# uber-research/UPSNet

Hardware: AMD Instinct MI355X
Metric: images/sec (whole node), UPSNet-50 1024x2048 (higher is better)
Workload: dtype f32

## Files before the change

include/upsnet_hip.h:

```cpp
#ifndef UPSNET_HIP_H
#define UPSNET_HIP_H

#include <stddef.h>
#include <stdint.h>

#ifdef __cplusplus
extern "C" {
#endif

const char *upsnet_last_error(void);
const char *upsnet_last_kernel_form(void);
int upsnet_abi_version(void);

int upsnet_zero_fill(void *stream, void *ptr, size_t bytes);


int upsnet_roi_align_forward(void *stream, const float *bottom_data, float spatial_scale, int num_rois,
                             int height, int width, int channels, int pooled_height, int pooled_width,
                             int sampling_ratio, const float *bottom_rois, float *top_data);

int upsnet_roi_align_forward_nhwc(void *stream, const float *feat_nhwc, int batch, int height, int width,
                                  int channels, float spatial_scale, const float *rois, int num_rois,
                                  int pooled_height, int pooled_width, int sampling_ratio, float *out_nhwc);

int upsnet_fpn_roi_align_forward(void *stream, const float *const feat_nhwc[4], const int feat_h[4],
                                 const int feat_w[4], const float spatial_scale[4], int channels,
                                 const float *rois, int num_rois, const int *num_rois_dev, int pooled_height,
                                 int pooled_width, int sampling_ratio, float *out_nhwc, int *levels_out);

int upsnet_fpn_roi_order(void *stream, const float *rois, int num_rois, const int *num_rois_dev, int image_height, int image_width,
                         int *order_out);
int upsnet_fpn_roi_align_forward_ordered(void *stream, const float *const feat_nhwc[4], const int feat_h[4], const int feat_w[4],
                                         const float spatial_scale[4], int channels, const float *rois, int num_rois, const int *num_rois_dev,
                                         int pooled_height, int pooled_width, int sampling_ratio, float *out_nhwc, int *levels_out,
                                         const int *order);

void upsnet_roi_tuning(int variant);
void upsnet_roi_geometry(int target_workgroups, int min_bins);


int upsnet_deform_im2col(void *stream, const float *data_im, const float *data_offset, int channels,
                         int height, int width, int ksize_h, int ksize_w, int pad_h, int pad_w, int stride_h,
                         int stride_w, int dilation_h, int dilation_w, int parallel_imgs, int deformable_group,
                         float *data_col);

int upsnet_mod_deform_im2col(void *stream, const float *data_im, const float *data_offset,
                             const float *data_mask, int batch_size, int channels, int height_im, int width_im,
                             int height_col, int width_col, int kernel_h, int kernel_w, int pad_h, int pad_w,
                             int stride_h, int stride_w, int dilation_h, int dilation_w, int deformable_group,
                             float *data_col);


int upsnet_roi_align_backward(void *stream, const float *top_diff, float spatial_scale, int batch_size, int num_rois,
                              int height, int width, int channels, int pooled_height, int pooled_width,
                              int sampling_ratio, const float *bottom_rois, float *bottom_diff);

int upsnet_deform_col2im(void *stream, const float *data_col, const float *data_offset, int channels, int height,
                         int width, int ksize_h, int ksize_w, int pad_h, int pad_w, int stride_h, int stride_w,
                         int dilation_h, int dilation_w, int parallel_imgs, int deformable_group, float *grad_im);

int upsnet_deform_col2im_coord(void *stream, const float *data_col, const float *data_im, const float *data_offset,
                               int channels, int height, int width, int ksize_h, int ksize_w, int pad_h, int pad_w,
                               int stride_h, int stride_w, int dilation_h, int dilation_w, int parallel_imgs,
                               int deformable_group, float *grad_offset);

int upsnet_mod_deform_col2im(void *stream, const float *data_col, const float *data_offset, const float *data_mask,
                             int batch_size, int channels, int height_im, int width_im, int height_col, int width_col,
                             int kernel_h, int kernel_w, int pad_h, int pad_w, int stride_h, int stride_w,
                             int dilation_h, int dilation_w, int deformable_group, float *grad_im);

int upsnet_mod_deform_col2im_coord(void *stream, const float *data_col, const float *data_im, const float *data_offset,
                                   const float *data_mask, int batch_size, int channels, int height_im, int width_im,
                                   int height_col, int width_col, int kernel_h, int kernel_w, int pad_h, int pad_w,
                                   int stride_h, int stride_w, int dilation_h, int dilation_w, int deformable_group,
                                   float *grad_offset, float *grad_mask);

int upsnet_deform_conv_forward_nhwc(void *stream, int nlev, const float *const x[], const float *const offset[],
                                    const float *const mask[], float *const out[], const int height[],
                                    const int width[], int cin, int cout, int kh, int kw, int pad_h, int pad_w,
                                    int stride_h, int stride_w, int dil_h, int dil_w, int deformable_group,
                                    const float *wpack, int ldw, const float *bias, int relu);

size_t upsnet_dcn_packed_weight_floats(int cout, int cin, int kh, int kw);
int upsnet_dcn_pack_weight(void *stream, const float *weight, int cout, int cin, int kh, int kw, float *wpack);
int upsnet_deform_conv_fused_nhwc(void *stream, int nlev, const float *const x[], const float *const offset[],
                                  const float *const mask[], float *const out[], const int height[], const int width[],
                                  int cin, int cout, int kh, int kw, int pad, int stride, int dil, const float *wpack,
                                  const float *bias, int relu);
size_t upsnet_deform_conv_fused_splitk_workspace_bytes(int height, int width, int cout, int kh, int kw, int pad, int stride, int dil,
                                                       int ksplit);
int upsnet_deform_conv_fused_nhwc_splitk(void *stream, const float *x, const float *offset, const float *mask, float *out, int height,
                                         int width, int cin, int cout, int kh, int kw, int pad, int stride, int dil,
                                         const float *wpack, const float *bias, int relu, int ksplit, void *workspace);
void upsnet_dcn_tuning(int variant);

size_t upsnet_dcn_packed_weight_bf16_elems(int cout, int cin, int kh, int kw);
int upsnet_dcn_pack_weight_bf16(void *stream, const float *weight, int cout, int cin, int kh, int kw, void *wpack);
int upsnet_deform_conv_fused_nhwc_bf16(void *stream, int nlev, const float *const x[], const float *const offset[],
                                       const float *const mask[], float *const out[], const int height[], const int width[], int cin,
                                       int cout, int kh, int kw, int pad, int stride, int dil, const void *wpack, const float *bias,
                                       int relu);


int upsnet_prep_image_u8(void *stream, const unsigned char *image_hwc, int height, int width, const double pixel_means[3],
                         double im_scale, int resized_h, int resized_w, int padded_h, int padded_w, int nhwc4, float *blob);

int upsnet_image_to_nhwc4(void *stream, const float *nchw, int batch, int channels, int height, int width, float *nhwc4);


int upsnet_conv2d_nhwc_f32_multiw(void *stream, int nseg, const float *const x[], float *const out[], const int batch[],
                                  const int height[], const int width[], int Cin, const float *const wpack[], int ldw, int Cout,
                                  int KH, int KW, int stride, int pad, int relu);

int upsnet_conv2d_nhwc_f32(void *stream, int nseg, const float *const x[], const float *const residual[],
                           float *const out[], const int batch[], const int height[], const int width[], int Cin,
                           const float *wpack, int ldw, const float *bias, int Cout, int KH, int KW, int stride, int pad,
                           int relu, int residual_up);

size_t upsnet_conv2d_splitk_workspace_bytes(int batch, int height, int width, int Cout, int KH, int KW, int stride, int pad, int ksplit);
int upsnet_conv2d_nhwc_f32_splitk(void *stream, const float *x, const float *residual, float *out, int batch, int height, int width,
                                  int Cin, const float *wpack, int ldw, const float *bias, int Cout, int KH, int KW, int stride,
                                  int pad, int relu, int ksplit, void *workspace);

int upsnet_conv2d_winograd_nhwc_f32(void *stream, int nseg, const float *const x[], const float *const residual[],
                                    float *const out[], const int batch[], const int height[], const int width[], int Cin,
                                    const float *wpack, int ldw, const float *bias, int Cout, int relu);

int upsnet_conv2d_winograd_nhwc_f32_splitk(void *stream, const float *x, const float *residual, float *out, int batch, int height,
                                           int width, int Cin, const float *wpack, int ldw, const float *bias, int Cout, int relu,
                                           int ksplit, void *workspace);
int upsnet_conv_pack_weight_winograd(void *stream, const float *weight, int cout, int cin, int ldw, float *wpack);

int upsnet_conv2d_winograd_nhwc_f32_tn32(void *stream, int nseg, const float *const x[], const float *const residual[],
                                         float *const out[], const int batch[], const int height[], const int width[], int Cin,
                                         const float *wpack, int ldw, const float *bias, int Cout, int relu);
int upsnet_conv_pack_weight_winograd_tn32(void *stream, const float *weight, int cout, int cin, int ldw, float *wpack);
int upsnet_conv2d_winograd_nhwc_f32_tail(void *stream, const float *x, float *out, int batch, int n_main, int height, int width, int Cin,
                                         const float *wpack, int ldw, const float *wpack32, int ldw32, const float *bias, int Cout, int relu);

int upsnet_conv2d_nhwc_bf16(void *stream, int nseg, const float *const x[], const float *const residual[], float *const out[],
                            const int batch[], const int height[], const int width[], int Cin, const void *wpack_hi,
                            const void *wpack_lo, int ldw, const float *bias, int Cout, int KH, int KW, int stride, int pad,
                            int relu);
int upsnet_conv_pack_weight_bf16(void *stream, const float *weight, int cout, int cin, int kh, int kw, int ldw, void *wpack_hi,
                                 void *wpack_lo);
int upsnet_bottleneck_proj_bf16(void *stream, const void *x, void *out, int batch, int height_in, int width_in, int cin, int cmid, int stride,
                                const void *w1, const void *w2, const void *w3d, const float *b1, const float *b2, const float *b3d);
int upsnet_conv_bf16_tuning(int enable, int tile_rows);
int upsnet_conv1x1_bf16_tuning(int enable);
int upsnet_stem_pool_pack_weight_f32(void *stream, const float *weight, int cin, float *wpack);
int upsnet_stem_pool_f32(void *stream, const float *x4, int batch, int height, int width, const float *wpack, const float *bias, float *out);
int upsnet_stem_pool_pack_weight_bf16(void *stream, const float *weight, int cin, void *wpack);
int upsnet_stem_pool_bf16(void *stream, const float *x4, int batch, int height, int width, const void *wpack, const float *bias, void *out);
int upsnet_deconv2x2_nhwc_bf16(void *stream, const void *x, int batch, int height, int width, int Cin, const void *wpack_hi, int ldw,
                               const float *bias, int Cout, int relu, void *out, int out_bf16);

int upsnet_bottleneck_bf16(void *stream, const void *x, void *out, int batch, int height, int width, int cmid, const void *w1,
                           const void *w2, const void *w3, const float *b1, const float *b2, const float *b3);

int upsnet_conv2d_stem_nhwc4_f32(void *stream, const float *x, int batch, int height, int width, const float *wpack,
                                 int ldw, const float *bias, int Cout, int KH, int KW, int stride, int pad, int relu,
                                 float *out);
int upsnet_conv_pack_weight_stem(void *stream, const float *weight, int cout, int cin, int kh, int kw, int ldw, float *wpack);

int upsnet_deconv2x2_nhwc_f32(void *stream, const float *x, int batch, int height, int width, int Cin, const float *wpack,
                              int ldw, const float *bias, int Cout, int relu, float *out);
int upsnet_deconv2x2_pack_weight(void *stream, const float *weight, int cin, int cout, int ldw, float *wpack);

int upsnet_deconv2x2_frag_nhwc_f32(void *stream, const float *x, float *out, int batch, int height, int width, int Cin,
                                   const float *wpack, const float *bias4, int Cout, int relu);

void upsnet_conv_tuning(int winograd_tiles, int force_tile);

int upsnet_conv_pack_weight(void *stream, const float *weight, int cout, int cin, int kh, int kw, int ldw, float *wpack);

int upsnet_conv1x1_frag_nhwc_f32(void *stream, const float *x, const float *residual, float *out, int batch, int height, int width,
                                 int Cin, const float *wpack, const float *bias, int Cout, int stride, int relu, int residual_up);
void upsnet_conv1x1_tuning(int bn);
int upsnet_conv1x1_siblings_nhwc_f32(void *stream, const float *x, float *out_a, float *out_b, int batch, int height, int width, int Cin,
                                     const float *wpack, const float *bias, int cout_a, int cout_b, int stride, int relu_a, int relu_b);
void upsnet_conv1x1_pair32_tuning(int waves);

int upsnet_conv2d_winograd36_nhwc_f32(void *stream, int nseg, const float *const x[], float *const out[], const int batch[],
                                      const int height[], const int width[], int Cin, const float *wpack, int ldw, const float *bias,
                                      int Cout, int relu);
int upsnet_conv_pack_weight_winograd36(void *stream, const float *weight, int cout, int cin, int ldw, float *wpack);
size_t upsnet_conv2d_winograd36_splitk_workspace_bytes(int batch, int height, int width, int Cout, int ksplit);
int upsnet_conv2d_winograd36_nhwc_f32_splitk(void *stream, const float *x, float *out, int batch, int height, int width, int Cin,
                                             const float *wpack, int ldw, const float *bias, int Cout, int relu, int ksplit, void *workspace);

size_t upsnet_conv1x1_ksw_packed_weight_floats(int cout, int cin);
int upsnet_conv1x1_ksw_pack_weight(void *stream, const float *weight, int cout, int cin, float *wpack);
int upsnet_conv1x1_ksw_nhwc_f32(void *stream, const float *x, const float *residual, float *out, int batch, int height, int width, int Cin,
                                const float *wpack, const float *bias, int Cout, int stride, int relu, int tile_pixels, int tile_channels,
                                int split_n);
void upsnet_conv1x1_ksw_tuning(int tile);

size_t upsnet_conv3x3_ksw_packed_weight_floats(int cin);
int upsnet_conv3x3_ksw_pack_weight(void *stream, const float *weight, int cout, int cin, float *wpack);
int upsnet_conv3x3_ksw_nhwc_f32(void *stream, const float *x, float *out, int batch, int height, int width, int Cin, const float *wpack,
                                const float *bias, int Cout, int relu);

size_t upsnet_conv1x1_splitk_workspace_bytes(int batch, int out_height, int out_width, int Cout, int ksplit);
int upsnet_conv1x1_frag_nhwc_f32_splitk(void *stream, const float *x, const float *residual, float *out, int batch, int height, int width,
                                        int Cin, const float *wpack, const float *bias, int Cout, int stride, int relu, int ksplit,
                                        void *workspace);

int upsnet_conv1x1_pair_nhwc_f32(void *stream, const float *x, const float *residual, float *out1, float *out2, long pixels, int C0,
                                 const float *w3pack, const float *bias3, int C1, const float *w1pack, const float *bias1, int C2);


int upsnet_nms_host(int *keep_out_host, int *num_out_host, const float *boxes_host, int boxes_num,
                    int boxes_dim, float nms_overlap_thresh, int device_id);

size_t upsnet_nms_workspace_bytes(int num_problems, int nmax);
int upsnet_nms_batched(void *stream, const float *boxes, const float *scores, const int *counts,
                       const uint8_t *pre_removed, int num_problems, int nmax, float thresh, int *keep_idx,
                       int *keep_cnt, void *workspace);

void upsnet_nms_tuning(int lds_staging);

int upsnet_cpu_nms_batched(void *stream, const float *boxes, const float *scores, const int *counts, int num_problems,
                           int nmax, double thresh, int *keep_idx, int *keep_cnt, void *workspace);

size_t upsnet_soft_nms_batched_workspace_bytes(int num_problems, int nmax);
int upsnet_soft_nms_batched(void *stream, float *boxes, int64_t *inds, const int *counts, int num_problems, int nmax,
                            float sigma, float Nt, float threshold, int method, int *n_out, void *workspace);

size_t upsnet_soft_nms_workspace_bytes(int n);
int upsnet_soft_nms(void *stream, float *boxes, int64_t *inds, int n, float sigma, float Nt, float threshold,
                    int method, int *n_out, void *workspace);


size_t upsnet_proposal_workspace_bytes(int nlev, const int *heights_host, const int *widths_host, int num_anchors,
                                       int pre_nms_top_n, int post_nms_top_n);
int upsnet_pyramid_proposals(void *stream, int nlev, const float *const cls_prob[], const float *const bbox_pred[],
                             const int *heights_host, const int *widths_host, const int *strides_host,
                             const float *anchors_host, int num_anchors, const float *im_info, int pre_nms_top_n,
                             int post_nms_top_n, float nms_thresh, float min_size, float *rois_out,
                             float *scores_out, int *num_out, void *workspace);

int upsnet_pyramid_proposals_strided(void *stream, int nlev, const float *const cls_prob[], const float *const bbox_pred[],
                                     const long *cls_chan_stride, const long *cls_pix_stride, const long *box_chan_stride,
                                     const long *box_pix_stride, const int *heights_host, const int *widths_host,
                                     const int *strides_host, const float *anchors_host, int num_anchors, const float *im_info,
                                     int pre_nms_top_n, int post_nms_top_n, float nms_thresh, float min_size, float *rois_out,
                                     float *scores_out, int *num_out, void *workspace);
int upsnet_pyramid_proposals_strided_ordered(void *stream, int nlev, const float *const cls_prob[], const float *const bbox_pred[],
                                     const long *cls_chan_stride, const long *cls_pix_stride, const long *box_chan_stride,
                                     const long *box_pix_stride, const int *heights_host, const int *widths_host,
                                     const int *strides_host, const float *anchors_host, int num_anchors, const float *im_info,
                                     int pre_nms_top_n, int post_nms_top_n, float nms_thresh, float min_size, float *rois_out,
                                     float *scores_out, int *num_out, void *workspace, int *roi_order_out);

int upsnet_pyramid_proposals_joint_strided(void *stream, int nlev, const float *const cls_prob[], const float *const bbox_pred[],
                                           const long *cls_chan_stride, const long *cls_pix_stride, const long *box_chan_stride,
                                           const long *box_pix_stride, const int *heights_host, const int *widths_host,
                                           const int *strides_host, const float *anchors_host, int num_anchors, const float *im_info,
                                           int pre_nms_top_n, int post_nms_top_n, float nms_thresh, float min_size, float *rois_out,
                                           float *scores_out, int *num_out, void *workspace);


int upsnet_mask_roi_capacity(int num_rois, int num_classes, int class_agnostic);
size_t upsnet_mask_roi_workspace_bytes(int num_rois, int num_classes, int class_agnostic);
int upsnet_mask_roi(void *stream, const float *rois, const float *bbox_delta, const float *cls_prob, int num_rois,
                    const int *num_rois_dev, int num_classes, const float *im_info, int class_agnostic,
                    float score_thresh, float nms_thresh, int max_det, const float reg_weights_host[4],
                    float *boxes_out, float *scores_out, int64_t *cls_out, int *src_out, int *num_out,
                    void *workspace);
int upsnet_mask_roi_ex(void *stream, const float *rois, const float *bbox_delta, const float *cls_prob, int num_rois,
                       const int *num_rois_dev, int num_classes, const float *im_info, int class_agnostic, int clip_boxes,
                       float score_thresh, float nms_thresh, int max_det, const float reg_weights_host[4],
                       float *boxes_out, float *scores_out, int64_t *cls_out, int *src_out, int *num_out,
                       void *workspace);

int upsnet_mask_roi_dedup(void *stream, const int *a_src, const int64_t *a_cls, const int *num_a, int cap_a, const int *b_src,
                          const int64_t *b_cls, const float *b_boxes, const int *num_b, int cap_b, int *map_out,
                          float *extra_boxes, int *num_extra);

int upsnet_mask_logit_gather(void *stream, const float *mask_logit, int n_rows, int num_classes, int hw, long stride_n,
                             long stride_c, long stride_e, const int *row, const int64_t *cls, int K, float *out);


size_t upsnet_mask_removal_workspace_bytes(int m, int num_thing_classes, int height, int width);
int upsnet_mask_removal(void *stream, const float *mask_rois, const float *cls_prob, const float *mask_logit,
                        const int64_t *cls_idx, int m, const int *m_dev, int mask_size, int num_thing_classes, int height, int width,
                        double fraction_threshold, int64_t *keep_inds, int *num_keep, int *real_keep,
                        void *workspace);

int upsnet_panoptic_tail_pack(void *stream, const int64_t *keep, const int *num_keep, int K, const int64_t *cls, const float *scores,
                              const int *det_num, const int *pan_num, const int *extra_num, int64_t *kept_cls, float *kept_scores,
                              int *counters);

int upsnet_mask_paste(void *stream, const float *mask_rois, const float *mask_logit, const int64_t *keep_inds,
                      const int *num_keep, const int *real_keep, int kmax, int mask_size, int height, int width,
                      float *mask_energy);

int upsnet_seg_term(void *stream, const float *fcn_output, int num_seg, int height, int width, const float *boxes,
                    const int64_t *cls, const int64_t *class_map, int k, float *seg_inst);

int upsnet_panoptic_fuse(void *stream, const float *fcn_output, int num_seg, int height, int width, int num_stuff,
                         const float *mask_rois, const float *mask_logit, const int64_t *cls_idx,
                         const int64_t *keep_inds, const int *num_keep, const int *real_keep, int kmax,
                         int mask_size, const int64_t *class_map, int enable_void, int64_t *pan_out,
                         int64_t *sem_out);

int upsnet_fcn_score_combine(void *stream, int nlev, const float *const part[], int num_seg, int height, int width,
                             const float *bias, float *score);

int upsnet_panoptic_fuse_up(void *stream, const float *fcn_score, int score_nhwc, int num_seg, int score_h, int score_w,
                            int scale, int num_stuff, const float *mask_rois, const float *mask_logit,
                            const int64_t *cls_idx, const int64_t *keep_inds, const int *num_keep, const int *real_keep,
                            int kmax, int mask_size, const int64_t *class_map, int64_t *pan_out, int64_t *sem_out);

int upsnet_panoptic_argmax(void *stream, const float *fcn_output, int num_seg, int height, int width, int num_stuff,
                           const float *seg_inst, const float *mask_energy, int k, int enable_void,
                           int64_t *pan_out);


size_t upsnet_unified_pan_workspace_bytes(void);
int upsnet_unified_pan_result(void *stream, const int64_t *pan, const int64_t *seg, const int64_t *cls_inds, int num_inst,
                              int height, int width, int id_last_stuff, int num_seg_classes, int stuff_area_limit,
                              void *workspace, unsigned char *pan_2ch);

size_t upsnet_combined_pan_workspace_bytes(int num_images, long total_pixels);
int upsnet_combined_pan_result(void *stream, int num_images, const int64_t *images, int max_height, int max_width, long total_pixels,
                               const int *cand, const int *segments, int id_last_stuff, int num_classes, int stuff_area_limit,
                               double fraction_threshold, void *workspace);

int upsnet_im_post_rle(void *stream, const float *pred_boxes, const float *mask_prob, const int64_t *cls_inds, int num_det,
                       int num_mask_channels, int mask_size, int im_height, int im_width, int cap, unsigned *transitions,
                       int *transition_count);

int upsnet_restore_label_maps(void *stream, const int64_t *sseg, const int64_t *pano, long src_stride, int src_height, int src_width,
                              const int *y_ofs, int out_height, const int *x_ofs, int out_width, unsigned char *out_sseg,
                              unsigned char *out_pano);


size_t upsnet_pq_workspace_bytes(int max_gt);
int upsnet_pq_accumulate(void *stream, const unsigned char *pred_2ch, const unsigned char *gt_rgb, int height, int width,
                         const int64_t *segments, int num_segments, const unsigned char *cat_known, int image_index, int max_gt,
                         void *workspace, int64_t *tp, int64_t *fp, int64_t *fn, double *iou, uint64_t *status);

int upsnet_confusion_accumulate(void *stream, const unsigned char *gt_label, const unsigned char *pred_label, long npix,
                                int class_num, int ignore_label, int64_t *confusion);


size_t upsnet_det_eval_image_workspace_bytes(int num_det, int num_rows, int num_gt, int height, int width, int segm);
int upsnet_det_eval_image(void *stream, int segm, int height, int width, int num_rows, int num_det, const double *det_xyxy,
                          const double *det_score, const int64_t *det_cls, const int *class_to_row, int num_classes,
                          const float *det_box_f32, const float *mask_prob, int num_mask_channels, int mask_size,
                          const int *det_trans, const int64_t *det_trans_off, int num_gt, const int *gt_row_off,
                          const double *gt_box, const double *gt_area, const int *gt_crowd, const int *gt_trans,
                          const int64_t *gt_trans_off, const int *gt_trans_dst, int num_gt_rle, const unsigned char *const *gt_u8,
                          const int *gt_u8_dst, int num_gt_u8, const int *rows_with_gt, int num_rows_with_gt,
                          const double *params, int image_index, void *workspace, double *rec_score, int *rec_img, int *rec_rk,
                          uint64_t *rec_match, uint64_t *rec_ign, int64_t *npig);

size_t upsnet_det_eval_accumulate_workspace_bytes(long num_records, int num_rows);
int upsnet_det_eval_accumulate(void *stream, long num_records, const double *rec_score, const int *rec_img, const int *rec_rk,
                               const uint64_t *rec_match, const uint64_t *rec_ign, const int *img_ord, int num_rows,
                               const int64_t *npig, const double *rec_thrs, void *workspace, double *precision, double *recall,
                               double *scores);

size_t upsnet_poly_raster_workspace_bytes(long total_vertices, long total_points);
int upsnet_poly_raster(void *stream, const double *vertices, const int *poly_off, const int *obj_off, const int *poly_off_dev,
                       const int *obj_off_dev, int num_poly, int num_obj, long total_points, int height, int width, void *workspace,
                       int *trans, int64_t *trans_off);


size_t upsnet_proposal_recall_workspace_bytes(int num_problems, long total_proposals);
int upsnet_proposal_recall(void *stream, int num_problems, const int64_t *problems, const float *proposals, const float *gt_boxes,
                           int max_gt, long total_proposals, void *workspace, float *out);

#ifdef __cplusplus
}
#endif
#endif
```

upsnet_amd/_lib.py:

```python
import ctypes
import os

import torch

_HERE = os.path.dirname(os.path.abspath(__file__))
LIB_PATH = os.environ.get("UPSNET_LIB_PATH") or os.path.join(_HERE, "csrc", "libupsnet_hip.so")

c_int, c_float, c_double, c_void_p, c_size_t, c_long = ctypes.c_int, ctypes.c_float, ctypes.c_double, ctypes.c_void_p, ctypes.c_size_t, ctypes.c_long
P = c_void_p

_SIGNATURES = {
    "upsnet_last_error": (ctypes.c_char_p, []),
    "upsnet_last_kernel_form": (ctypes.c_char_p, []),
    "upsnet_abi_version": (c_int, []),
    "upsnet_zero_fill": (c_int, [P, P, c_size_t]),
    "upsnet_roi_align_forward": (c_int, [P, P, c_float, c_int, c_int, c_int, c_int, c_int, c_int, c_int, P, P]),
    "upsnet_roi_align_forward_nhwc": (c_int, [P, P, c_int, c_int, c_int, c_int, c_float, P, c_int, c_int, c_int, c_int, P]),
    "upsnet_fpn_roi_align_forward": (c_int, [P, P, P, P, P, c_int, P, c_int, P, c_int, c_int, c_int, P, P]),
    "upsnet_fpn_roi_order": (c_int, [P, P, c_int, P, c_int, c_int, P]),
    "upsnet_fpn_roi_align_forward_ordered": (c_int, [P, P, P, P, P, c_int, P, c_int, P, c_int, c_int, c_int, P, P, P]),
    "upsnet_roi_tuning": (None, [c_int]),
    "upsnet_roi_geometry": (None, [c_int, c_int]),
    "upsnet_deform_im2col": (c_int, [P, P, P] + [c_int] * 13 + [P]),
    "upsnet_mod_deform_im2col": (c_int, [P, P, P, P] + [c_int] * 15 + [P]),
    "upsnet_roi_align_backward": (c_int, [P, P, c_float] + [c_int] * 8 + [P, P]),
    "upsnet_deform_col2im": (c_int, [P, P, P] + [c_int] * 13 + [P]),
    "upsnet_deform_col2im_coord": (c_int, [P, P, P, P] + [c_int] * 13 + [P]),
    "upsnet_mod_deform_col2im": (c_int, [P, P, P, P] + [c_int] * 15 + [P]),
    "upsnet_mod_deform_col2im_coord": (c_int, [P, P, P, P, P] + [c_int] * 15 + [P, P]),
    "upsnet_deform_conv_forward_nhwc": (c_int, [P, c_int, P, P, P, P, P, P] + [c_int] * 11 + [P, c_int, P, c_int]),
    "upsnet_dcn_packed_weight_floats": (c_size_t, [c_int, c_int, c_int, c_int]),
    "upsnet_dcn_pack_weight": (c_int, [P, P, c_int, c_int, c_int, c_int, P]),
    "upsnet_deform_conv_fused_nhwc": (c_int, [P, c_int, P, P, P, P, P, P] + [c_int] * 7 + [P, P, c_int]),
    "upsnet_deform_conv_fused_splitk_workspace_bytes": (c_size_t, [c_int] * 9),
    "upsnet_deform_conv_fused_nhwc_splitk": (c_int, [P, P, P, P, P] + [c_int] * 9 + [P, P, c_int, c_int, P]),
    "upsnet_dcn_tuning": (None, [c_int]),
    "upsnet_dcn_packed_weight_bf16_elems": (c_size_t, [c_int, c_int, c_int, c_int]),
    "upsnet_dcn_pack_weight_bf16": (c_int, [P, P, c_int, c_int, c_int, c_int, P]),
    "upsnet_deform_conv_fused_nhwc_bf16": (c_int, [P, c_int, P, P, P, P, P, P] + [c_int] * 7 + [P, P, c_int]),
    "upsnet_conv1x1_frag_nhwc_f32": (c_int, [P, P, P, P, c_int, c_int, c_int, c_int, P, P, c_int, c_int, c_int, c_int]),
    "upsnet_conv1x1_tuning": (None, [c_int]),
    "upsnet_conv1x1_siblings_nhwc_f32": (c_int, [P, P, P, P, c_int, c_int, c_int, c_int, P, P, c_int, c_int, c_int, c_int, c_int]),
    "upsnet_conv1x1_pair32_tuning": (None, [c_int]),
    "upsnet_conv1x1_splitk_workspace_bytes": (ctypes.c_size_t, [c_int, c_int, c_int, c_int, c_int]),
    "upsnet_conv1x1_frag_nhwc_f32_splitk": (c_int, [P, P, P, P, c_int, c_int, c_int, c_int, P, P, c_int, c_int, c_int, c_int, P]),
    "upsnet_conv1x1_ksw_packed_weight_floats": (ctypes.c_size_t, [c_int, c_int]),
    "upsnet_conv1x1_ksw_pack_weight": (c_int, [P, P, c_int, c_int, P]),
    "upsnet_conv1x1_ksw_nhwc_f32": (c_int, [P, P, P, P, c_int, c_int, c_int, c_int, P, P, c_int, c_int, c_int, c_int, c_int, c_int]),
    "upsnet_conv1x1_ksw_tuning": (None, [c_int]),
    "upsnet_conv3x3_ksw_packed_weight_floats": (ctypes.c_size_t, [c_int]),
    "upsnet_conv3x3_ksw_pack_weight": (c_int, [P, P, c_int, c_int, P]),
    "upsnet_conv3x3_ksw_nhwc_f32": (c_int, [P, P, P, c_int, c_int, c_int, c_int, P, P, c_int, c_int]),
    "upsnet_conv2d_winograd36_splitk_workspace_bytes": (ctypes.c_size_t, [c_int, c_int, c_int, c_int, c_int]),
    "upsnet_conv2d_winograd36_nhwc_f32_splitk": (c_int, [P, P, P, c_int, c_int, c_int, c_int, P, c_int, P, c_int, c_int, c_int, P]),
    "upsnet_conv1x1_pair_nhwc_f32": (c_int, [P, P, P, P, P, c_long, c_int, P, P, c_int, P, P, c_int]),
    "upsnet_conv2d_nhwc_f32": (c_int, [P, c_int, P, P, P, P, P, P, c_int, P, c_int, P, c_int, c_int, c_int, c_int, c_int, c_int, c_int]),
    "upsnet_conv2d_nhwc_f32_multiw": (c_int, [P, c_int, P, P, P, P, P, c_int, P, c_int, c_int, c_int, c_int, c_int, c_int, c_int]),
    "upsnet_conv_tuning": (None, [c_int, c_int]),
    "upsnet_conv_pack_weight": (c_int, [P, P, c_int, c_int, c_int, c_int, c_int, P]),
    "upsnet_nms_host": (c_int, [P, P, P, c_int, c_int, c_float, c_int]),
    "upsnet_nms_workspace_bytes": (c_size_t, [c_int, c_int]),
    "upsnet_nms_batched": (c_int, [P, P, P, P, P, c_int, c_int, c_float, P, P, P]),
    "upsnet_nms_tuning": (None, [c_int]),
    "upsnet_cpu_nms_batched": (c_int, [P, P, P, P, c_int, c_int, c_double, P, P, P]),
    "upsnet_soft_nms_batched_workspace_bytes": (c_size_t, [c_int, c_int]),
    "upsnet_soft_nms_batched": (c_int, [P, P, P, P, c_int, c_int, c_float, c_float, c_float, c_int, P, P]),
    "upsnet_soft_nms_workspace_bytes": (c_size_t, [c_int]),
    "upsnet_soft_nms": (c_int, [P, P, P, c_int, c_float, c_float, c_float, c_int, P, P]),
    "upsnet_proposal_workspace_bytes": (c_size_t, [c_int, P, P, c_int, c_int, c_int]),
    "upsnet_pyramid_proposals_strided": (c_int, [P, c_int, P, P, P, P, P, P, P, P, P, P, c_int, P, c_int, c_int, c_float, c_float, P, P, P, P]),
    "upsnet_pyramid_proposals_strided_ordered": (c_int, [P, c_int, P, P, P, P, P, P, P, P, P, P, c_int, P, c_int, c_int, c_float, c_float, P, P, P, P, P]),
    "upsnet_pyramid_proposals_joint_strided": (c_int, [P, c_int, P, P, P, P, P, P, P, P, P, P, c_int, P, c_int, c_int, c_float, c_float, P, P, P, P]),
    "upsnet_pyramid_proposals": (c_int, [P, c_int, P, P, P, P, P, P, c_int, P, c_int, c_int, c_float, c_float, P, P, P, P]),
    "upsnet_mask_roi_capacity": (c_int, [c_int, c_int, c_int]),
    "upsnet_mask_roi_workspace_bytes": (c_size_t, [c_int, c_int, c_int]),
    "upsnet_mask_roi": (c_int, [P, P, P, P, c_int, P, c_int, P, c_int, c_float, c_float, c_int, P, P, P, P, P, P, P]),
    "upsnet_mask_roi_ex": (c_int, [P, P, P, P, c_int, P, c_int, P, c_int, c_int, c_float, c_float, c_int, P, P, P, P, P, P, P]),
    "upsnet_mask_logit_gather": (c_int, [P, P, c_int, c_int, c_int, c_long, c_long, c_long, P, P, c_int, P]),
    "upsnet_mask_removal_workspace_bytes": (c_size_t, [c_int, c_int, c_int, c_int]),
    "upsnet_mask_removal": (c_int, [P, P, P, P, P, c_int, P, c_int, c_int, c_int, c_int, c_double, P, P, P, P]),
    "upsnet_panoptic_tail_pack": (c_int, [P, P, P, c_int, P, P, P, P, P, P, P, P]),
    "upsnet_mask_paste": (c_int, [P, P, P, P, P, P, c_int, c_int, c_int, c_int, P]),
    "upsnet_seg_term": (c_int, [P, P, c_int, c_int, c_int, P, P, P, c_int, P]),
    "upsnet_panoptic_fuse": (c_int, [P, P, c_int, c_int, c_int, c_int, P, P, P, P, P, P, c_int, c_int, P, c_int, P, P]),
    "upsnet_panoptic_fuse_up": (c_int, [P, P, c_int, c_int, c_int, c_int, c_int, c_int, P, P, P, P, P, P, c_int, c_int, P, P, P]),
    "upsnet_conv2d_stem_nhwc4_f32": (c_int, [P, P, c_int, c_int, c_int, P, c_int, P, c_int, c_int, c_int, c_int, c_int, c_int, P]),
    "upsnet_conv_pack_weight_stem": (c_int, [P, P, c_int, c_int, c_int, c_int, c_int, P]),
    "upsnet_deconv2x2_nhwc_f32": (c_int, [P, P, c_int, c_int, c_int, c_int, P, c_int, P, c_int, c_int, P]),
    "upsnet_deconv2x2_pack_weight": (c_int, [P, P, c_int, c_int, c_int, P]),
    "upsnet_deconv2x2_frag_nhwc_f32": (c_int, [P, P, P, c_int, c_int, c_int, c_int, P, P, c_int, c_int]),
    "upsnet_prep_image_u8": (c_int, [P, P, c_int, c_int, P, c_double, c_int, c_int, c_int, c_int, c_int, P]),
    "upsnet_image_to_nhwc4": (c_int, [P, P, c_int, c_int, c_int, c_int, P]),
    "upsnet_unified_pan_workspace_bytes": (c_size_t, []),
    "upsnet_unified_pan_result": (c_int, [P, P, P, P, c_int, c_int, c_int, c_int, c_int, c_int, P, P]),
    "upsnet_combined_pan_workspace_bytes": (c_size_t, [c_int, c_long]),
    "upsnet_combined_pan_result": (c_int, [P, c_int, P, c_int, c_int, c_long, P, P, c_int, c_int, c_int, c_double, P]),
    "upsnet_mask_roi_dedup": (c_int, [P, P, P, P, c_int, P, P, P, P, c_int, P, P, P]),
    "upsnet_conv2d_winograd_nhwc_f32": (c_int, [P, c_int, P, P, P, P, P, P, c_int, P, c_int, P, c_int, c_int]),
    "upsnet_conv2d_winograd_nhwc_f32_splitk": (c_int, [P, P, P, P, c_int, c_int, c_int, c_int, P, c_int, P, c_int, c_int, c_int, P]),
    "upsnet_conv_pack_weight_winograd": (c_int, [P, P, c_int, c_int, c_int, P]),
    "upsnet_conv_pack_weight_winograd_tn32": (c_int, [P, P, c_int, c_int, c_int, P]),
    "upsnet_conv2d_winograd_nhwc_f32_tn32": (c_int, [P, c_int, P, P, P, P, P, P, c_int, P, c_int, P, c_int, c_int]),
    "upsnet_conv2d_winograd_nhwc_f32_tail": (c_int, [P, P, P, c_int, c_int, c_int, c_int, c_int, P, c_int, P, c_int, P, c_int, c_int]),
    "upsnet_conv2d_winograd36_nhwc_f32": (c_int, [P, c_int, P, P, P, P, P, c_int, P, c_int, P, c_int, c_int]),
    "upsnet_conv_pack_weight_winograd36": (c_int, [P, P, c_int, c_int, c_int, P]),
    "upsnet_conv2d_nhwc_bf16": (c_int, [P, c_int, P, P, P, P, P, P, c_int, P, P, c_int, P, c_int, c_int, c_int, c_int, c_int, c_int]),
    "upsnet_bottleneck_proj_bf16": (c_int, [P, P, P, c_int, c_int, c_int, c_int, c_int, c_int, P, P, P, P, P, P]),
    "upsnet_conv_bf16_tuning": (c_int, [c_int, c_int]),
    "upsnet_conv1x1_bf16_tuning": (c_int, [c_int]),
    "upsnet_stem_pool_pack_weight_f32": (c_int, [P, P, c_int, P]),
    "upsnet_stem_pool_f32": (c_int, [P, P, c_int, c_int, c_int, P, P, P]),
    "upsnet_stem_pool_pack_weight_bf16": (c_int, [P, P, c_int, P]),
    "upsnet_stem_pool_bf16": (c_int, [P, P, c_int, c_int, c_int, P, P, P]),
    "upsnet_deconv2x2_nhwc_bf16": (c_int, [P, P, c_int, c_int, c_int, c_int, P, c_int, P, c_int, c_int, P, c_int]),
    "upsnet_bottleneck_bf16": (c_int, [P, P, P, c_int, c_int, c_int, c_int, P, P, P, P, P, P]),
    "upsnet_conv_pack_weight_bf16": (c_int, [P, P, c_int, c_int, c_int, c_int, c_int, P, P]),
    "upsnet_conv2d_splitk_workspace_bytes": (c_size_t, [c_int, c_int, c_int, c_int, c_int, c_int, c_int, c_int, c_int]),
    "upsnet_conv2d_nhwc_f32_splitk": (c_int, [P, P, P, P, c_int, c_int, c_int, c_int, P, c_int, P, c_int, c_int, c_int, c_int, c_int, c_int, c_int, P]),
    "upsnet_im_post_rle": (c_int, [P, P, P, P, c_int, c_int, c_int, c_int, c_int, c_int, P, P]),
    "upsnet_fcn_score_combine": (c_int, [P, c_int, P, c_int, c_int, c_int, P, P]),
    "upsnet_panoptic_argmax": (c_int, [P, P, c_int, c_int, c_int, c_int, P, P, c_int, c_int, P]),
    "upsnet_pq_workspace_bytes": (c_size_t, [c_int]),
    "upsnet_pq_accumulate": (c_int, [P, P, P, c_int, c_int, P, c_int, P, c_int, c_int, P, P, P, P, P, P]),
    "upsnet_restore_label_maps": (c_int, [P, P, P, c_long, c_int, c_int, P, c_int, P, c_int, P, P]),
    "upsnet_confusion_accumulate": (c_int, [P, P, P, c_long, c_int, c_int, P]),
    "upsnet_det_eval_image_workspace_bytes": (c_size_t, [c_int] * 6),
    "upsnet_det_eval_image": (c_int, [P, c_int, c_int, c_int, c_int, c_int, P, P, P, P, c_int, P, P, c_int, c_int, P, P, c_int, P, P, P, P,
                                      P, P, P, c_int, P, P, c_int, P, c_int, P, c_int, P, P, P, P, P, P, P]),
    "upsnet_det_eval_accumulate_workspace_bytes": (c_size_t, [c_long, c_int]),
    "upsnet_det_eval_accumulate": (c_int, [P, c_long, P, P, P, P, P, P, c_int, P, P, P, P, P, P]),
    "upsnet_poly_raster_workspace_bytes": (c_size_t, [c_long, c_long]),
    "upsnet_poly_raster": (c_int, [P, P, P, P, P, P, c_int, c_int, c_long, c_int, c_int, P, P, P]),
    "upsnet_proposal_recall_workspace_bytes": (c_size_t, [c_int, c_long]),
    "upsnet_proposal_recall": (c_int, [P, c_int, P, P, P, c_int, c_long, P, P]),
}

_lib = None


def exported_symbols():
    return sorted(_SIGNATURES)


def lib():
    global _lib
    if _lib is None:
        if not os.path.exists(LIB_PATH):
            raise RuntimeError("upsnet_amd: %s is missing -- build it with `python -m upsnet_amd.build` "
                               "(there is no CPU fallback)" % LIB_PATH)
        l = ctypes.CDLL(LIB_PATH)
        for name, (res, args) in _SIGNATURES.items():
            fn = getattr(l, name)
            fn.restype = res
            fn.argtypes = args
        _lib = l
    return _lib


def check(rc, what):
    if rc != 0:
        raise RuntimeError("upsnet_amd.%s failed: %s" % (what, lib().upsnet_last_error().decode()))


def ptr(t):
    return None if t is None else c_void_p(t.data_ptr())


def stream():
    return c_void_p(torch.cuda.current_stream().cuda_stream)


def require_cuda(*tensors):
    for t in tensors:
        if t is not None and not t.is_cuda:
            raise Exception("not implemented")


def f32c(t):
    if t.dtype != torch.float32:
        t = t.float()
    return t.contiguous()


def nhwc(t):
    return t.contiguous(memory_format=torch.channels_last)


def int_array(vals):
    return (c_int * len(vals))(*[int(v) for v in vals])


def float_array(vals):
    return (c_float * len(vals))(*[float(v) for v in vals])


def ptr_array(tensors):
    return (c_void_p * len(tensors))(*[None if t is None else t.data_ptr() for t in tensors])
```

upsnet_amd/csrc/conv_params.h:

```cpp
#pragma once
#include "common.h"

#define CV_BM 128
#define CV_BK 32
#define CV_LDA (CV_BM + 1)
#define CV_MAXSEG 5

typedef float floatx16 __attribute__((ext_vector_type(16)));

struct ConvSeg {
    const float *x, *res, *off, *mask;
    const float *w;
    float *out;
    int N, H, W, Ho, Wo;
    int OH, OW;
    int tile_start;
    long M;
};

struct ConvParams {
    ConvSeg seg[CV_MAXSEG];
    const float *w, *bias;
    int nseg, Cin, Cout, ldw, KH, KW, stride, pad, dil, relu;
    int res_up;
    int m_tiles, n_tiles;
    int ksplit;
    float *partial;
    long m_total;
    int io;
    int sib_split, sib_relu;
    float *sib_out;
};

static inline int conv_fill(ConvParams &p, const char *who, int nseg, const float *const x[], const float *const res[],
                     const float *const off[], const float *const mask[], float *const out[], const int batch[],
                     const int height[], const int width[], int Cin, int Cout, const float *wpack, int ldw, const float *bias,
                     int KH, int KW, int stride, int pad, int dil, int relu)
{
    UPS_REQUIRE(nseg >= 1 && nseg <= CV_MAXSEG, "%s: 1..%d feature maps per launch (got %d)", who, CV_MAXSEG, nseg);
    UPS_REQUIRE(x && out && height && width && wpack, "%s: null pointer", who);
    UPS_REQUIRE(Cin > 0 && Cin % CV_BK == 0, "%s: Cin must be a multiple of 32 (got %d)", who, Cin);
    UPS_REQUIRE(Cout > 0 && ldw % 32 == 0 && ldw >= Cout, "%s: ldw must be Cout rounded up to 32 (got %d for Cout=%d)", who, ldw, Cout);
    UPS_REQUIRE(KH >= 1 && KW >= 1 && KH * KW <= 49 && stride >= 1 && pad >= 0 && dil >= 1, "%s: bad kernel/stride/pad/dilation", who);
    UPS_REQUIRE((long)KH * KW * Cin * ldw < (1L << 30), "%s: packed weight exceeds 4 GiB", who);
    p.w = wpack; p.bias = bias; p.nseg = nseg; p.Cin = Cin; p.Cout = Cout; p.ldw = ldw; p.KH = KH; p.KW = KW;
    p.stride = stride; p.pad = pad; p.dil = dil; p.relu = relu; p.res_up = 0;
    p.ksplit = 1; p.partial = nullptr; p.m_total = 0; p.io = 0; p.sib_split = 0; p.sib_relu = 0; p.sib_out = nullptr;
    int tiles = 0;
    for (int i = 0; i < CV_MAXSEG; ++i) {
        ConvSeg &s = p.seg[i];
        if (i < nseg) {
            const int nb = batch ? batch[i] : 1;
            UPS_REQUIRE(x[i] && out[i] && nb > 0 && height[i] > 0 && width[i] > 0, "%s: bad feature map %d", who, i);
            s.x = x[i]; s.out = out[i]; s.res = res ? res[i] : nullptr; s.off = off ? off[i] : nullptr; s.mask = mask ? mask[i] : nullptr;
            s.w = nullptr;
            s.N = nb; s.H = height[i]; s.W = width[i];
            s.OH = s.OW = 0;
            s.Ho = (height[i] + 2 * pad - (dil * (KH - 1) + 1)) / stride + 1;
            s.Wo = (width[i] + 2 * pad - (dil * (KW - 1) + 1)) / stride + 1;
            UPS_REQUIRE(s.Ho > 0 && s.Wo > 0, "%s: empty output for feature map %d", who, i);
            UPS_REQUIRE((long)nb * height[i] * width[i] * Cin < (1L << 30), "%s: feature map %d exceeds 4 GiB (32-bit byte offsets); split the batch", who, i);
            s.M = (long)nb * s.Ho * s.Wo;
            UPS_REQUIRE(s.M * Cout < (1L << 29), "%s: output %d exceeds 2 GiB (32-bit byte offsets in the epilogue); split the batch", who, i);
            s.tile_start = tiles;
            tiles += (int)((s.M + 127) / 128);
        } else {
            s.x = s.res = s.off = s.mask = nullptr; s.w = nullptr; s.out = nullptr;
            s.N = s.H = s.W = s.Ho = s.Wo = s.OH = s.OW = 0; s.M = 0; s.tile_start = 0x7fffffff;
        }
    }
    p.m_tiles = tiles;
    return 0;
}


int conv_splitk_reduce(hipStream_t st, const float *partial, int ksplit, long m_total, long M, int Cout, const float *bias, const float *res,
                       int relu, float *out);
```

upsnet_amd/csrc/conv_wino.hip:

```cpp
#include <cstdlib>
#include "conv_params.h"
#include "upsnet_hip.h"

#define WG_STEPS 32

typedef unsigned uintx4 __attribute__((ext_vector_type(4)));
typedef unsigned uintx2 __attribute__((ext_vector_type(2)));

__device__ static inline float f1sub(const float a, const float b) { float r; asm("v_sub_f32 %0, %1, %2" : "=v"(r) : "v"(a), "v"(b)); return r; }
__device__ static inline float f1add(const float a, const float b) { float r; asm("v_add_f32 %0, %1, %2" : "=v"(r) : "v"(a), "v"(b)); return r; }
__device__ static inline float2 f2sub(const float2 a, const float2 b) { return make_float2(f1sub(a.x, b.x), f1sub(a.y, b.y)); }
__device__ static inline float2 f2add(const float2 a, const float2 b) { return make_float2(f1add(a.x, b.x), f1add(a.y, b.y)); }

template <bool SPLITK, int TM, int TN>
__device__ __forceinline__ void conv_wino16_body(const ConvParams &p, const int wg)
{
    static_assert(TN == 64 || (TN == 32 && TM == 32), "tile forms: 64x64, 32x64, 32x32");
    extern __shared__ __attribute__((aligned(16))) unsigned char smem_raw[];
    constexpr unsigned WG_BUF = 16u * 4u * TM * 16u;
    constexpr int NPAIR = (TM / 32) * (TN / 32);
    constexpr int NX = (TM / 8) / NPAIR;
    constexpr int NA = 16 / NX;
    constexpr int NS = 2 * NA;
    constexpr unsigned BSTEP = TN * 32u;
    constexpr int WG_RING = 4;
    const int tid = threadIdx.x, lane = tid & 63, wave = tid >> 6;
    const int pair = wave % NPAIR, xh = wave / NPAIR;
    const int wm = TM == 64 ? (pair & 1) : 0, wn = TM == 64 ? (pair >> 1) : pair;
    const int lhalf = lane >> 5, l32 = lane & 31;
    int m_t, n_t, kz;
    {
        const int nt = p.n_tiles;
        const int per = (p.m_tiles + 7) >> 3;
        const int base_grid = 8 * per * nt;
        kz = SPLITK ? wg / base_grid : 0;
        const int bid = wg - kz * base_grid;
        const int q = bid >> 3;
        n_t = q % nt;
        const int local = q / nt;
        m_t = (bid & 7) * per + local;
        if (local >= per || m_t >= p.m_tiles) return;
    }
    int si = 0;
#pragma unroll
    for (int q = 1; q < CV_MAXSEG; ++q) if (q < p.nseg && m_t >= p.seg[q].tile_start) si = q;
    const ConvSeg sg = p.seg[si];
    const long p0 = (long)(m_t - sg.tile_start) * TM;
    const int n0 = n_t * TN;
    const int nslabs = p.Cin >> 4;
    const int s_per = SPLITK ? (nslabs + p.ksplit - 1) / p.ksplit : nslabs;
    const int s_begin = kz * s_per, s_end = min(s_begin + s_per, nslabs);
    const long HoWo = (long)sg.Ho * sg.Wo;

    const int ltile = tid >> 3, lc2 = tid & 7, lq = lc2 >> 1;
    unsigned ro0, ro1, ro2, ro3, co0, co1, co2, co3;
    {
        const long pp = p0 + ltile;
        const bool tile_ok = pp < sg.M;
        const long ppc = tile_ok ? pp : sg.M - 1;
        const int n = (int)(ppc / HoWo);
        const int rem = (int)(ppc - (long)n * HoWo);
        const int ty = rem / sg.Wo, tx = rem - ty * sg.Wo;
        const int h0 = 2 * ty - 1, w0 = 2 * tx - 1;
        const unsigned cin4 = 4u * (unsigned)p.Cin;
        unsigned ro[4], co[4];
#pragma unroll
        for (int r = 0; r < 4; ++r) {
            const int h = h0 + r, w = w0 + r;
            const unsigned rv = (unsigned)((n * sg.H + min(max(h, 0), sg.H - 1)) * sg.W) * cin4;
            const unsigned cv = (unsigned)min(max(w, 0), sg.W - 1) * cin4 + 8u * (unsigned)lc2;
            ro[r] = rv | ((tile_ok && h >= 0 && h < sg.H) ? 0u : 0x80000000u);
            co[r] = cv | ((w >= 0 && w < sg.W) ? 0u : 0x40000000u);
        }
        ro0 = ro[0]; ro1 = ro[1]; ro2 = ro[2]; ro3 = ro[3];
        co0 = co[0]; co1 = co[1]; co2 = co[2]; co3 = co[3];
    }
    const size_t xaddr = reinterpret_cast<size_t>(sg.x);
    const unsigned xlo = __builtin_amdgcn_readfirstlane((unsigned)xaddr), xhi = __builtin_amdgcn_readfirstlane((unsigned)(xaddr >> 32));
    const unsigned xbytes = __builtin_amdgcn_readfirstlane((unsigned)(sg.N * sg.H * sg.W) * 4u * (unsigned)p.Cin);
    const char *xbase = reinterpret_cast<const char *>(((size_t)xhi << 32) | xlo);
    const unsigned st_base = (unsigned)((lq * TM + (ltile ^ (2 * lq))) * 16 + (lc2 & 1) * 8);
    const int frow = 32 * wm + l32;
    constexpr unsigned PLANE = TM * 16u;
    const unsigned fr_base0 = (unsigned)(lhalf * PLANE + (frow ^ (2 * lhalf)) * 16 + xh * NS * 2 * PLANE);
    const unsigned fr_base1 = (unsigned)(lhalf * PLANE + (frow ^ (4 + 2 * lhalf)) * 16 + xh * NS * 2 * PLANE);
    const size_t waddr = reinterpret_cast<size_t>(p.w) + (size_t)n_t * (size_t)nslabs * (WG_STEPS * BSTEP);
    const unsigned wlo = __builtin_amdgcn_readfirstlane((unsigned)waddr), whi = __builtin_amdgcn_readfirstlane((unsigned)(waddr >> 32));
    const __amdgpu_buffer_rsrc_t wrsrc = __builtin_amdgcn_make_buffer_rsrc(reinterpret_cast<void *>(((size_t)whi << 32) | wlo), 0,
                                                                            nslabs * (int)(WG_STEPS * BSTEP), 0x00020000);
    const unsigned b_lane = (unsigned)(lhalf * (TN * 16) + (32 * wn + l32) * 16);
    const int gmax = nslabs * WG_STEPS - 1;
    const int xh_u = __builtin_amdgcn_readfirstlane(xh);

    floatx16 acc[NA];
#pragma unroll
    for (int i = 0; i < NA; ++i)
#pragma unroll
        for (int r = 0; r < 16; ++r) acc[i][r] = 0.f;

#define WG_PO(PX) (((PX) >> 2) == 0 ? ro0 : ((PX) >> 2) == 1 ? ro1 : ((PX) >> 2) == 2 ? ro2 : ro3) + (((PX) & 3) == 0 ? co0 : ((PX) & 3) == 1 ? co1 : ((PX) & 3) == 2 ? co2 : co3)
    float2 ld[16];
    float4 breg[WG_RING];

#define WG_LOAD(PX, RS) { const uintx2 v_ = __builtin_amdgcn_raw_buffer_load_b64(RS, WG_PO(PX), 0, 0); ld[PX] = make_float2(__uint_as_float(v_.x), __uint_as_float(v_.y)); }
#define WG_ROWPASS(R)                                                                                                 \
    {                                                                                                                 \
        const float2 d0 = ld[4 * R + 0], d1 = ld[4 * R + 1], d2 = ld[4 * R + 2], d3 = ld[4 * R + 3];                 \
        ld[4 * R + 0] = f2sub(d0, d2); ld[4 * R + 1] = f2add(d1, d2); ld[4 * R + 2] = f2sub(d2, d1); ld[4 * R + 3] = f2sub(d1, d3); \
    }
#define WG_COLSTASH(J, SB)                                                                                            \
    {                                                                                                                 \
        *reinterpret_cast<float2 *>(smem_raw + (SB) + (0 * 4 + J) * 4 * PLANE) = f2sub(ld[0 + J], ld[8 + J]);            \
        *reinterpret_cast<float2 *>(smem_raw + (SB) + (1 * 4 + J) * 4 * PLANE) = f2add(ld[4 + J], ld[8 + J]);            \
        *reinterpret_cast<float2 *>(smem_raw + (SB) + (2 * 4 + J) * 4 * PLANE) = f2sub(ld[8 + J], ld[4 + J]);            \
        *reinterpret_cast<float2 *>(smem_raw + (SB) + (3 * 4 + J) * 4 * PLANE) = f2sub(ld[4 + J], ld[12 + J]);           \
    }
#define WG_BLOAD(SLOT, G) { const uintx4 v_ = __builtin_amdgcn_raw_buffer_load_b128(wrsrc, b_lane, (unsigned)min((G), gmax) * BSTEP, 0); \
        breg[SLOT] = make_float4(__uint_as_float(v_.x), __uint_as_float(v_.y), __uint_as_float(v_.z), __uint_as_float(v_.w)); }

    {
        const __amdgpu_buffer_rsrc_t xr = __builtin_amdgcn_make_buffer_rsrc(const_cast<char *>(xbase) + (size_t)s_begin * 64, 0, xbytes - (unsigned)s_begin * 64u, 0x00020000);
#pragma unroll
        for (int i = 0; i < 16; ++i) WG_LOAD(i, xr)
#pragma unroll
        for (int u = 0; u < WG_RING; ++u) WG_BLOAD(u, s_begin * WG_STEPS + NS * xh_u + u)
        WG_ROWPASS(0) WG_ROWPASS(1) WG_ROWPASS(2) WG_ROWPASS(3)
        WG_COLSTASH(0, st_base) WG_COLSTASH(1, st_base) WG_COLSTASH(2, st_base) WG_COLSTASH(3, st_base)
    }
    __syncthreads();
    float4 afr = *reinterpret_cast<const float4 *>(smem_raw + fr_base0);

    for (int s = s_begin; s < s_end; ++s) {
        const int sn = min(s + 1, s_end - 1);
        const __amdgpu_buffer_rsrc_t xr = __builtin_amdgcn_make_buffer_rsrc(const_cast<char *>(xbase) + (size_t)sn * 64, 0, xbytes - (unsigned)sn * 64u, 0x00020000);
        const unsigned cur = ((s - s_begin) & 1) ? WG_BUF : 0u, nxt = WG_BUF - cur;
        const unsigned sb = nxt + st_base;
        const int g0 = s * WG_STEPS + NS * xh_u;
#pragma unroll
        for (int u = 0; u < NS; ++u) {
            if (NS == 16 && u < 8) { WG_LOAD(2 * u, xr) WG_LOAD(2 * u + 1, xr) }
            if (NS == 8 && u < 4) { WG_LOAD(4 * u, xr) WG_LOAD(4 * u + 1, xr) WG_LOAD(4 * u + 2, xr) WG_LOAD(4 * u + 3, xr) }
            float4 afn;
            if (u < NS - 1) afn = *reinterpret_cast<const float4 *>(smem_raw + cur + (((u + 1) & 1) ? fr_base1 : fr_base0) + (unsigned)(u + 1) * 2u * PLANE);
            else afn = *reinterpret_cast<const float4 *>(smem_raw + nxt + fr_base0);
            if (NS == 16) {
                if (u == 8) WG_ROWPASS(0)
                if (u == 9) WG_ROWPASS(1)
                if (u == 10) WG_ROWPASS(2)
                if (u == 11) { WG_ROWPASS(3) WG_COLSTASH(0, sb) }
                if (u == 12) WG_COLSTASH(1, sb)
                if (u == 13) WG_COLSTASH(2, sb)
                if (u == 14) WG_COLSTASH(3, sb)
            } else {
                if (u == 4) { WG_ROWPASS(0) WG_ROWPASS(1) }
                if (u == 5) { WG_ROWPASS(2) WG_ROWPASS(3) WG_COLSTASH(0, sb) }
                if (u == 6) { WG_COLSTASH(1, sb) WG_COLSTASH(2, sb) WG_COLSTASH(3, sb) }
            }
            const float4 bf = breg[u % WG_RING];
            acc[u >> 1] = __builtin_amdgcn_mfma_f32_32x32x2f32(afr.x, bf.x, acc[u >> 1], 0, 0, 0);
            acc[u >> 1] = __builtin_amdgcn_mfma_f32_32x32x2f32(afr.y, bf.y, acc[u >> 1], 0, 0, 0);
            acc[u >> 1] = __builtin_amdgcn_mfma_f32_32x32x2f32(afr.z, bf.z, acc[u >> 1], 0, 0, 0);
            acc[u >> 1] = __builtin_amdgcn_mfma_f32_32x32x2f32(afr.w, bf.w, acc[u >> 1], 0, 0, 0);
            WG_BLOAD(u % WG_RING, (u + WG_RING < NS ? g0 : g0 + WG_STEPS - NS) + u + WG_RING)
            if (u == NS - 2) __syncthreads();
            afr = afn;
            __builtin_amdgcn_sched_barrier(0);
        }
    }
#undef WG_LOAD
#undef WG_PO
#undef WG_ROWPASS
#undef WG_COLSTASH
#undef WG_BLOAD

    __syncthreads();
    const bool has_res = sg.res != nullptr;
    const long pbase = p0 + wm * 32 + 4 * lhalf;
    const long pb = pbase < sg.M ? pbase : sg.M - 1;
    const int n_b = (int)(pb / HoWo);
    const int rem_b = (int)(pb - (long)n_b * HoWo);
    const int h_b = rem_b / sg.Wo, w_b = rem_b - h_b * sg.Wo;
    const bool fast = sg.Wo >= 32;
    const int co = n0 + wn * 32 + l32;
    const bool co_ok = co < p.Cout;
    const float bv = (p.bias != nullptr && co_ok) ? p.bias[co] : 0.f;
#define WG_WHERE(OFF, N_, H_, W_)                                                                                     \
    int N_ = n_b, H_ = h_b, W_ = w_b;                                                                                 \
    if (fast) {                                                                                                       \
        W_ += (OFF);                                                                                                  \
        if (W_ >= sg.Wo) { W_ -= sg.Wo; ++H_; }                                                                       \
        if (H_ >= sg.Ho) { H_ -= sg.Ho; ++N_; }                                                                       \
    } else {                                                                                                          \
        const long pp_ = pbase + (OFF);                                                                               \
        N_ = (int)(pp_ / HoWo);                                                                                       \
        const int rem_ = (int)(pp_ - (long)N_ * HoWo);                                                                \
        H_ = rem_ / sg.Wo; W_ = rem_ - H_ * sg.Wo;                                                                    \
    }
    const unsigned crow = (unsigned)p.Cout * 4u;
    const unsigned co4 = 4u * (unsigned)co;
    const size_t oaddr_ = reinterpret_cast<size_t>(SPLITK ? (float *)(p.partial + (long)kz * p.m_total * p.Cout) : sg.out);
    const unsigned obytes_ = __builtin_amdgcn_readfirstlane((unsigned)(SPLITK ? p.m_total : (long)sg.N * sg.OH * sg.OW) * crow);
    const __amdgpu_buffer_rsrc_t orsrc = __builtin_amdgcn_make_buffer_rsrc(
        reinterpret_cast<void *>(((size_t)(unsigned)__builtin_amdgcn_readfirstlane((unsigned)(oaddr_ >> 32)) << 32) | (unsigned)__builtin_amdgcn_readfirstlane((unsigned)oaddr_)),
        0, (int)obytes_, 0x00020000);
    const size_t raddr_ = reinterpret_cast<size_t>(has_res ? sg.res : sg.out);
    const __amdgpu_buffer_rsrc_t rrsrc = __builtin_amdgcn_make_buffer_rsrc(
        reinterpret_cast<void *>(((size_t)(unsigned)__builtin_amdgcn_readfirstlane((unsigned)(raddr_ >> 32)) << 32) | (unsigned)__builtin_amdgcn_readfirstlane((unsigned)raddr_)),
        0, (int)__builtin_amdgcn_readfirstlane((unsigned)((long)sg.N * sg.OH * sg.OW) * crow), 0x00020000);
#define WG_STORE_ROW(N_, OY, OX, V0, V1)                                                                              \
    if ((OY) < sg.OH) {                                                                                               \
        float v0_ = (V0), v1_ = (V1);                                                                                 \
        const unsigned o0_ = (unsigned)(((N_) * sg.OH + (OY)) * sg.OW + (OX)) * crow + co4;                           \
        const unsigned o1_ = ((OX) + 1 < sg.OW) ? o0_ + crow : 0x80000000u;                                           \
        if (!SPLITK) {                                                                                                \
            v0_ = v0_ + bv; v1_ = v1_ + bv;                                                                           \
            if (has_res) {                                                                                            \
                v0_ = v0_ + __uint_as_float(__builtin_amdgcn_raw_buffer_load_b32(rrsrc, o0_, 0, 0));                  \
                v1_ = v1_ + __uint_as_float(__builtin_amdgcn_raw_buffer_load_b32(rrsrc, o1_, 0, 0));                  \
            }                                                                                                         \
            if (p.relu) { v0_ = fmaxf(v0_, 0.f); v1_ = fmaxf(v1_, 0.f); }                                             \
        }                                                                                                             \
        __builtin_amdgcn_raw_buffer_store_b32(__float_as_uint(v0_), orsrc, o0_, 0, 0);                                \
        __builtin_amdgcn_raw_buffer_store_b32(__float_as_uint(v1_), orsrc, o1_, 0, 0);                                \
    }
    if constexpr (NX == 2) {
        float4 *mine = reinterpret_cast<float4 *>(smem_raw + pair * 32768 + xh_u * 16384) + lane;
        const float4 *theirs = reinterpret_cast<const float4 *>(smem_raw + pair * 32768 + (1 - xh_u) * 16384) + lane;
        if (xh_u == 0) {
#pragma unroll
            for (int r = 0; r < 16; ++r) mine[r * 64] = make_float4(acc[4][r], acc[5][r], acc[6][r], acc[7][r]);
        } else {
#pragma unroll
            for (int r = 0; r < 16; ++r) mine[r * 64] = make_float4(acc[0][r], acc[1][r], acc[2][r], acc[3][r]);
        }
        __syncthreads();
#pragma unroll
        for (int r = 0; r < 16; ++r) {
            const int off = (r & 3) + 8 * (r >> 2);
            const float4 o = theirs[r * 64];
            if (!(co_ok && pbase + off < sg.M)) continue;
            WG_WHERE(off, n, h, w)
            float t0, t1, t2, t3;
            if (xh_u == 0) {
                t0 = (acc[0][r] + acc[4][r]) + o.x; t1 = (acc[1][r] + acc[5][r]) + o.y;
                t2 = (acc[2][r] + acc[6][r]) + o.z; t3 = (acc[3][r] + acc[7][r]) + o.w;
            } else {
                t0 = (o.x - acc[0][r]) - acc[4][r]; t1 = (o.y - acc[1][r]) - acc[5][r];
                t2 = (o.z - acc[2][r]) - acc[6][r]; t3 = (o.w - acc[3][r]) - acc[7][r];
            }
            WG_STORE_ROW(n, 2 * h + xh_u, 2 * w, (t0 + t1) + t2, (t1 - t2) - t3)
        }
    } else {
        float4 *mine = reinterpret_cast<float4 *>(smem_raw + xh_u * 16384) + lane;
#pragma unroll
        for (int r = 0; r < 16; ++r) mine[r * 64] = make_float4(acc[0][r], acc[1][r], acc[2][r], acc[3][r]);
        __syncthreads();
#pragma unroll
        for (int rr = 0; rr < 4; ++rr) {
            const int r = 4 * xh_u + rr;
            const int off = rr + 8 * xh_u;
            const float4 m0 = reinterpret_cast<const float4 *>(smem_raw)[r * 64 + lane];
            const float4 m1 = reinterpret_cast<const float4 *>(smem_raw + 16384)[r * 64 + lane];
            const float4 m2 = reinterpret_cast<const float4 *>(smem_raw + 32768)[r * 64 + lane];
            const float4 m3 = reinterpret_cast<const float4 *>(smem_raw + 49152)[r * 64 + lane];
            if (!(co_ok && pbase + off < sg.M)) continue;
            WG_WHERE(off, n, h, w)
            const float a0 = (m0.x + m1.x) + m2.x, a1 = (m0.y + m1.y) + m2.y, a2 = (m0.z + m1.z) + m2.z, a3 = (m0.w + m1.w) + m2.w;
            const float b0 = (m1.x - m2.x) - m3.x, b1 = (m1.y - m2.y) - m3.y, b2 = (m1.z - m2.z) - m3.z, b3 = (m1.w - m2.w) - m3.w;
            WG_STORE_ROW(n, 2 * h, 2 * w, (a0 + a1) + a2, (a1 - a2) - a3)
            WG_STORE_ROW(n, 2 * h + 1, 2 * w, (b0 + b1) + b2, (b1 - b2) - b3)
        }
    }
#undef WG_WHERE
#undef WG_STORE_ROW
}

template <bool SPLITK, int TM, int TN>
__global__ void __launch_bounds__(8 * TM, TM == 64 ? 1 : 2) conv_wino16_f32_kernel(const ConvParams p)
{
    conv_wino16_body<SPLITK, TM, TN>(p, (int)blockIdx.x);
}

__global__ void __launch_bounds__(256, 2) conv_wino16_tail_f32_kernel(const ConvParams pm, const ConvParams pt, const int main_grid)
{
    if ((int)blockIdx.x < main_grid) conv_wino16_body<false, 32, 64>(pm, (int)blockIdx.x);
    else conv_wino16_body<false, 32, 32>(pt, (int)blockIdx.x - main_grid);
}

template <int TM, int TN>
static int conv_wino16_launch_tm(hipStream_t st, ConvParams &p)
{
    int tiles = 0;
    for (int i = 0; i < p.nseg; ++i) { p.seg[i].tile_start = tiles; tiles += (int)((p.seg[i].M + TM - 1) / TM); }
    p.m_tiles = tiles;
    p.n_tiles = p.ldw / TN;
    const size_t smem = 2 * 16 * 4 * TM * 16;
    static std::atomic<unsigned long long> attr_dev{0};
    UPS_ONCE_PER_DEVICE(attr_dev,
        UPS_CHECK_HIP(hipFuncSetAttribute(reinterpret_cast<const void *>(&conv_wino16_f32_kernel<false, TM, TN>), hipFuncAttributeMaxDynamicSharedMemorySize, (int)smem));
        UPS_CHECK_HIP(hipFuncSetAttribute(reinterpret_cast<const void *>(&conv_wino16_f32_kernel<true, TM, TN>), hipFuncAttributeMaxDynamicSharedMemorySize, (int)smem)));
    const int grid = 8 * ((p.m_tiles + 7) / 8) * p.n_tiles;
    if (p.ksplit > 1) hipLaunchKernelGGL((conv_wino16_f32_kernel<true, TM, TN>), dim3(grid * p.ksplit), dim3(8 * TM), smem, st, p);
    else hipLaunchKernelGGL((conv_wino16_f32_kernel<false, TM, TN>), dim3(grid), dim3(8 * TM), smem, st, p);
    UPS_CHECK_LAUNCH("conv_wino16_f32_kernel");
    ups_set_form("wino<%d,%d,%d>", p.ksplit > 1 ? 1 : 0, TM, TN);
    return 0;
}

int g_wino_tm = 0;
static int conv_wino16_launch(hipStream_t st, ConvParams &p, int tn32 = 0)
{
    UPS_REQUIRE(p.Cin % 16 == 0 && (p.ldw == 32 || p.ldw % 64 == 0 || (tn32 && p.ldw % 32 == 0)), "conv2d_winograd_nhwc_f32: Cin %% 16 must be 0 and ldw 32 or a multiple of 64");
    for (int i = 0; i < p.nseg; ++i) {
        UPS_REQUIRE((long)p.seg[i].N * p.seg[i].H * p.seg[i].W * p.Cin < (1L << 28), "conv2d_winograd_nhwc_f32: feature map %d exceeds 1 GiB; split the batch", i);
        UPS_REQUIRE((long)p.seg[i].N * p.seg[i].OH * p.seg[i].OW * p.Cout < (1L << 29), "conv2d_winograd_nhwc_f32: output %d exceeds 2 GiB; split the batch", i);
    }
    if (p.ksplit > 1) {
        const int nslabs = p.Cin / 16;
        UPS_REQUIRE(p.nseg == 1 && p.partial, "conv2d_winograd_nhwc_f32_splitk: one map and a workspace");
        UPS_REQUIRE(((nslabs + p.ksplit - 1) / p.ksplit) * (p.ksplit - 1) < nslabs, "conv2d_winograd_nhwc_f32_splitk: %d K slabs cannot be split %d ways", nslabs, p.ksplit);
        p.m_total = (long)p.seg[0].N * p.seg[0].OH * p.seg[0].OW;
    }
    if (p.ldw == 32 || tn32) {
        UPS_REQUIRE(p.ldw % 32 == 0, "conv2d_winograd_nhwc_f32: the 32-channel form needs ldw %% 32 == 0");
        return conv_wino16_launch_tm<32, 32>(st, p);
    }
    long wgs64 = 0;
    for (int i = 0; i < p.nseg; ++i) wgs64 += (p.seg[i].M + 63) / 64;
    wgs64 *= p.ldw / 64;
    static const long tm64_min = getenv("UPSNET_WINO_TM64_MIN") ? atol(getenv("UPSNET_WINO_TM64_MIN")) : 768;
    const int tm = g_wino_tm ? g_wino_tm : (wgs64 > tm64_min ? 64 : 32);
    return tm == 32 ? conv_wino16_launch_tm<32, 64>(st, p) : conv_wino16_launch_tm<64, 64>(st, p);
}

__global__ void conv_pack_weight_wino16_kernel(const float *__restrict__ w, int cout, int cin, int ldw, int tn, float *__restrict__ wp)
{
    const long total = (long)ldw * cin;
    const int nslabs = cin >> 4;
    for (long idx = (long)blockIdx.x * blockDim.x + threadIdx.x; idx < total; idx += (long)blockDim.x * gridDim.x) {
        const int co = idx % ldw, c = idx / ldw;
        float g[3][3], t[4][3], u[4][4];
#pragma unroll
        for (int a = 0; a < 3; ++a)
#pragma unroll
            for (int b = 0; b < 3; ++b) g[a][b] = co < cout ? w[(((long)co * cin + c) * 3 + a) * 3 + b] : 0.f;
#pragma unroll
        for (int b = 0; b < 3; ++b) {
            t[0][b] = g[0][b];
            t[1][b] = 0.5f * ((g[0][b] + g[1][b]) + g[2][b]);
            t[2][b] = 0.5f * ((g[0][b] - g[1][b]) + g[2][b]);
            t[3][b] = g[2][b];
        }
#pragma unroll
        for (int a = 0; a < 4; ++a) {
            u[a][0] = t[a][0];
            u[a][1] = 0.5f * ((t[a][0] + t[a][1]) + t[a][2]);
            u[a][2] = 0.5f * ((t[a][0] - t[a][1]) + t[a][2]);
            u[a][3] = t[a][2];
        }
        const long blk = ((long)(co / tn) * nslabs + (c >> 4)) * 16;
        const int q = (c & 15) >> 2, ci = c & 3, cl = co % tn;
#pragma unroll
        for (int a = 0; a < 4; ++a)
#pragma unroll
            for (int b = 0; b < 4; ++b) wp[(((blk + a * 4 + b) * 4 + q) * tn + cl) * 4 + ci] = u[a][b];
    }
}

static int wino_pack(void *stream, const float *weight, int cout, int cin, int ldw, int tn, float *wpack)
{
    UPS_REQUIRE(weight && wpack && cout > 0 && cin > 0 && ldw >= cout, "conv_pack_weight_winograd: bad args");
    UPS_REQUIRE(cin % 16 == 0 && (tn == 32 || tn == 64) && ldw % tn == 0, "conv_pack_weight_winograd: Cin %% 16 must be 0 and ldw a multiple of the channel tile");
    const long total = (long)ldw * cin;
    int blocks = (int)((total + 255) / 256);
    if (blocks > 65535) blocks = 65535;
    hipLaunchKernelGGL(conv_pack_weight_wino16_kernel, dim3(blocks), dim3(256), 0, (hipStream_t)stream, weight, cout, cin, ldw, tn, wpack);
    UPS_CHECK_LAUNCH("conv_pack_weight_wino16_kernel");
    return 0;
}

extern "C" int upsnet_conv_pack_weight_winograd(void *stream, const float *weight, int cout, int cin, int ldw, float *wpack)
{
    UPS_REQUIRE(ldw == 32 || ldw % 64 == 0, "conv_pack_weight_winograd: ldw 32 or a multiple of 64");
    return wino_pack(stream, weight, cout, cin, ldw, ldw == 32 ? 32 : 64, wpack);
}

extern "C" int upsnet_conv_pack_weight_winograd_tn32(void *stream, const float *weight, int cout, int cin, int ldw, float *wpack)
{
    return wino_pack(stream, weight, cout, cin, ldw, 32, wpack);
}

static int wino_fill(ConvParams &p, const char *who, int nseg, const float *const x[], const float *const residual[], float *const out[],
                     const int batch[], const int height[], const int width[], int Cin, int Cout, const float *wpack, int ldw,
                     const float *bias, int relu)
{
    int rc = conv_fill(p, who, nseg, x, residual, nullptr, nullptr, out, batch, height, width, Cin, Cout, wpack, ldw, bias, 3, 3, 1, 1, 1, relu);
    if (rc) return rc;
    UPS_REQUIRE((long)16 * Cin * ldw < (1L << 30), "%s: packed weight exceeds 4 GiB", who);
    for (int i = 0; i < nseg; ++i) {
        ConvSeg &s = p.seg[i];
        s.OH = s.Ho; s.OW = s.Wo;
        s.Ho = (s.OH + 1) / 2; s.Wo = (s.OW + 1) / 2;
        s.M = (long)s.N * s.Ho * s.Wo;
    }
    return 0;
}

extern "C" int upsnet_conv2d_winograd_nhwc_f32(void *stream, int nseg, const float *const x[], const float *const residual[],
                                               float *const out[], const int batch[], const int height[], const int width[], int Cin,
                                               const float *wpack, int ldw, const float *bias, int Cout, int relu)
{
    ConvParams p;
    int rc = wino_fill(p, "conv2d_winograd_nhwc_f32", nseg, x, residual, out, batch, height, width, Cin, Cout, wpack, ldw, bias, relu);
    if (rc) return rc;
    return conv_wino16_launch((hipStream_t)stream, p);
}

extern "C" int upsnet_conv2d_winograd_nhwc_f32_tn32(void *stream, int nseg, const float *const x[], const float *const residual[],
                                                    float *const out[], const int batch[], const int height[], const int width[], int Cin,
                                                    const float *wpack, int ldw, const float *bias, int Cout, int relu)
{
    ConvParams p;
    int rc = wino_fill(p, "conv2d_winograd_nhwc_f32_tn32", nseg, x, residual, out, batch, height, width, Cin, Cout, wpack, ldw, bias, relu);
    if (rc) return rc;
    return conv_wino16_launch((hipStream_t)stream, p, 1);
}

extern "C" int upsnet_conv2d_winograd_nhwc_f32_tail(void *stream, const float *x, float *out, int batch, int n_main, int height, int width,
                                                    int Cin, const float *wpack, int ldw, const float *wpack32, int ldw32, const float *bias,
                                                    int Cout, int relu)
{
    UPS_REQUIRE(x && out && wpack && wpack32 && n_main > 0 && n_main < batch && ldw % 64 == 0 && ldw32 % 32 == 0 && Cin % 16 == 0,
                "conv2d_winograd_nhwc_f32_tail: 0 < n_main < batch, ldw %% 64 == 0, ldw32 %% 32 == 0, Cin %% 16 == 0");
    ConvParams pm, pt;
    const float *xm[1] = {x}, *xt[1] = {x + (size_t)n_main * height * width * Cin};
    float *om[1] = {out}, *ot[1] = {out + (size_t)n_main * height * width * Cout};
    const int nm[1] = {n_main}, nt[1] = {batch - n_main}, hh[1] = {height}, ww[1] = {width};
    int rc = wino_fill(pm, "conv2d_winograd_nhwc_f32_tail", 1, xm, nullptr, om, nm, hh, ww, Cin, Cout, wpack, ldw, bias, relu);
    if (rc) return rc;
    rc = wino_fill(pt, "conv2d_winograd_nhwc_f32_tail", 1, xt, nullptr, ot, nt, hh, ww, Cin, Cout, wpack32, ldw32, bias, relu);
    if (rc) return rc;
    UPS_REQUIRE((long)batch * height * width * Cin < (1L << 28) && (long)batch * height * width * Cout < (1L << 29),
                "conv2d_winograd_nhwc_f32_tail: feature map exceeds 1 GiB; split the batch");
    pm.seg[0].tile_start = 0; pm.m_tiles = (int)((pm.seg[0].M + 31) / 32); pm.n_tiles = ldw / 64;
    pt.seg[0].tile_start = 0; pt.m_tiles = (int)((pt.seg[0].M + 31) / 32); pt.n_tiles = ldw32 / 32;
    const int main_grid = 8 * ((pm.m_tiles + 7) / 8) * pm.n_tiles, tail_grid = 8 * ((pt.m_tiles + 7) / 8) * pt.n_tiles;
    const size_t smem = 2 * 16 * 4 * 32 * 16;
    static std::atomic<unsigned long long> attr_dev{0};
    UPS_ONCE_PER_DEVICE(attr_dev, UPS_CHECK_HIP(hipFuncSetAttribute(reinterpret_cast<const void *>(&conv_wino16_tail_f32_kernel), hipFuncAttributeMaxDynamicSharedMemorySize, (int)smem)));
    hipLaunchKernelGGL(conv_wino16_tail_f32_kernel, dim3(main_grid + tail_grid), dim3(256), smem, (hipStream_t)stream, pm, pt, main_grid);
    UPS_CHECK_LAUNCH("conv_wino16_tail_f32_kernel");
    ups_set_form("wino_tail<%d,%d>", main_grid, tail_grid);
    return 0;
}

extern "C" int upsnet_conv2d_winograd_nhwc_f32_splitk(void *stream, const float *x, const float *residual, float *out, int batch, int height,
                                                      int width, int Cin, const float *wpack, int ldw, const float *bias, int Cout, int relu,
                                                      int ksplit, void *workspace)
{
    const float *xs[1] = {x};
    float *os[1] = {out};
    const int nb[1] = {batch}, hh[1] = {height}, ww[1] = {width};
    ConvParams p;
    int rc = wino_fill(p, "conv2d_winograd_nhwc_f32_splitk", 1, xs, nullptr, os, nb, hh, ww, Cin, Cout, wpack, ldw, bias, relu);
    if (rc) return rc;
    UPS_REQUIRE(workspace && ksplit >= 2 && ksplit <= 8, "conv2d_winograd_nhwc_f32_splitk: ksplit must be 2..8 and a workspace given");
    UPS_REQUIRE(Cout % 4 == 0, "conv2d_winograd_nhwc_f32_splitk: Cout must be a multiple of 4");
    p.ksplit = ksplit;
    p.partial = (float *)workspace;
    rc = conv_wino16_launch((hipStream_t)stream, p);
    if (rc) return rc;
    return conv_splitk_reduce((hipStream_t)stream, p.partial, ksplit, p.m_total, p.m_total, Cout, bias, residual, relu, out);
}
```

upsnet_amd/csrc/conv_wino36.hip:

```cpp
#include <cstdlib>
#include <type_traits>
#include "conv_params.h"
#include "upsnet_hip.h"

#define W36_TM 32
#define W36_TN 64
#define W36_PTS 36
#define W36_VBUF (W36_PTS * 4 * W36_TM * 16)
#define W36_BSTEP (2 * W36_TN * 16)
#define W36_STEPS (2 * W36_PTS)
#define W36_XCH (16 * W36_PTS * 64 * 4)
#define W36_RING 3

typedef unsigned w36_uintx4 __attribute__((ext_vector_type(4)));

#define W36_BT(D0, D1, D2, D3, D4, D5)                                                                               \
    {                                                                                                                \
        const float a0_ = D0, a1_ = D1, a2_ = D2, a3_ = D3, a4_ = D4, a5_ = D5;                                       \
        const float e1_ = __builtin_fmaf(-2.25f, a2_, a4_), o1_ = __builtin_fmaf(-2.25f, a1_, a3_);                   \
        const float e3_ = __builtin_fmaf(-0.5625f, a2_, a4_), o3_ = __builtin_fmaf(-0.5625f, a1_, a3_);               \
        D0 = __builtin_fmaf(1.265625f, a0_, __builtin_fmaf(-2.8125f, a2_, a4_));                                     \
        D1 = __builtin_fmaf(0.75f, o1_, e1_);                                                                        \
        D2 = __builtin_fmaf(-0.75f, o1_, e1_);                                                                       \
        D3 = __builtin_fmaf(1.5f, o3_, e3_);                                                                         \
        D4 = __builtin_fmaf(-1.5f, o3_, e3_);                                                                        \
        D5 = __builtin_fmaf(1.265625f, a1_, __builtin_fmaf(-2.8125f, a3_, a5_));                                     \
    }
#define W36_AT(M0, M1, M2, M3, M4, M5, Y0, Y1, Y2, Y3)                                                               \
    {                                                                                                                \
        const float s1_ = (M1) + (M2), d1_ = (M1) - (M2), s2_ = (M3) + (M4), d2_ = (M3) - (M4);                      \
        Y0 = ((M0) + s1_) + s2_;                                                                                     \
        Y1 = __builtin_fmaf(1.5f, d2_, 0.75f * d1_);                                                                 \
        Y2 = __builtin_fmaf(2.25f, s2_, 0.5625f * s1_);                                                              \
        Y3 = __builtin_fmaf(3.375f, d2_, __builtin_fmaf(0.421875f, d1_, (M5)));                                      \
    }

template <bool SK>
__global__ void __launch_bounds__(512, 1) conv_wino36_f32_kernel(const ConvParams p)
{
    extern __shared__ __attribute__((aligned(16))) unsigned char smem_raw[];
    const int tid = threadIdx.x, lane = tid & 63;
    const int wave = __builtin_amdgcn_readfirstlane(tid >> 6);
    const int cb = wave >> 2, pg = wave & 3;
    const int lhalf = lane >> 5, l32 = lane & 31;
    int m_t, n_t, kz = 0;
    {
        const int nt = p.n_tiles;
        const int per = (p.m_tiles + 7) >> 3;
        int bid = (int)blockIdx.x;
        if constexpr (SK) { const int base_grid = 8 * per * nt; kz = bid / base_grid; bid -= kz * base_grid; }
        const int q = bid >> 3;
        n_t = q % nt;
        const int local = q / nt;
        m_t = (bid & 7) * per + local;
        if (local >= per || m_t >= p.m_tiles) return;
    }
    int si = 0;
#pragma unroll
    for (int q = 1; q < CV_MAXSEG; ++q) if (q < p.nseg && m_t >= p.seg[q].tile_start) si = q;
    const ConvSeg sg = p.seg[si];
    const long p0 = (long)(m_t - sg.tile_start) * W36_TM;
    const int nslabs_all = p.Cin >> 4;
    const int s_first = SK ? (kz * nslabs_all) / p.ksplit : 0;
    const int nslabs = SK ? ((kz + 1) * nslabs_all) / p.ksplit - s_first : nslabs_all;
    const long HoWo = (long)sg.Ho * sg.Wo;

    const int ltile = tid >> 4, lch = tid & 15;
    int hrow0, wcol0;
    int hlo, hhi;
    unsigned tbase, nrmask = 0, ncmask = 0;
    bool lane_fix;
    {
        const long pp = p0 + ltile;
        const bool tile_ok = pp < sg.M;
        const long ppc = tile_ok ? pp : sg.M - 1;
        const int n = (int)(ppc / HoWo);
        const int rem = (int)(ppc - (long)n * HoWo);
        const int ty = rem / sg.Wo, tx = rem - ty * sg.Wo;
        const int h0 = 4 * ty - 1;
        hlo = n * sg.H; hhi = tile_ok ? hlo + sg.H : hlo;
        hrow0 = hlo + h0;
        wcol0 = 4 * tx - 1;
#pragma unroll
        for (int r = 0; r < 6; ++r) nrmask |= (h0 + r >= 0 && h0 + r < sg.H) ? 0u : (1u << r);
#pragma unroll
        for (int c = 0; c < 6; ++c) ncmask |= (wcol0 + c >= 0 && wcol0 + c < sg.W) ? 0u : (1u << c);
        lane_fix = tile_ok && (nrmask | ncmask) != 0;
        tbase = (unsigned)(hrow0 * sg.W + wcol0) * (4u * (unsigned)p.Cin) + 4u * (unsigned)lch;
    }
    const bool fix = __builtin_amdgcn_ballot_w64(lane_fix) != 0ull;
    bool risky;
    {
        const long plast = min(p0 + (long)W36_TM, sg.M) - 1;
        const long nl = plast / HoWo;
        const long tyl = (plast - nl * HoWo) / sg.Wo;
        risky = (nl * sg.H + 4 * tyl + 4) * (long)sg.W + 4L * sg.Wo >= (long)sg.N * sg.H * sg.W;
    }
    const unsigned cin4 = 4u * (unsigned)p.Cin;
    const unsigned rowpitch = (unsigned)sg.W * cin4;
    const unsigned cin4_s = __builtin_amdgcn_readfirstlane(cin4);
    const unsigned rowpitch_s = __builtin_amdgcn_readfirstlane((unsigned)sg.W) * cin4_s;
    const unsigned cbase = (unsigned)wcol0 * cin4 + 4u * (unsigned)lch;
#define W36_ROWOFF(R) (((unsigned)min(max(hrow0 + (R), hlo), max(hhi - 1, hlo)) * rowpitch) | ((hrow0 + (R) >= hlo && hrow0 + (R) < hhi) ? 0u : 0x80000000u))
    const size_t xaddr = reinterpret_cast<size_t>(sg.x);
    const unsigned xlo = __builtin_amdgcn_readfirstlane((unsigned)xaddr), xhi = __builtin_amdgcn_readfirstlane((unsigned)(xaddr >> 32));
    const unsigned xbytes = __builtin_amdgcn_readfirstlane((unsigned)(sg.N * sg.H * sg.W) * 4u * (unsigned)p.Cin - (SK ? (unsigned)s_first * 64u : 0u));
    const char *xbase = reinterpret_cast<const char *>(((size_t)xhi << 32) | xlo) + (SK ? (size_t)s_first * 64 : 0);
#define W36_SWZ(Q) ((((Q) & 1) << 2) | (((Q) >> 1) << 1))
    const unsigned st_base = (unsigned)((((lch >> 2) * W36_TM + (ltile ^ W36_SWZ(lch >> 2))) * 16) + (lch & 3) * 4);
    constexpr unsigned XI_PITCH = 4 * W36_TM * 16;
    const unsigned fr_base0 = (unsigned)((lhalf * W36_TM + (l32 ^ W36_SWZ(lhalf))) * 16) + (unsigned)pg * 9u * XI_PITCH;
    const unsigned fr_base1 = (unsigned)(((2 + lhalf) * W36_TM + (l32 ^ W36_SWZ(2 + lhalf))) * 16) + (unsigned)pg * 9u * XI_PITCH;
    const size_t waddr = reinterpret_cast<size_t>(p.w) + ((size_t)n_t * (size_t)nslabs_all + (size_t)s_first) * (W36_STEPS * W36_BSTEP);
    const unsigned wlo = __builtin_amdgcn_readfirstlane((unsigned)waddr), whi = __builtin_amdgcn_readfirstlane((unsigned)(waddr >> 32));
    const __amdgpu_buffer_rsrc_t wrsrc = __builtin_amdgcn_make_buffer_rsrc(reinterpret_cast<void *>(((size_t)whi << 32) | wlo), 0,
                                                                            nslabs * (int)(W36_STEPS * W36_BSTEP), 0x00020000);
    const unsigned b_lane = (unsigned)(lhalf * (W36_TN * 16) + (32 * cb + l32) * 16);
    const int gmax = nslabs * W36_STEPS - 1;

    floatx16 acc[9];
#pragma unroll
    for (int i = 0; i < 9; ++i)
#pragma unroll
        for (int r = 0; r < 16; ++r) acc[i][r] = 0.f;

    float ld[36];
    float4 breg[W36_RING];

#define W36_LOADROW_FAST(R, RS) { unsigned so_ = (unsigned)((R) ? (R) - 1 : 0) * rowpitch_s; asm volatile("" : "+s"(so_));              \
        ld[6 * (R)] = __uint_as_float(__builtin_amdgcn_raw_buffer_load_b32(RS, (R) ? tbase + rowpitch_s : tbase, so_, 0));               \
        _Pragma("unroll") for (int c_ = 1; c_ < 6; ++c_) ld[6 * (R) + c_] = __uint_as_float(__builtin_amdgcn_raw_buffer_load_b32(       \
            RS, ((R) ? tbase + rowpitch_s : tbase) + cin4_s, so_ + (unsigned)(c_ - 1) * cin4_s, 0)); }
#define W36_LOADROW_SAFE(R, RS) { unsigned cb_ = cbase; asm volatile("" : "+v"(cb_)); const unsigned rb_ = W36_ROWOFF(R) + cb_; _Pragma("unroll") for (int c_ = 0; c_ < 6; ++c_) \
        ld[6 * (R) + c_] = __uint_as_float(__builtin_amdgcn_raw_buffer_load_b32(RS, (rb_ + (unsigned)c_ * cin4) | ((ncmask << (30 - c_)) & 0x40000000u), 0, 0)); }
#define W36_FIXROW(R) if (fix) { asm volatile("" ::: "memory"); const unsigned bad_ = ((nrmask >> (R)) & 1u) ? 0x3fu : ncmask;           \
        _Pragma("unroll") for (int c_ = 0; c_ < 6; ++c_) ld[6 * (R) + c_] = ((bad_ >> c_) & 1u) ? 0.f : ld[6 * (R) + c_]; }
#define W36_ROWPASS(R) W36_BT(ld[6 * (R) + 0], ld[6 * (R) + 1], ld[6 * (R) + 2], ld[6 * (R) + 3], ld[6 * (R) + 4], ld[6 * (R) + 5])
#define W36_COLSTASH(J, SB)                                                                                           \
    {                                                                                                                 \
        float c0_ = ld[0 + (J)], c1_ = ld[6 + (J)], c2_ = ld[12 + (J)], c3_ = ld[18 + (J)], c4_ = ld[24 + (J)], c5_ = ld[30 + (J)]; \
        W36_BT(c0_, c1_, c2_, c3_, c4_, c5_)                                                                          \
        *reinterpret_cast<float *>(smem_raw + (SB) + (0 * 6 + (J)) * XI_PITCH) = c0_;                                 \
        *reinterpret_cast<float *>(smem_raw + (SB) + (1 * 6 + (J)) * XI_PITCH) = c1_;                                 \
        *reinterpret_cast<float *>(smem_raw + (SB) + (2 * 6 + (J)) * XI_PITCH) = c2_;                                 \
        *reinterpret_cast<float *>(smem_raw + (SB) + (3 * 6 + (J)) * XI_PITCH) = c3_;                                 \
        *reinterpret_cast<float *>(smem_raw + (SB) + (4 * 6 + (J)) * XI_PITCH) = c4_;                                 \
        *reinterpret_cast<float *>(smem_raw + (SB) + (5 * 6 + (J)) * XI_PITCH) = c5_;                                 \
    }
#define W36_BLOAD(SLOT, G) { const w36_uintx4 v_ = __builtin_amdgcn_raw_buffer_load_b128(wrsrc, b_lane, (unsigned)min((G), gmax) * W36_BSTEP, 0); \
        breg[SLOT] = make_float4(__uint_as_float(v_.x), __uint_as_float(v_.y), __uint_as_float(v_.z), __uint_as_float(v_.w)); }

#pragma unroll
    for (int u = 0; u < W36_RING; ++u) W36_BLOAD(u, 18 * pg + u)
    {
        const __amdgpu_buffer_rsrc_t xr = __builtin_amdgcn_make_buffer_rsrc(const_cast<char *>(xbase), 0, xbytes, 0x00020000);
#pragma unroll
        for (int r = 0; r < 6; ++r) { W36_LOADROW_SAFE(r, xr) }
#pragma unroll
        for (int r = 0; r < 6; ++r) { W36_ROWPASS(r) }
#pragma unroll
        for (int j = 0; j < 6; ++j) { W36_COLSTASH(j, st_base) }
    }
    __syncthreads();
    float4 afr = *reinterpret_cast<const float4 *>(smem_raw + fr_base0);

    auto slab_loop = [&](auto fast_tag) __attribute__((always_inline)) {
    constexpr bool FAST = decltype(fast_tag)::value;
    for (int s = 0; s < nslabs; ++s) {
        const int sn = min(s + 1, nslabs - 1);
        const __amdgpu_buffer_rsrc_t xr = __builtin_amdgcn_make_buffer_rsrc(const_cast<char *>(xbase) + (size_t)sn * 64, 0, xbytes - (unsigned)sn * 64u, 0x00020000);
        const unsigned cur = (s & 1) ? W36_VBUF : 0u, nxt = W36_VBUF - cur;
        const unsigned sb = nxt + st_base;
        const int g0 = s * W36_STEPS + 18 * pg;
#pragma unroll
        for (int u = 0; u < 18; ++u) {
            if (u < 6) { if constexpr (FAST) { W36_LOADROW_FAST(u, xr) } else { W36_LOADROW_SAFE(u, xr) } }
            float4 afn;
            if (u < 17) afn = *reinterpret_cast<const float4 *>(smem_raw + cur + (((u + 1) & 1) ? fr_base1 : fr_base0) + (unsigned)((u + 1) >> 1) * XI_PITCH);
            else afn = *reinterpret_cast<const float4 *>(smem_raw + nxt + fr_base0);
            if (u == 6) { if constexpr (FAST) { W36_FIXROW(0) } W36_ROWPASS(0) }
            if (u == 7) { if constexpr (FAST) { W36_FIXROW(1) } W36_ROWPASS(1) }
            if (u == 8) { if constexpr (FAST) { W36_FIXROW(2) } W36_ROWPASS(2) }
            if (u == 9) { if constexpr (FAST) { W36_FIXROW(3) } W36_ROWPASS(3) }
            if (u == 10) { if constexpr (FAST) { W36_FIXROW(4) } W36_ROWPASS(4) }
            if (u == 11) { if constexpr (FAST) { W36_FIXROW(5) } W36_ROWPASS(5) W36_COLSTASH(0, sb) }
            if (u == 12) { W36_COLSTASH(1, sb) }
            if (u == 13) { W36_COLSTASH(2, sb) }
            if (u == 14) { W36_COLSTASH(3, sb) }
            if (u == 15) { W36_COLSTASH(4, sb) }
            if (u == 16) { W36_COLSTASH(5, sb) }
            const float4 bf = breg[u % W36_RING];
            acc[u >> 1] = __builtin_amdgcn_mfma_f32_32x32x2f32(afr.x, bf.x, acc[u >> 1], 0, 0, 0);
            acc[u >> 1] = __builtin_amdgcn_mfma_f32_32x32x2f32(afr.y, bf.y, acc[u >> 1], 0, 0, 0);
            acc[u >> 1] = __builtin_amdgcn_mfma_f32_32x32x2f32(afr.z, bf.z, acc[u >> 1], 0, 0, 0);
            acc[u >> 1] = __builtin_amdgcn_mfma_f32_32x32x2f32(afr.w, bf.w, acc[u >> 1], 0, 0, 0);
            W36_BLOAD(u % W36_RING, (u + W36_RING < 18 ? g0 : g0 + W36_STEPS - 18) + u + W36_RING)
            if (u == 16) __syncthreads();
            afr = afn;
            __builtin_amdgcn_sched_barrier(0);
        }
    }
    };
    if (risky) slab_loop(std::false_type{}); else slab_loop(std::true_type{});
#undef W36_LOADROW_FAST
#undef W36_LOADROW_SAFE
#undef W36_ROWOFF
#undef W36_FIXROW
#undef W36_ROWPASS
#undef W36_COLSTASH
#undef W36_BLOAD

    const unsigned crow = (unsigned)p.Cout * 4u;
    const size_t oaddr_ = reinterpret_cast<size_t>(SK ? p.partial + (size_t)kz * (size_t)p.m_total * (size_t)p.Cout : sg.out);
    const unsigned obytes_ = __builtin_amdgcn_readfirstlane((unsigned)((long)sg.N * sg.OH * sg.OW) * crow);
    const __amdgpu_buffer_rsrc_t orsrc = __builtin_amdgcn_make_buffer_rsrc(
        reinterpret_cast<void *>(((size_t)(unsigned)__builtin_amdgcn_readfirstlane((unsigned)(oaddr_ >> 32)) << 32) | (unsigned)__builtin_amdgcn_readfirstlane((unsigned)oaddr_)),
        0, (int)obytes_, 0x00020000);
    float *xch = reinterpret_cast<float *>(smem_raw);
#pragma unroll 1
    for (int bb = 0; bb < 2; ++bb) {
        __syncthreads();
        if (cb == bb) {
#pragma unroll
            for (int u = 0; u < 9; ++u)
#pragma unroll
                for (int r = 0; r < 16; ++r) xch[(r * W36_PTS + 9 * pg + u) * 64 + lane] = acc[u][r];
        }
        __syncthreads();
        const int co_ch = n_t * W36_TN + 32 * bb + l32;
        const bool co_ok = co_ch < p.Cout;
        const float bv = (p.bias != nullptr && co_ok) ? p.bias[co_ch] : 0.f;
#pragma unroll 1
        for (int rr = 0; rr < 2; ++rr) {
            const int r = 2 * wave + rr;
            const long pp = p0 + 8 * (r >> 2) + 4 * lhalf + (r & 3);
            float m[36];
#pragma unroll
            for (int x = 0; x < 36; ++x) m[x] = xch[(r * W36_PTS + x) * 64 + lane];
            if (!(co_ok && pp < sg.M)) continue;
            const int n = (int)(pp / HoWo);
            const int rem = (int)(pp - (long)n * HoWo);
            const int ty = rem / sg.Wo, tx = rem - ty * sg.Wo;
            float t[6][4];
#pragma unroll
            for (int i = 0; i < 6; ++i) W36_AT(m[6 * i + 0], m[6 * i + 1], m[6 * i + 2], m[6 * i + 3], m[6 * i + 4], m[6 * i + 5], t[i][0], t[i][1], t[i][2], t[i][3])
#pragma unroll
            for (int c = 0; c < 4; ++c) {
                float y[4];
                W36_AT(t[0][c], t[1][c], t[2][c], t[3][c], t[4][c], t[5][c], y[0], y[1], y[2], y[3])
                const int ox = 4 * tx + c;
#pragma unroll
                for (int a = 0; a < 4; ++a) {
                    const int oy = 4 * ty + a;
                    float v = y[a];
                    if constexpr (!SK) { v = v + bv; if (p.relu) v = fmaxf(v, 0.f); }
                    const unsigned off = (oy < sg.OH && ox < sg.OW) ? (unsigned)((n * sg.OH + oy) * sg.OW + ox) * crow + 4u * (unsigned)co_ch : 0x80000000u;
                    __builtin_amdgcn_raw_buffer_store_b32(__float_as_uint(v), orsrc, off, 0, 0);
                }
            }
        }
    }
}

static int w36_fill(ConvParams &p, const char *who, int nseg, const float *const x[], float *const out[], const int batch[], const int height[],
                    const int width[], int Cin, int Cout, const float *wpack, int ldw, const float *bias, int relu)
{
    UPS_REQUIRE(Cin > 0 && Cin % 32 == 0 && ldw % W36_TN == 0, "%s: Cin %% 32 == 0 and ldw %% 64 == 0 (got %d, %d)", who, Cin, ldw);
    int rc = conv_fill(p, who, nseg, x, nullptr, nullptr, nullptr, out, batch, height, width, Cin, Cout, wpack, ldw, bias, 3, 3, 1, 1, 1, relu);
    if (rc) return rc;
    UPS_REQUIRE((long)W36_PTS * Cin * ldw < (1L << 29), "%s: packed weight exceeds 2 GiB", who);
    int tiles = 0;
    for (int i = 0; i < nseg; ++i) {
        ConvSeg &s = p.seg[i];
        s.OH = s.Ho; s.OW = s.Wo;
        s.Ho = (s.OH + 3) / 4; s.Wo = (s.OW + 3) / 4;
        s.M = (long)s.N * s.Ho * s.Wo;
        UPS_REQUIRE((long)s.N * s.H * s.W * Cin < (1L << 28), "%s: feature map %d exceeds 1 GiB; split the batch", who, i);
        UPS_REQUIRE((long)s.N * s.OH * s.OW * Cout < (1L << 29), "%s: output %d exceeds 2 GiB; split the batch", who, i);
        s.tile_start = tiles;
        tiles += (int)((s.M + W36_TM - 1) / W36_TM);
    }
    p.m_tiles = tiles;
    p.n_tiles = ldw / W36_TN;
    return 0;
}

extern "C" int upsnet_conv2d_winograd36_nhwc_f32(void *stream, int nseg, const float *const x[], float *const out[], const int batch[],
                                                 const int height[], const int width[], int Cin, const float *wpack, int ldw, const float *bias,
                                                 int Cout, int relu)
{
    ConvParams p;
    int rc = w36_fill(p, "conv2d_winograd36_nhwc_f32", nseg, x, out, batch, height, width, Cin, Cout, wpack, ldw, bias, relu);
    if (rc) return rc;
    static std::atomic<unsigned long long> attr_dev{0};
    UPS_ONCE_PER_DEVICE(attr_dev, UPS_CHECK_HIP(hipFuncSetAttribute(reinterpret_cast<const void *>(&conv_wino36_f32_kernel<false>), hipFuncAttributeMaxDynamicSharedMemorySize, W36_XCH)));
    const int grid = 8 * ((p.m_tiles + 7) / 8) * p.n_tiles;
    hipLaunchKernelGGL(conv_wino36_f32_kernel<false>, dim3(grid), dim3(512), W36_XCH, (hipStream_t)stream, p);
    UPS_CHECK_LAUNCH("conv_wino36_f32_kernel");
    ups_set_form("wino36<%d,%d>", W36_TM, W36_TN);
    return 0;
}

extern "C" size_t upsnet_conv2d_winograd36_splitk_workspace_bytes(int batch, int height, int width, int Cout, int ksplit)
{
    return (size_t)ksplit * (size_t)batch * height * width * Cout * sizeof(float);
}

extern "C" int upsnet_conv2d_winograd36_nhwc_f32_splitk(void *stream, const float *x, float *out, int batch, int height, int width, int Cin,
                                                        const float *wpack, int ldw, const float *bias, int Cout, int relu, int ksplit,
                                                        void *workspace)
{
    const float *xs[1] = {x};
    float *os[1] = {out};
    const int nb[1] = {batch}, hh[1] = {height}, ww[1] = {width};
    ConvParams p;
    int rc = w36_fill(p, "conv2d_winograd36_nhwc_f32_splitk", 1, xs, os, nb, hh, ww, Cin, Cout, wpack, ldw, bias, relu);
    if (rc) return rc;
    UPS_REQUIRE(workspace && ksplit >= 2 && ksplit <= 8 && Cin / 16 >= ksplit, "conv2d_winograd36_nhwc_f32_splitk: ksplit 2..8, <= Cin / 16, and a workspace");
    p.ksplit = ksplit;
    p.partial = (float *)workspace;
    p.m_total = (long)batch * height * width;
    UPS_REQUIRE(p.m_total * Cout < (1L << 29), "conv2d_winograd36_nhwc_f32_splitk: output exceeds 2 GiB; split the batch");
    static std::atomic<unsigned long long> attr_dev{0};
    UPS_ONCE_PER_DEVICE(attr_dev, UPS_CHECK_HIP(hipFuncSetAttribute(reinterpret_cast<const void *>(&conv_wino36_f32_kernel<true>), hipFuncAttributeMaxDynamicSharedMemorySize, W36_XCH)));
    const int grid = 8 * ((p.m_tiles + 7) / 8) * p.n_tiles * ksplit;
    hipLaunchKernelGGL(conv_wino36_f32_kernel<true>, dim3(grid), dim3(512), W36_XCH, (hipStream_t)stream, p);
    UPS_CHECK_LAUNCH("conv_wino36_f32_kernel<splitk>");
    ups_set_form("wino36<%d,%d> splitk%d", W36_TM, W36_TN, ksplit);
    return conv_splitk_reduce((hipStream_t)stream, p.partial, ksplit, p.m_total, p.m_total, Cout, bias, nullptr, relu, out);
}

__global__ void conv_pack_weight_wino36_kernel(const float *__restrict__ w, int cout, int cin, int ldw, float *__restrict__ wp)
{
    const long total = (long)ldw * cin;
    const int nslabs = cin >> 4;
    const double G[6][3] = {{64.0 / 81, 0.0, 0.0}, {-128.0 / 243, -32.0 / 81, -8.0 / 27}, {-128.0 / 243, 32.0 / 81, -8.0 / 27},
                            {32.0 / 243, 16.0 / 81, 8.0 / 27}, {32.0 / 243, -16.0 / 81, 8.0 / 27}, {0.0, 0.0, 1.0}};
    for (long idx = (long)blockIdx.x * blockDim.x + threadIdx.x; idx < total; idx += (long)blockDim.x * gridDim.x) {
        const int co = idx % ldw, c = idx / ldw;
        double g[3][3], t[6][3];
#pragma unroll
        for (int a = 0; a < 3; ++a)
#pragma unroll
            for (int b = 0; b < 3; ++b) g[a][b] = co < cout ? (double)w[(((long)co * cin + c) * 3 + a) * 3 + b] : 0.0;
#pragma unroll
        for (int i = 0; i < 6; ++i)
#pragma unroll
            for (int b = 0; b < 3; ++b) t[i][b] = G[i][0] * g[0][b] + G[i][1] * g[1][b] + G[i][2] * g[2][b];
        const long blk = ((long)(co / W36_TN) * nslabs + (c >> 4)) * W36_PTS;
        const int q = (c & 15) >> 2, ci = c & 3, cl = co % W36_TN;
#pragma unroll
        for (int i = 0; i < 6; ++i)
#pragma unroll
            for (int j = 0; j < 6; ++j) {
                const double u = t[i][0] * G[j][0] + t[i][1] * G[j][1] + t[i][2] * G[j][2];
                wp[(((blk + i * 6 + j) * 4 + q) * W36_TN + cl) * 4 + ci] = (float)u;
            }
    }
}

extern "C" int upsnet_conv_pack_weight_winograd36(void *stream, const float *weight, int cout, int cin, int ldw, float *wpack)
{
    UPS_REQUIRE(weight && wpack && cout > 0 && cin > 0 && ldw >= cout, "conv_pack_weight_winograd36: bad args");
    UPS_REQUIRE(cin % 16 == 0 && ldw % W36_TN == 0, "conv_pack_weight_winograd36: Cin %% 16 must be 0 and ldw a multiple of 64");
    const long total = (long)ldw * cin;
    int blocks = (int)((total + 255) / 256);
    if (blocks > 65535) blocks = 65535;
    hipLaunchKernelGGL(conv_pack_weight_wino36_kernel, dim3(blocks), dim3(256), 0, (hipStream_t)stream, weight, cout, cin, ldw, wpack);
    UPS_CHECK_LAUNCH("conv_pack_weight_wino36_kernel");
    return 0;
}
```

upsnet_amd/csrc/proposal.hip:

```cpp
#include "common.h"
#include "roi_order.h"
#include "sort.h"
#include "upsnet_hip.h"

#define PROP_CH 8192
#define PROP_MAXLEV 8

int ups_nms_batched_impl(hipStream_t st, const float *boxes, const float *scores, const int *counts,
                         const uint8_t *pre_removed, int P, int nmax, float thresh, int tie_mode, int *keep_idx,
                         int *keep_cnt, void *workspace, int ge);
void ups_nms_ws_views(void *workspace, int P, int nmax, float4 **sorted_boxes, int **order);
int ups_nms_batched_presorted_impl(hipStream_t st, const int *counts, const uint8_t *pre_removed, int P, int nmax, float thresh,
                                   int *keep_idx, int *keep_cnt, void *workspace, int ge);

struct PropLevels {
    const float *cls[PROP_MAXLEV];
    const float *box[PROP_MAXLEV];
    long cls_cs[PROP_MAXLEV], cls_ps[PROP_MAXLEV];
    long box_cs[PROP_MAXLEV], box_ps[PROP_MAXLEV];
    int H[PROP_MAXLEV], W[PROP_MAXLEV], stride[PROP_MAXLEV];
    int n[PROP_MAXLEV];
    long key_off[PROP_MAXLEV];
    float anchors[PROP_MAXLEV][4][4];
    int nlev, A;
};

struct PropSel {
    ups_u64 prefix;
    unsigned need;
    unsigned done;
    unsigned cnt;
    unsigned pad;
};

#define PROP_BINS 2048

__global__ void __launch_bounds__(256)
prop_key_kernel(const PropLevels lv, ups_u64 *__restrict__ keys, PropSel *__restrict__ sel, const int k)
{
    const int l = blockIdx.y;
    if (blockIdx.x == 0 && threadIdx.x == 0) {
        PropSel st;
        st.prefix = 0; st.need = (unsigned)k; st.done = 0; st.cnt = 0; st.pad = 0;
        sel[l] = st;
    }
    const int n = lv.n[l], A = lv.A;
    const long hw = (long)lv.H[l] * lv.W[l];
    const float *__restrict__ s = lv.cls[l];
    ups_u64 *__restrict__ out = keys + lv.key_off[l];
    for (long i = (long)blockIdx.x * blockDim.x + threadIdx.x; i < n; i += (long)blockDim.x * gridDim.x) {
        const int a = (int)(i / hw);
        const long pix = i % hw;
        const unsigned idx = (unsigned)(pix * A + a);
        out[idx] = ups_make_key(s[a * lv.cls_cs[l] + pix * lv.cls_ps[l]], idx, 1);
    }
}

__global__ void __launch_bounds__(256)
prop_hist_kernel(const PropLevels lv, const ups_u64 *__restrict__ keys, const PropSel *__restrict__ sel, unsigned *__restrict__ hist,
                 const int shift, const int hi)
{
    __shared__ unsigned s_hist[PROP_BINS];
    const int l = blockIdx.y;
    const PropSel st = sel[l];
    if (st.done) return;
    for (int i = threadIdx.x; i < PROP_BINS; i += blockDim.x) s_hist[i] = 0;
    __syncthreads();
    const int n = lv.n[l];
    const ups_u64 *__restrict__ src = keys + lv.key_off[l];
    const unsigned mask = (1u << (hi - shift)) - 1u;
    const long stride = (long)blockDim.x * gridDim.x;
    long i = (long)blockIdx.x * blockDim.x + threadIdx.x;
    for (; i < n; i += 8 * stride) {
        ups_u64 kk[8];
#pragma unroll
        for (int u = 0; u < 8; ++u) kk[u] = (i + u * stride < n) ? src[i + u * stride] : 0ULL;
#pragma unroll
        for (int u = 0; u < 8; ++u)
            if (i + u * stride < n && (hi >= 64 || ((kk[u] ^ st.prefix) >> hi) == 0)) atomicAdd(&s_hist[(unsigned)(kk[u] >> shift) & mask], 1u);
    }
    __syncthreads();
    for (int i = threadIdx.x; i < PROP_BINS; i += blockDim.x) {
        const unsigned v = s_hist[i];
        if (v) atomicAdd(&hist[(long)l * PROP_BINS + i], v);
    }
}

__global__ void __launch_bounds__(256)
prop_pick_kernel(PropSel *__restrict__ sel, unsigned *__restrict__ hist, const int shift, const int last)
{
    __shared__ unsigned s_hist[PROP_BINS], s_part[256];
    const int l = blockIdx.x, tid = threadIdx.x;
    unsigned *h = hist + (long)l * PROP_BINS;
    PropSel st = sel[l];
    unsigned part = 0;
    for (int q = 0; q < PROP_BINS / 256; ++q) {
        const unsigned v = h[tid * (PROP_BINS / 256) + q];
        s_hist[tid * (PROP_BINS / 256) + q] = v;
        part += v;
        h[tid * (PROP_BINS / 256) + q] = 0;
    }
    s_part[tid] = part;
    __syncthreads();
    if (st.done) return;
    unsigned above = 0;
    for (int u = tid + 1; u < 256; ++u) above += s_part[u];
    if (tid == 0 && above + part < st.need) {
        st.done = 1;
        sel[l] = st;
    }
    if (above < st.need && st.need <= above + part) {
        unsigned cum = above;
        for (int q = PROP_BINS / 256 - 1; q >= 0; --q) {
            const int bin = tid * (PROP_BINS / 256) + q;
            const unsigned v = s_hist[bin];
            if (cum + v >= st.need) {
                st.prefix |= (ups_u64)bin << shift;
                st.need -= cum;
                if (v == st.need || last) st.done = 1;
                sel[l] = st;
                break;
            }
            cum += v;
        }
    }
}

__global__ void __launch_bounds__(1024)
prop_tail_select_kernel(const PropLevels lv, const ups_u64 *__restrict__ keys, PropSel *__restrict__ sel)
{
    __shared__ unsigned s_hist[PROP_BINS], s_part[256];
    __shared__ PropSel s_st;
    const int l = blockIdx.x, tid = threadIdx.x;
    PropSel st = sel[l];
    if (st.done) return;
    const int n = lv.n[l];
    const ups_u64 *__restrict__ src = keys + lv.key_off[l];
    const int shifts[3] = {20, 9, 0}, his[3] = {31, 20, 9};
    for (int pass = 0; pass < 3; ++pass) {
        const int shift = shifts[pass], hi = his[pass];
        for (int i = tid; i < PROP_BINS; i += 1024) s_hist[i] = 0;
        __syncthreads();
        const unsigned mask = (1u << (hi - shift)) - 1u;
        for (int i = tid; i < n; i += 1024) {
            const ups_u64 key = src[i];
            if (((key ^ st.prefix) >> hi) == 0) atomicAdd(&s_hist[(unsigned)(key >> shift) & mask], 1u);
        }
        __syncthreads();
        unsigned part = 0;
        if (tid < 256) {
            for (int q = 0; q < PROP_BINS / 256; ++q) part += s_hist[tid * (PROP_BINS / 256) + q];
            s_part[tid] = part;
        }
        if (tid == 0) s_st = st;
        __syncthreads();
        if (tid < 256) {
            unsigned above = 0;
            for (int u = tid + 1; u < 256; ++u) above += s_part[u];
            if (tid == 0 && above + part < st.need) {
                PropSel t = st;
                t.done = 1;
                s_st = t;
            }
            if (above < st.need && st.need <= above + part) {
                unsigned cum = above;
                for (int q = PROP_BINS / 256 - 1; q >= 0; --q) {
                    const int bin = tid * (PROP_BINS / 256) + q;
                    const unsigned v = s_hist[bin];
                    if (cum + v >= st.need) {
                        PropSel t = st;
                        t.prefix |= (ups_u64)bin << shift;
                        t.need -= cum;
                        if (v == t.need || pass == 2) t.done = 1;
                        s_st = t;
                        break;
                    }
                    cum += v;
                }
            }
        }
        __syncthreads();
        st = s_st;
        if (st.done) break;
        __syncthreads();
    }
    if (tid == 0) sel[l] = st;
}

__global__ void __launch_bounds__(256)
prop_compact_kernel(const PropLevels lv, const ups_u64 *__restrict__ keys, PropSel *__restrict__ sel, ups_u64 *__restrict__ out,
                    const int k)
{
    __shared__ unsigned s_wave[4], s_base;
    const int l = blockIdx.y, lane = threadIdx.x & 63, wave = threadIdx.x >> 6;
    const int n = lv.n[l];
    const ups_u64 thr = sel[l].prefix;
    const ups_u64 *__restrict__ src = keys + lv.key_off[l];
    ups_u64 *__restrict__ dst = out + lv.key_off[l];
    const long stride = (long)blockDim.x * gridDim.x;
    for (long i0 = (long)blockIdx.x * blockDim.x; i0 < n; i0 += 8 * stride) {
        ups_u64 kk[8];
#pragma unroll
        for (int u = 0; u < 8; ++u) { const long i = i0 + u * stride + threadIdx.x; kk[u] = i < n ? src[i] : 0ULL; }
        unsigned mine = 0;
#pragma unroll
        for (int u = 0; u < 8; ++u) mine |= (kk[u] != 0ULL && kk[u] >= thr) ? (1u << u) : 0u;
        const unsigned cnt = (unsigned)__builtin_popcount(mine);
        unsigned incl = cnt;
#pragma unroll
        for (int d = 1; d < 64; d <<= 1) { const unsigned t = __shfl_up(incl, d, 64); if (lane >= d) incl += t; }
        if (lane == 63) s_wave[wave] = incl;
        __syncthreads();
        const unsigned w0 = s_wave[0], w1 = s_wave[1], w2 = s_wave[2], w3 = s_wave[3];
        const unsigned total = w0 + w1 + w2 + w3;
        if (total) {
            if (threadIdx.x == 0) s_base = atomicAdd(&sel[l].cnt, total);
            __syncthreads();
            unsigned pos = s_base + (wave > 0 ? w0 : 0u) + (wave > 1 ? w1 : 0u) + (wave > 2 ? w2 : 0u) + (incl - cnt);
#pragma unroll
            for (int u = 0; u < 8; ++u)
                if (mine & (1u << u)) { if (pos < (unsigned)k) dst[pos] = kk[u]; ++pos; }
        }
        __syncthreads();
    }
}

__global__ void __launch_bounds__(1024)
prop_sortk_kernel(const PropLevels lv, const PropSel *__restrict__ sel, ups_u64 *__restrict__ out, const int k, const int M)
{
    extern __shared__ __attribute__((aligned(16))) unsigned char smem_raw[];
    ups_u64 *keys = reinterpret_cast<ups_u64 *>(smem_raw);
    const int l = blockIdx.x;
    const int c = (int)min(sel[l].cnt, (unsigned)k);
    ups_u64 *__restrict__ buf = out + lv.key_off[l];
    for (int i = threadIdx.x; i < M; i += blockDim.x) keys[i] = i < c ? buf[i] : 0ULL;
    ups_block_sort_desc(keys, M);
    for (int i = threadIdx.x; i < k; i += blockDim.x) buf[i] = keys[i];
}

__device__ static inline void prop_decode_anchor(const PropLevels &lv, const int l, const unsigned idx, const float im_h, const float im_w,
                                                 float o[4])
{
    const int A = lv.A, W = lv.W[l];
    const int a = idx % A;
    const int pix = idx / A;
    const int h = pix / W, w = pix % W;
    const float sx = (float)(w * lv.stride[l]), sy = (float)(h * lv.stride[l]);
    const float ax1 = lv.anchors[l][a][0] + sx, ay1 = lv.anchors[l][a][1] + sy;
    const float ax2 = lv.anchors[l][a][2] + sx, ay2 = lv.anchors[l][a][3] + sy;
    const long bcs = lv.box_cs[l];
    const float *__restrict__ d = lv.box[l] + (long)(a * 4) * bcs + (long)pix * lv.box_ps[l];
    ups_decode_clip(ax1, ay1, ax2, ay2, d[0], d[bcs], d[2 * bcs], d[3 * bcs], 1.f, 1.f, 1.f, 1.f, im_h, im_w, true, o);
}

__global__ void __launch_bounds__(1024)
prop_sort_decode_kernel(const PropLevels lv, const PropSel *__restrict__ sel, const ups_u64 *__restrict__ cand, const int k, const int M,
                        const float *__restrict__ im_info, const float min_size, float *__restrict__ boxes, float *__restrict__ scores,
                        uint8_t *__restrict__ pre_removed, int *__restrict__ counts, float4 *__restrict__ sorted_boxes,
                        int *__restrict__ order)
{
    extern __shared__ __attribute__((aligned(16))) unsigned char smem_raw[];
    ups_u64 *keys = reinterpret_cast<ups_u64 *>(smem_raw);
    const int l = blockIdx.x;
    const int c = (int)min(sel[l].cnt, (unsigned)k);
    const ups_u64 *__restrict__ buf = cand + lv.key_off[l];
    for (int i = threadIdx.x; i < M; i += blockDim.x) keys[i] = i < c ? buf[i] : 0ULL;
    ups_block_sort_desc(keys, M);
    if (threadIdx.x == 0) counts[l] = c;
    const float im_h = im_info[0], im_w = im_info[1], ms = min_size * im_info[2];
    for (int i = threadIdx.x; i < k; i += blockDim.x) {
        const long row = (long)l * k + i;
        float *b = boxes + row * 4;
        if (i >= c) {
            b[0] = b[1] = b[2] = b[3] = 0.f;
            scores[row] = 0.f;
            pre_removed[row] = 1;
            continue;
        }
        const ups_u64 key = keys[i];
        float o[4];
        prop_decode_anchor(lv, l, ups_key_index(key, 1), im_h, im_w, o);
        b[0] = o[0]; b[1] = o[1]; b[2] = o[2]; b[3] = o[3];
        scores[row] = ups_key_score(key);
        const float ws = o[2] - o[0] + 1.0f, hs = o[3] - o[1] + 1.0f;
        pre_removed[row] = !((ws >= ms) && (hs >= ms));
        const unsigned sb = (unsigned)(key >> 32);
        int lo = 0, hi = i;
        while (lo < hi) { const int mid = (lo + hi) >> 1; if ((unsigned)(keys[mid] >> 32) > sb) lo = mid + 1; else hi = mid; }
        const int a = lo;
        lo = i; hi = c;
        while (lo < hi) { const int mid = (lo + hi) >> 1; if ((unsigned)(keys[mid] >> 32) >= sb) lo = mid + 1; else hi = mid; }
        const int pos = a + (lo - 1) - i;
        order[(long)l * k + pos] = i;
        sorted_boxes[(long)l * k + pos] = make_float4(o[0], o[1], o[2], o[3]);
    }
}

__global__ void __launch_bounds__(1024)
prop_merge_kernel(const int nlev, const int pre_n, const int post_n, const float *__restrict__ boxes,
                  const float *__restrict__ scores, const int *__restrict__ keep_idx, const int *__restrict__ keep_cnt,
                  float *__restrict__ rois_out, float *__restrict__ scores_out, int *__restrict__ num_out, int *__restrict__ roi_order,
                  const float *__restrict__ im_info)
{
    extern __shared__ __attribute__((aligned(16))) unsigned char smem_raw[];
    ups_u64 *keys = reinterpret_cast<ups_u64 *>(smem_raw);
    __shared__ int s_start[PROP_MAXLEV + 1];
    if (threadIdx.x == 0) {
        int t = 0;
        for (int l = 0; l < nlev; ++l) { s_start[l] = t; t += min(keep_cnt[l], post_n); }
        s_start[nlev] = t;
    }
    __syncthreads();
    const int total = s_start[nlev];
    const int nout = min(total, post_n);
    for (int i = threadIdx.x; i < total; i += blockDim.x) {
        int l = 0;
        for (int q = 1; q < nlev; ++q) if (i >= s_start[q]) l = q;
        const int src = keep_idx[(long)l * pre_n + (i - s_start[l])];
        keys[i] = ups_make_key(scores[(long)l * pre_n + src], (unsigned)i, 1);
    }
    for (int i = nout + threadIdx.x; i < post_n; i += blockDim.x) {
        float *r = rois_out + (long)i * 5;
        r[0] = r[1] = r[2] = r[3] = r[4] = 0.f;
        scores_out[i] = 0.f;
    }
    __syncthreads();
    for (int i = threadIdx.x; i < total; i += blockDim.x) {
        int l = 0;
        for (int q = 1; q < nlev; ++q) if (i >= s_start[q]) l = q;
        const ups_u64 key = keys[i];
        int rank = i - s_start[l];
        for (int q = 0; q < nlev; ++q) {
            if (q == l) continue;
            int lo = s_start[q], hi = s_start[q + 1];
            while (lo < hi) {
                const int mid = (lo + hi) >> 1;
                if (keys[mid] > key) lo = mid + 1; else hi = mid;
            }
            rank += lo - s_start[q];
        }
        if (rank < post_n) {
            const int src = keep_idx[(long)l * pre_n + (i - s_start[l])];
            const float *b = boxes + ((long)l * pre_n + src) * 4;
            float *r = rois_out + (long)rank * 5;
            r[0] = 0.f; r[1] = b[0]; r[2] = b[1]; r[3] = b[2]; r[4] = b[3];
            scores_out[rank] = scores[(long)l * pre_n + src];
        }
    }
    if (threadIdx.x == 0) *num_out = nout;
    if (roi_order != nullptr && post_n <= ROI_ORDER_MAX) {
        __syncthreads();
        ups_roi_order_block(rois_out, post_n, nout, 16.0f / im_info[0], 8.0f / im_info[1], roi_order, reinterpret_cast<int *>(smem_raw));
    }
}


struct PropJoint {
    long goff[PROP_MAXLEV + 1];
};

__global__ void __launch_bounds__(256)
prop_key_joint_kernel(const PropLevels lv, const PropJoint jt, ups_u64 *__restrict__ keys, PropSel *__restrict__ sel, const int k,
                      const float *__restrict__ im_info, const float min_size)
{
    const int l = blockIdx.y;
    if (blockIdx.x == 0 && l == 0 && threadIdx.x == 0) {
        PropSel st;
        st.prefix = 0; st.need = (unsigned)k; st.done = 0; st.cnt = 0; st.pad = 0;
        sel[0] = st;
    }
    const int n = lv.n[l], A = lv.A;
    const long hw = (long)lv.H[l] * lv.W[l];
    const float *__restrict__ s = lv.cls[l];
    const float im_h = im_info[0], im_w = im_info[1], ms = min_size * im_info[2];
    ups_u64 *__restrict__ out = keys + jt.goff[l];
    for (long i = (long)blockIdx.x * blockDim.x + threadIdx.x; i < n; i += (long)blockDim.x * gridDim.x) {
        const int a = (int)(i / hw);
        const long pix = i % hw;
        const unsigned idx = (unsigned)(pix * A + a);
        float o[4];
        prop_decode_anchor(lv, l, idx, im_h, im_w, o);
        const float ws = o[2] - o[0] + 1.0f, hs = o[3] - o[1] + 1.0f;
        const bool ok = (ws >= ms) && (hs >= ms);
        out[idx] = ok ? ups_make_key(s[a * lv.cls_cs[l] + pix * lv.cls_ps[l]], (unsigned)(jt.goff[l] + idx), 0) : 0ULL;
    }
}

__global__ void __launch_bounds__(256)
prop_decode_joint_kernel(const PropLevels lv, const PropJoint jt, const ups_u64 *__restrict__ keys, const PropSel *__restrict__ sel,
                         const int pre_n, const float *__restrict__ im_info, float *__restrict__ boxes, float *__restrict__ scores,
                         int *__restrict__ counts)
{
    const int cnt = (int)min(sel[0].cnt, (unsigned)pre_n);
    if (blockIdx.x == 0 && threadIdx.x == 0) counts[0] = cnt;
    const int i = blockIdx.x * blockDim.x + threadIdx.x;
    if (i >= pre_n) return;
    float *b = boxes + (long)i * 4;
    const ups_u64 key = i < cnt ? keys[i] : 0ULL;
    if (key == 0ULL) {
        b[0] = b[1] = b[2] = b[3] = 0.f;
        scores[i] = 0.f;
        return;
    }
    const long g = (long)ups_key_index(key, 0);
    int l = 0;
    for (int q = 1; q < lv.nlev; ++q) if (g >= jt.goff[q]) l = q;
    float o[4];
    prop_decode_anchor(lv, l, (unsigned)(g - jt.goff[l]), im_info[0], im_info[1], o);
    b[0] = o[0]; b[1] = o[1]; b[2] = o[2]; b[3] = o[3];
    scores[i] = ups_key_score(key);
}

__global__ void __launch_bounds__(256)
prop_emit_joint_kernel(const int post_n, const float *__restrict__ boxes, const float *__restrict__ scores,
                       const int *__restrict__ keep_idx, const int *__restrict__ keep_cnt, float *__restrict__ rois_out,
                       float *__restrict__ scores_out, int *__restrict__ num_out)
{
    const int nout = min(keep_cnt[0], post_n);
    const int i = blockIdx.x * blockDim.x + threadIdx.x;
    if (i == 0) *num_out = nout;
    if (i >= post_n) return;
    float *r = rois_out + (long)i * 5;
    if (i < nout) {
        const int src = keep_idx[i];
        const float *b = boxes + (long)src * 4;
        r[0] = 0.f; r[1] = b[0]; r[2] = b[1]; r[3] = b[2]; r[4] = b[3];
        scores_out[i] = scores[src];
    } else {
        r[0] = r[1] = r[2] = r[3] = r[4] = 0.f;
        scores_out[i] = 0.f;
    }
}

static inline size_t al256(size_t v) { return (v + 255) & ~(size_t)255; }

struct PropPlan {
    long key_total;
    size_t off_keys0, off_keys1, off_boxes, off_scores, off_pre, off_counts, off_keep, off_keepcnt, off_hist, off_sel, off_nms, total;
};

static PropPlan prop_plan(int nlev, const int *H, const int *W, int A, int pre_n)
{
    PropPlan p;
    long tot = 0;
    for (int l = 0; l < nlev; ++l) {
        long n = (long)H[l] * W[l] * A;
        long chunks = (n + PROP_CH - 1) / PROP_CH;
        long need = n > chunks * pre_n ? n : chunks * pre_n;
        tot += need + pre_n;
    }
    p.key_total = tot;
    size_t o = 0;
    p.off_keys0 = o; o += al256((size_t)tot * 8);
    p.off_keys1 = o; o += al256((size_t)tot * 8);
    p.off_boxes = o; o += al256((size_t)nlev * pre_n * 16);
    p.off_scores = o; o += al256((size_t)nlev * pre_n * 4);
    p.off_pre = o; o += al256((size_t)nlev * pre_n);
    p.off_counts = o; o += 256;
    p.off_keep = o; o += al256((size_t)nlev * pre_n * 4);
    p.off_keepcnt = o; o += 256;
    p.off_hist = o; o += al256((size_t)nlev * PROP_BINS * 4);
    p.off_sel = o; o += al256((size_t)nlev * sizeof(PropSel));
    p.off_nms = o; o += upsnet_nms_workspace_bytes(nlev, pre_n);
    p.total = o + 256;
    return p;
}

extern "C" size_t upsnet_proposal_workspace_bytes(int nlev, const int *heights, const int *widths, int num_anchors,
                                                  int pre_nms_top_n, int post_nms_top_n)
{
    (void)post_nms_top_n;
    if (nlev <= 0 || nlev > PROP_MAXLEV || !heights || !widths) return 0;
    return prop_plan(nlev, heights, widths, num_anchors, pre_nms_top_n).total;
}

static int prop_fill_levels(PropLevels &lv, int nlev, const float *const cls_prob[], const float *const bbox_pred[], const long *cls_cs,
                            const long *cls_ps, const long *box_cs, const long *box_ps, const int *heights, const int *widths,
                            const int *strides, const float *anchors, int num_anchors, int pre_n)
{
    lv.nlev = nlev; lv.A = num_anchors;
    long off = 0;
    int maxn = 0;
    for (int l = 0; l < nlev; ++l) {
        if (!(cls_prob[l] && bbox_pred[l] && heights[l] > 0 && widths[l] > 0)) return -1 - l;
        lv.cls[l] = cls_prob[l]; lv.box[l] = bbox_pred[l];
        const long hw_ = (long)heights[l] * widths[l];
        lv.cls_cs[l] = cls_cs ? cls_cs[l] : hw_; lv.cls_ps[l] = cls_ps ? cls_ps[l] : 1;
        lv.box_cs[l] = box_cs ? box_cs[l] : hw_; lv.box_ps[l] = box_ps ? box_ps[l] : 1;
        lv.H[l] = heights[l]; lv.W[l] = widths[l]; lv.stride[l] = strides[l];
        lv.n[l] = heights[l] * widths[l] * num_anchors;
        for (int a = 0; a < num_anchors; ++a)
            for (int q = 0; q < 4; ++q) lv.anchors[l][a][q] = anchors[((long)l * num_anchors + a) * 4 + q];
        long n = lv.n[l];
        long chunks = (n + PROP_CH - 1) / PROP_CH;
        long need = n > chunks * pre_n ? n : chunks * pre_n;
        lv.key_off[l] = off;
        off += need + pre_n;
        if (lv.n[l] > maxn) maxn = lv.n[l];
    }
    return maxn;
}

static int prop_select_compact(hipStream_t st, const PropLevels &lv, int nlev, int maxn, int pre_n, ups_u64 *keys, ups_u64 *out, unsigned *hist,
                               PropSel *sel)
{
    int gh = (maxn + 256 * 8 - 1) / (256 * 8);
    if (gh > 512) gh = 512;
    if (gh < 1) gh = 1;
    static const int digit_shift[3] = {53, 42, 31}, digit_hi[3] = {64, 53, 42};
    for (int pass = 0; pass < 3; ++pass) {
        hipLaunchKernelGGL(prop_hist_kernel, dim3(gh, nlev), dim3(256), 0, st, lv, keys, sel, hist, digit_shift[pass], digit_hi[pass]);
        UPS_CHECK_LAUNCH("prop_hist_kernel");
        hipLaunchKernelGGL(prop_pick_kernel, dim3(nlev), dim3(256), 0, st, sel, hist, digit_shift[pass], 0);
        UPS_CHECK_LAUNCH("prop_pick_kernel");
    }
    hipLaunchKernelGGL(prop_tail_select_kernel, dim3(nlev), dim3(1024), 0, st, lv, keys, sel);
    UPS_CHECK_LAUNCH("prop_tail_select_kernel");
    hipLaunchKernelGGL(prop_compact_kernel, dim3(gh, nlev), dim3(256), 0, st, lv, keys, sel, out, pre_n);
    UPS_CHECK_LAUNCH("prop_compact_kernel");
    return 0;
}

template <auto KERNEL>
static int prop_sort_lds(int pre_n, int *M2_out)
{
    constexpr auto kernel = KERNEL;
    const int M2 = ups_next_pow2(pre_n < 64 ? 64 : pre_n);
    *M2_out = M2;
    if ((size_t)M2 * 8 > 64 * 1024) {
        static std::atomic<unsigned long long> attr_dev{0};
        UPS_ONCE_PER_DEVICE(attr_dev, UPS_CHECK_HIP(hipFuncSetAttribute(reinterpret_cast<const void *>(kernel), hipFuncAttributeMaxDynamicSharedMemorySize,
                                                                        PROP_CH * 8)));
    }
    return 0;
}

extern "C" int upsnet_pyramid_proposals_strided_ordered(void *stream, int nlev, const float *const cls_prob[], const float *const bbox_pred[],
                                        const long *cls_cs, const long *cls_ps, const long *box_cs, const long *box_ps, const int *heights, const int *widths, const int *strides, const float *anchors,
                                        int num_anchors, const float *im_info, int pre_n, int post_n, float nms_thresh,
                                        float min_size, float *rois_out, float *scores_out, int *num_out, void *workspace, int *roi_order_out);

extern "C" int upsnet_pyramid_proposals_strided(void *stream, int nlev, const float *const cls_prob[], const float *const bbox_pred[],
                                        const long *cls_cs, const long *cls_ps, const long *box_cs, const long *box_ps, const int *heights, const int *widths, const int *strides, const float *anchors,
                                        int num_anchors, const float *im_info, int pre_n, int post_n, float nms_thresh,
                                        float min_size, float *rois_out, float *scores_out, int *num_out, void *workspace)
{
    return upsnet_pyramid_proposals_strided_ordered(stream, nlev, cls_prob, bbox_pred, cls_cs, cls_ps, box_cs, box_ps, heights, widths, strides, anchors, num_anchors,
                                                    im_info, pre_n, post_n, nms_thresh, min_size, rois_out, scores_out, num_out, workspace, nullptr);
}

extern "C" int upsnet_pyramid_proposals_strided_ordered(void *stream, int nlev, const float *const cls_prob[], const float *const bbox_pred[],
                                        const long *cls_cs, const long *cls_ps, const long *box_cs, const long *box_ps, const int *heights, const int *widths, const int *strides, const float *anchors,
                                        int num_anchors, const float *im_info, int pre_n, int post_n, float nms_thresh,
                                        float min_size, float *rois_out, float *scores_out, int *num_out, void *workspace, int *roi_order_out)
{
    UPS_REQUIRE(roi_order_out == nullptr || post_n <= ROI_ORDER_MAX, "pyramid_proposals: the ROI order table needs post_nms_top_n <= %d", ROI_ORDER_MAX);
    UPS_REQUIRE(nlev >= 1 && nlev <= PROP_MAXLEV, "pyramid_proposals: nlev must be 1..%d", PROP_MAXLEV);
    UPS_REQUIRE(cls_prob && bbox_pred && heights && widths && strides && anchors && im_info && rois_out && scores_out &&
                    num_out && workspace, "pyramid_proposals: null pointer");
    UPS_REQUIRE(num_anchors >= 1 && num_anchors <= 4, "pyramid_proposals: 1..4 anchors per cell supported (got %d)", num_anchors);
    UPS_REQUIRE(pre_n >= 1 && pre_n <= PROP_CH, "pyramid_proposals: pre_nms_top_n must be 1..%d", PROP_CH);
    UPS_REQUIRE(post_n >= 1 && (long)nlev * (post_n < pre_n ? post_n : pre_n) <= PROP_CH,
                "pyramid_proposals: nlev*post_nms_top_n must be <= %d", PROP_CH);
    hipStream_t st = (hipStream_t)stream;
    const PropPlan plan = prop_plan(nlev, heights, widths, num_anchors, pre_n);
    unsigned char *ws = (unsigned char *)workspace;
    ups_u64 *kbuf[2] = {(ups_u64 *)(ws + plan.off_keys0), (ups_u64 *)(ws + plan.off_keys1)};
    float *boxes = (float *)(ws + plan.off_boxes);
    float *scores = (float *)(ws + plan.off_scores);
    uint8_t *pre_removed = ws + plan.off_pre;
    int *counts = (int *)(ws + plan.off_counts);
    int *keep_idx = (int *)(ws + plan.off_keep);
    int *keep_cnt = (int *)(ws + plan.off_keepcnt);
    void *nms_ws = ws + plan.off_nms;

    PropLevels lv;
    const int maxn = prop_fill_levels(lv, nlev, cls_prob, bbox_pred, cls_cs, cls_ps, box_cs, box_ps, heights, widths, strides, anchors,
                                      num_anchors, pre_n);
    UPS_REQUIRE(maxn > 0, "pyramid_proposals: bad level %d", -1 - maxn);
    int gx = (maxn + 255) / 256;
    if (gx > 1024) gx = 1024;
    unsigned *hist = (unsigned *)(ws + plan.off_hist);
    PropSel *sel = (PropSel *)(ws + plan.off_sel);
    if (ups_zero_async(hist, (size_t)nlev * PROP_BINS * 4, st)) return 1;
    hipLaunchKernelGGL(prop_key_kernel, dim3(gx, nlev), dim3(256), 0, st, lv, kbuf[0], sel, pre_n);
    UPS_CHECK_LAUNCH("prop_key_kernel");

    if (int rc = prop_select_compact(st, lv, nlev, maxn, pre_n, kbuf[0], kbuf[1], hist, sel)) return rc;
    int M2;
    if (int rc = prop_sort_lds<&prop_sort_decode_kernel>(pre_n, &M2)) return rc;
    float4 *nms_sorted_boxes;
    int *nms_order;
    ups_nms_ws_views(nms_ws, nlev, pre_n, &nms_sorted_boxes, &nms_order);
    hipLaunchKernelGGL(prop_sort_decode_kernel, dim3(nlev), dim3(M2 < 1024 ? M2 : 1024), (size_t)M2 * 8, st, lv, sel, kbuf[1], pre_n, M2, im_info,
                       min_size, boxes, scores, pre_removed, counts, nms_sorted_boxes, nms_order);
    UPS_CHECK_LAUNCH("prop_sort_decode_kernel");
    int rc = ups_nms_batched_presorted_impl(st, counts, pre_removed, nlev, pre_n, nms_thresh, keep_idx, keep_cnt, nms_ws, 0);
    if (rc) return rc;
    hipLaunchKernelGGL(prop_merge_kernel, dim3(1), dim3(1024), (size_t)PROP_CH * 8, st, nlev, pre_n, post_n, boxes, scores,
                       keep_idx, keep_cnt, rois_out, scores_out, num_out, roi_order_out, im_info);
    UPS_CHECK_LAUNCH("prop_merge_kernel");
    return 0;
}

extern "C" int upsnet_pyramid_proposals_joint_strided(void *stream, int nlev, const float *const cls_prob[], const float *const bbox_pred[],
                                        const long *cls_cs, const long *cls_ps, const long *box_cs, const long *box_ps, const int *heights, const int *widths, const int *strides, const float *anchors,
                                        int num_anchors, const float *im_info, int pre_n, int post_n, float nms_thresh,
                                        float min_size, float *rois_out, float *scores_out, int *num_out, void *workspace)
{
    UPS_REQUIRE(nlev >= 1 && nlev <= PROP_MAXLEV, "pyramid_proposals_joint: nlev must be 1..%d", PROP_MAXLEV);
    UPS_REQUIRE(cls_prob && bbox_pred && heights && widths && strides && anchors && im_info && rois_out && scores_out &&
                    num_out && workspace, "pyramid_proposals_joint: null pointer");
    UPS_REQUIRE(num_anchors >= 1 && num_anchors <= 4, "pyramid_proposals_joint: 1..4 anchors per cell supported (got %d)", num_anchors);
    UPS_REQUIRE(pre_n >= 1 && pre_n <= PROP_CH, "pyramid_proposals_joint: pre_nms_top_n must be 1..%d (the reference's <= 0 = unlimited is not supported)", PROP_CH);
    UPS_REQUIRE(post_n >= 1, "pyramid_proposals_joint: post_nms_top_n must be >= 1");
    hipStream_t st = (hipStream_t)stream;
    const PropPlan plan = prop_plan(nlev, heights, widths, num_anchors, pre_n);
    unsigned char *ws = (unsigned char *)workspace;
    ups_u64 *kbuf[2] = {(ups_u64 *)(ws + plan.off_keys0), (ups_u64 *)(ws + plan.off_keys1)};
    float *boxes = (float *)(ws + plan.off_boxes);
    float *scores = (float *)(ws + plan.off_scores);
    int *counts = (int *)(ws + plan.off_counts);
    int *keep_idx = (int *)(ws + plan.off_keep);
    int *keep_cnt = (int *)(ws + plan.off_keepcnt);
    unsigned *hist = (unsigned *)(ws + plan.off_hist);
    PropSel *sel = (PropSel *)(ws + plan.off_sel);

    PropLevels lv;
    const int maxn = prop_fill_levels(lv, nlev, cls_prob, bbox_pred, cls_cs, cls_ps, box_cs, box_ps, heights, widths, strides, anchors,
                                      num_anchors, pre_n);
    UPS_REQUIRE(maxn > 0, "pyramid_proposals_joint: bad level %d", -1 - maxn);
    PropJoint jt;
    long total = 0;
    for (int l = 0; l < nlev; ++l) { jt.goff[l] = total; total += lv.n[l]; }
    jt.goff[nlev] = total;
    UPS_REQUIRE(total < (1L << 31), "pyramid_proposals_joint: %ld anchors exceed the 32-bit key index", total);
    PropLevels one = lv;
    one.nlev = 1; one.n[0] = (int)total; one.key_off[0] = 0;

    if (ups_zero_async(hist, (size_t)PROP_BINS * 4, st)) return 1;
    int gx = (maxn + 255) / 256;
    if (gx > 1024) gx = 1024;
    hipLaunchKernelGGL(prop_key_joint_kernel, dim3(gx, nlev), dim3(256), 0, st, lv, jt, kbuf[0], sel, pre_n, im_info, min_size);
    UPS_CHECK_LAUNCH("prop_key_joint_kernel");
    if (int rc = prop_select_compact(st, one, 1, (int)total, pre_n, kbuf[0], kbuf[1], hist, sel)) return rc;
    int M2;
    if (int rc = prop_sort_lds<&prop_sortk_kernel>(pre_n, &M2)) return rc;
    hipLaunchKernelGGL(prop_sortk_kernel, dim3(1), dim3(M2 < 1024 ? M2 : 1024), (size_t)M2 * 8, st, one, sel, kbuf[1], pre_n, M2);
    UPS_CHECK_LAUNCH("prop_sortk_kernel");
    hipLaunchKernelGGL(prop_decode_joint_kernel, dim3((pre_n + 255) / 256), dim3(256), 0, st, lv, jt, kbuf[1], sel, pre_n, im_info,
                       boxes, scores, counts);
    UPS_CHECK_LAUNCH("prop_decode_joint_kernel");
    int rc = ups_nms_batched_impl(st, boxes, scores, counts, nullptr, 1, pre_n, nms_thresh, 0, keep_idx, keep_cnt, ws + plan.off_nms, 0);
    if (rc) return rc;
    hipLaunchKernelGGL(prop_emit_joint_kernel, dim3((post_n + 255) / 256), dim3(256), 0, st, post_n, boxes, scores, keep_idx, keep_cnt,
                       rois_out, scores_out, num_out);
    UPS_CHECK_LAUNCH("prop_emit_joint_kernel");
    return 0;
}

extern "C" int upsnet_pyramid_proposals(void *stream, int nlev, const float *const cls_prob[], const float *const bbox_pred[],
                                        const int *heights, const int *widths, const int *strides, const float *anchors,
                                        int num_anchors, const float *im_info, int pre_n, int post_n, float nms_thresh,
                                        float min_size, float *rois_out, float *scores_out, int *num_out, void *workspace)
{
    return upsnet_pyramid_proposals_strided(stream, nlev, cls_prob, bbox_pred, nullptr, nullptr, nullptr, nullptr, heights, widths, strides,
                                            anchors, num_anchors, im_info, pre_n, post_n, nms_thresh, min_size, rois_out, scores_out,
                                            num_out, workspace);
}
```

upsnet_amd/models/fpn.py:

```python
import torch.nn as nn
import torch.nn.functional as F

from ..config.config import config
from . import hipconv


class FPN(nn.Module):

    def __init__(self, feature_dim, with_extra_level=True, with_bottom_up_path_aggregation=False, with_norm='none',
                 upsample_method='nearest'):
        super(FPN, self).__init__()
        assert with_norm == 'none', "only fpn_with_norm='none' is used by the reference configs"
        assert upsample_method in ['nearest', 'bilinear']
        self.feature_dim = feature_dim
        self.upsample_method = upsample_method
        if with_extra_level:
            self.fpn_p6 = nn.MaxPool2d(kernel_size=1, stride=2)
        if config.network.fpn_with_gap:
            self.fpn_gap = nn.Linear(2048, feature_dim)
        self.fpn_p5_1x1 = nn.Conv2d(2048, feature_dim, 1)
        self.fpn_p4_1x1 = nn.Conv2d(1024, feature_dim, 1)
        self.fpn_p3_1x1 = nn.Conv2d(512, feature_dim, 1)
        self.fpn_p2_1x1 = nn.Conv2d(256, feature_dim, 1)
        self.fpn_p5 = nn.Conv2d(feature_dim, feature_dim, 3, padding=1)
        self.fpn_p4 = nn.Conv2d(feature_dim, feature_dim, 3, padding=1)
        self.fpn_p3 = nn.Conv2d(feature_dim, feature_dim, 3, padding=1)
        self.fpn_p2 = nn.Conv2d(feature_dim, feature_dim, 3, padding=1)
        self.initialize()

    def initialize(self):
        for m in self.modules():
            if isinstance(m, nn.Conv2d):
                nn.init.kaiming_uniform_(m.weight.data, a=1)
                if m.bias is not None:
                    m.bias.data.zero_()

    def fpn_upsample(self, x):
        return F.interpolate(x, scale_factor=2, mode=self.upsample_method,
                             align_corners=False if self.upsample_method == 'bilinear' else None)

    def forward(self, res2, res3, res4, res5):
        p5_1x1 = hipconv.conv(self.fpn_p5_1x1, res5)
        if hasattr(self, 'fpn_gap'):
            gap = self.fpn_gap(F.adaptive_avg_pool2d(res5.float(), (1, 1)).flatten(1)).view(-1, self.feature_dim, 1, 1)
            p5_1x1 = p5_1x1 + gap
        if self.upsample_method == 'nearest' and all(t.shape[2] % 2 == 0 and t.shape[3] % 2 == 0 for t in (res2, res3, res4)):
            ad = hipconv.act_dtype()
            p4_plus = hipconv.conv(self.fpn_p4_1x1, res4, residual=p5_1x1, residual_up=True)
            p3_plus = hipconv.conv(self.fpn_p3_1x1, res3, residual=p4_plus, residual_up=True, out_dtype=ad)
            p2_plus = hipconv.conv(self.fpn_p2_1x1, res2, residual=p3_plus, residual_up=True, out_dtype=ad)
        else:
            p4_plus = hipconv.conv(self.fpn_p4_1x1, res4, residual=self.fpn_upsample(p5_1x1))
            p3_plus = hipconv.conv(self.fpn_p3_1x1, res3, residual=self.fpn_upsample(p4_plus))
            p2_plus = hipconv.conv(self.fpn_p2_1x1, res2, residual=self.fpn_upsample(p3_plus))
        p5 = hipconv.conv(self.fpn_p5, p5_1x1)
        p4 = hipconv.conv(self.fpn_p4, p4_plus)
        p3 = hipconv.conv(self.fpn_p3, p3_plus)
        p2 = hipconv.conv(self.fpn_p2, p2_plus)
        if hasattr(self, 'fpn_p6'):
            return p2, p3, p4, p5, self.fpn_p6(p5)
        return p2, p3, p4, p5
```

upsnet_amd/ops.py:

```python
import os

import numpy as np
import torch

from . import _lib
from ._lib import check, f32c, float_array, int_array, lib, nhwc, ptr, ptr_array, require_cuda, stream


PROFILE = {'enabled': False, 'events': []}


def _prof_begin():
    if not PROFILE['enabled']:
        return None
    ev0 = torch.cuda.Event(enable_timing=True)
    ev0.record()
    return ev0


def _prof_end(ev0, kind, flops, nbytes, label=None):
    ev1 = torch.cuda.Event(enable_timing=True)
    ev1.record()
    PROFILE['events'].append((kind, ev0, ev1, flops, nbytes) if label is None else (kind, ev0, ev1, flops, nbytes, label))

# ... 983 lines not shown

def restore_label_maps(sseg, pano, y_ofs, x_ofs):
    require_cuda(sseg, pano)
    maps = [m.reshape(m.shape[-2], m.shape[-1]) if m is not None else None for m in (sseg, pano)]
    for m in maps:
        if m is not None and (m.dtype != torch.int64 or m.stride(1) != 1):
            raise ValueError("restore_label_maps: int64 maps with contiguous rows required, got %s stride %s" % (m.dtype, m.stride()))
    s, p = maps
    if p is not None and (p.shape != s.shape or p.stride() != s.stride()):
        s, p = s.contiguous(), p.contiguous()
    H, W = s.shape
    ys = torch.as_tensor(y_ofs, dtype=torch.int32).reshape(-1)
    xs = torch.as_tensor(x_ofs, dtype=torch.int32).reshape(-1)
    for name, t, n in (("y_ofs", ys, H), ("x_ofs", xs, W)):
        if t.numel() and (int(t.min()) < 0 or int(t.max()) >= n):
            raise ValueError("restore_label_maps: %s outside 0..%d" % (name, n - 1))
    ys, xs = ys.to(s.device).contiguous(), xs.to(s.device).contiguous()
    H0, W0 = ys.numel(), xs.numel()
    out_s = torch.empty((H0, W0), dtype=torch.uint8, device=s.device)
    out_p = torch.empty((H0, W0), dtype=torch.uint8, device=s.device) if p is not None else None
    if H0 == 0 or W0 == 0:
        return out_s, out_p
    check(lib().upsnet_restore_label_maps(stream(), ptr(s), ptr(p), int(s.stride(0)), H, W, ptr(ys), H0, ptr(xs), W0, ptr(out_s),
                                          ptr(out_p)), "restore_label_maps")
    return out_s, out_p


def unified_pan_result(pan, seg, cls_inds, id_last_stuff, num_seg_classes, stuff_area_limit=4 * 64 * 64):
    require_cuda(pan, seg)
    pan = pan.reshape(pan.shape[-2], pan.shape[-1]).to(torch.int64).contiguous()
    seg = seg.reshape(seg.shape[-2], seg.shape[-1]).to(torch.int64).contiguous()
    if pan.shape != seg.shape:
        raise RuntimeError("unified_pan_result: pan %s and seg %s differ in shape" % (tuple(pan.shape), tuple(seg.shape)))
    cls_inds = cls_inds.to(device=pan.device, dtype=torch.int64).contiguous().reshape(-1)
    H, W = pan.shape
    ws = torch.empty((int(lib().upsnet_unified_pan_workspace_bytes()),), dtype=torch.uint8, device=pan.device)
    out = torch.empty((H, W, 3), dtype=torch.uint8, device=pan.device)
    check(lib().upsnet_unified_pan_result(stream(), ptr(pan), ptr(seg), ptr(cls_inds) if cls_inds.numel() else None, int(cls_inds.numel()),
                                          H, W, int(id_last_stuff), int(num_seg_classes), int(stuff_area_limit), ptr(ws), ptr(out)),
          "unified_pan_result")
    return out


COMBINED_PAN_CHUNK_IMAGES = 256
COMBINED_PAN_CHUNK_PIXELS = 1 << 28
_SEG_BLOCK = 4096


def _combined_seg_u8(seg, dev):
    if isinstance(seg, torch.Tensor):
        t = seg
    else:
        a = np.asarray(seg)
        if a.ndim == 2 and a.dtype != np.uint8 and a.size:
            if not np.issubdtype(a.dtype, np.integer) or int(a.min()) < 0 or int(a.max()) > 255:
                raise ValueError("combined_pan_result: semantic labels must be integers in 0..255")
            a = a.astype(np.uint8)
        t = torch.from_numpy(np.ascontiguousarray(a))
    if t.dim() != 2:
        raise ValueError("combined_pan_result: semantic maps must be [H,W], got %s" % (tuple(t.shape),))
    if t.dtype != torch.uint8 and (t.dtype.is_floating_point or t.dtype.is_complex or t.dtype == torch.bool):
        raise ValueError("combined_pan_result: semantic maps must be uint8 or int64, got %s" % t.dtype)
    return t.to(dev)


def combined_pan_result(segs, boxes, masks, id_last_stuff, score_threshold=0.6, fraction_threshold=0.7, stuff_area_limit=4 * 64 * 64):
    from .dataset.rle import _segmented_cumsum, decode_rle_strings
    n = len(segs)
    if len(boxes) != len(masks):
        raise ValueError("combined_pan_result: %d classes of boxes, %d of masks" % (len(boxes), len(masks)))
    num_classes = len(boxes)
    if num_classes < 2 or id_last_stuff < 0 or id_last_stuff + num_classes - 1 >= 255:
        raise ValueError("combined_pan_result: %d classes after id_last_stuff %d do not fit the uint8 labels" % (num_classes, id_last_stuff))
    for c in range(1, num_classes):
        if len(boxes[c]) != n or len(masks[c]) != n:
            raise ValueError("combined_pan_result: class %d has boxes for %d and masks for %d of %d images" % (c, len(boxes[c]), len(masks[c]), n))
    if n == 0:
        return []
    dev = next((s.device for s in segs if isinstance(s, torch.Tensor) and s.is_cuda), None) or torch.device('cuda', torch.cuda.current_device())
    seg_t = [_combined_seg_u8(s, dev) for s in segs]
    wide = [t for t in seg_t if t.dtype != torch.uint8 and t.numel()]
    if wide:
        r = torch.stack([torch.stack([t.min(), t.max()]).to(torch.int64) for t in wide]).cpu()
        if int(r[:, 0].min()) < 0 or int(r[:, 1].max()) > 255:
            raise ValueError("combined_pan_result: semantic labels must be integers in 0..255")
    seg_t = [t.to(torch.uint8).contiguous() for t in seg_t]
    thr = float(score_threshold)
    strings, cls_of, npix_of, img_ncand = [], [], [], []
    for i, t in enumerate(seg_t):
        H, W = int(t.shape[0]), int(t.shape[1])
        if H * W > (1 << 24):
            raise ValueError("combined_pan_result: image %d has %d x %d pixels; the pixel counts are exact only up to 2^24" % (i, H, W))
        sc, cl, rl = [], [], []
        for c in range(1, num_classes):
            b, m = boxes[c][i], masks[c][i]
            b = np.asarray(b)
            nb = b.shape[0] if b.size else 0
            if nb != len(m):
                raise ValueError("combined_pan_result: image %d class %d: %d boxes, %d masks" % (i, c, nb, len(m)))
            if nb:
                if b.ndim != 2 or b.shape[1] < 5:
                    raise ValueError("combined_pan_result: image %d class %d: boxes must be [n,5], got %s" % (i, c, b.shape))
                sc.append(b[:, 4].astype(np.float64))
                cl.append(np.full(nb, c, np.int32))
                rl.extend(m)
        for r in rl:
            if not isinstance(r, dict) or [int(v) for v in r.get('size', ())] != [H, W]:
                raise ValueError("combined_pan_result: image %d: mask size %s differs from the semantic map's %s" %
                                 (i, r.get('size') if isinstance(r, dict) else type(r), [H, W]))
        if sc:
            s = np.concatenate(sc)
            order = np.argsort(s, kind='stable')[::-1]
            order = order[~(s[order] < thr)]
            cls = np.concatenate(cl)[order]
            per = np.bincount(cls, minlength=num_classes)
            if per.max(initial=0) > 255:
                raise ValueError("combined_pan_result: image %d class %d has %d candidates at or above the score threshold; the "
                                 "instance ids are uint8" % (i, int(per.argmax()), int(per.max())))
            for k in order:
                cnt = rl[k]['counts']
                if not isinstance(cnt, (str, bytes)):
                    raise ValueError("combined_pan_result: image %d: RLE counts must be a compressed string" % i)
                strings.append(cnt)
            cls_of.append(cls)
        npix_of.append(np.full(len(order) if sc else 0, H * W, np.int64))
        img_ncand.append(len(order) if sc else 0)
    cls_all = np.concatenate(cls_of) if cls_of else np.zeros(0, np.int32)
    npix_all = np.concatenate(npix_of)
    counts, off = decode_rle_strings(strings)
    ncodes = np.diff(off)
    str_of = np.repeat(np.arange(len(strings)), ncodes)
    if counts.size and counts.min() < 0:
        raise ValueError("combined_pan_result: negative RLE count (string %d)" % int(str_of[np.argmax(counts < 0)]))
    total = np.bincount(str_of, weights=counts.astype(np.float64), minlength=len(strings))
    bad = np.flatnonzero(total != npix_all)
    if bad.size:
        raise ValueError("combined_pan_result: RLE counts of candidate %d sum to %d, not H * W = %d" %
                         (int(bad[0]), int(total[bad[0]]), int(npix_all[bad[0]])))
    first = np.zeros(counts.size, bool)
    first[off[:-1][ncodes > 0]] = True
    pos = _segmented_cumsum(counts, first) if counts.size else counts
    j = np.arange(counts.size) - np.repeat(off[:-1], ncodes)
    odd = np.flatnonzero(((j & 1) == 1) & (counts > 0))
    run_b = pos[odd]
    run_a = run_b - counts[odd]
    run_str = str_of[odd]
    area = np.bincount(run_str, weights=(run_b - run_a).astype(np.float64), minlength=len(strings)).astype(np.int64)
    blk_a, blk_b = run_a // _SEG_BLOCK, (run_b - 1) // _SEG_BLOCK
    nseg = blk_b - blk_a + 1
    run_idx = np.repeat(np.arange(run_a.size), nseg)
    blk = blk_a[run_idx] + (np.arange(run_idx.size) - np.repeat(np.cumsum(nseg) - nseg, nseg))
    seg_a = np.maximum(run_a[run_idx], blk * _SEG_BLOCK)
    seg_b = np.minimum(run_b[run_idx], (blk + 1) * _SEG_BLOCK)
    seg_str = run_str[run_idx]
    seg_cnt = np.bincount(seg_str, minlength=len(strings))
    keep = area > 0
    cand_img = np.repeat(np.arange(n), img_ncand)
    out = [torch.empty((int(t.shape[0]), int(t.shape[1]), 3), dtype=torch.uint8, device=dev) for t in seg_t]
    live = [i for i in range(n) if seg_t[i].numel()]
    chunks, cur, cur_pix = [], [], 0
    for i in live:
        p = seg_t[i].numel()
        if cur and (len(cur) >= COMBINED_PAN_CHUNK_IMAGES or cur_pix + p > COMBINED_PAN_CHUNK_PIXELS):
            chunks.append(cur)
            cur, cur_pix = [], 0
        cur.append(i)
        cur_pix += p
    if cur:
        chunks.append(cur)
    for ch in chunks:
        in_chunk = keep & np.isin(cand_img, ch)
        sel = np.flatnonzero(in_chunk)
        cbeg = np.concatenate([[0], np.cumsum(np.bincount(np.searchsorted(ch, cand_img[sel]), minlength=len(ch)))])
        segs_sel = np.flatnonzero(in_chunk[seg_str])
        c_seg_end = np.cumsum(seg_cnt[sel])
        cand = np.stack([cls_all[sel], area[sel], c_seg_end - seg_cnt[sel], c_seg_end], 1).astype(np.int32) if sel.size else None
        segs_np = np.stack([seg_a[segs_sel], seg_b[segs_sel]], 1).astype(np.int32) if segs_sel.size else None
        hw = np.array([[int(seg_t[i].shape[0]), int(seg_t[i].shape[1])] for i in ch], np.int64)
        npx = hw[:, 0] * hw[:, 1]
        img = np.zeros((len(ch), 8), np.int64)
        img[:, 0:2] = hw
        img[:, 2] = [seg_t[i].data_ptr() for i in ch]
        img[:, 3] = [out[i].data_ptr() for i in ch]
        img[:, 4], img[:, 5] = cbeg[:-1], cbeg[1:]
        img[:, 6] = np.concatenate([[0], np.cumsum((npx + 63) // 64)[:-1]])
        img[:, 7] = np.concatenate([[0], np.cumsum(npx)[:-1]])
        total_pix = int(npx.sum())
        img_d = torch.from_numpy(img).to(dev)
        cand_d = torch.from_numpy(cand).to(dev) if cand is not None else None
        segs_d = torch.from_numpy(segs_np).to(dev) if segs_np is not None else None
        ws = torch.empty((int(lib().upsnet_combined_pan_workspace_bytes(len(ch), total_pix)),), dtype=torch.uint8, device=dev)
        check(lib().upsnet_combined_pan_result(stream(), len(ch), ptr(img_d), int(hw[:, 0].max()), int(hw[:, 1].max()), total_pix,
                                               ptr(cand_d), ptr(segs_d), int(id_last_stuff), num_classes, int(stuff_area_limit),
                                               float(fraction_threshold), ptr(ws)), "combined_pan_result")
    return out


def pq_workspace(max_gt, device):
    nbytes = int(lib().upsnet_pq_workspace_bytes(int(max_gt)))
    if nbytes == 0:
        raise ValueError("pq_workspace: max_gt %d outside 0..4096" % max_gt)
    return torch.zeros((nbytes,), dtype=torch.uint8, device=device)


def pq_accumulate(pred_2ch, gt_rgb, segments, cat_known, image_index, max_gt, workspace, tp, fp, fn, iou, status):
    require_cuda(pred_2ch, gt_rgb, segments, cat_known, workspace, tp, fp, fn, iou, status)
    if pred_2ch.dtype != torch.uint8 or gt_rgb.dtype != torch.uint8 or pred_2ch.dim() != 3 or pred_2ch.shape[2] != 3 \
            or tuple(pred_2ch.shape) != tuple(gt_rgb.shape):
        raise ValueError("pq_accumulate: pred_2ch %s %s and gt_rgb %s %s must both be uint8 [H,W,3]"
                         % (tuple(pred_2ch.shape), pred_2ch.dtype, tuple(gt_rgb.shape), gt_rgb.dtype))
    if segments.dtype != torch.int64 or segments.dim() != 2 or segments.shape[1] != 4:
        raise ValueError("pq_accumulate: segments must be int64 [n,4]")
    for t, dt, n in ((cat_known, torch.uint8, 256), (tp, torch.int64, 256), (fp, torch.int64, 256), (fn, torch.int64, 256),
                     (iou, torch.float64, 256), (status, torch.int64, 1)):
        if t.dtype != dt or t.numel() != n or not t.is_contiguous():
            raise ValueError("pq_accumulate: accumulator / table of %d %s expected, got %s %s" % (n, dt, tuple(t.shape), t.dtype))
    pred_2ch, gt_rgb, segments = pred_2ch.contiguous(), gt_rgb.contiguous(), segments.contiguous()
    H, W = pred_2ch.shape[:2]
    check(lib().upsnet_pq_accumulate(stream(), ptr(pred_2ch), ptr(gt_rgb), H, W, ptr(segments) if segments.numel() else None,
                                     int(segments.shape[0]), ptr(cat_known), int(image_index), int(max_gt), ptr(workspace), ptr(tp), ptr(fp),
                                     ptr(fn), ptr(iou), ptr(status)), "pq_accumulate")


def confusion_accumulate(gt_label, pred_label, class_num, ignore_label, confusion):
    require_cuda(gt_label, pred_label, confusion)
    if gt_label.dtype != torch.uint8 or pred_label.dtype != torch.uint8 or gt_label.shape != pred_label.shape:
        raise ValueError("confusion_accumulate: gt %s %s and pred %s %s must both be uint8 of one shape"
                         % (tuple(gt_label.shape), gt_label.dtype, tuple(pred_label.shape), pred_label.dtype))
    if confusion.dtype != torch.int64 or tuple(confusion.shape) != (class_num, class_num) or not confusion.is_contiguous():
        raise ValueError("confusion_accumulate: confusion must be a contiguous int64 [%d,%d] tensor" % (class_num, class_num))
    gt_label, pred_label = gt_label.contiguous(), pred_label.contiguous()
    check(lib().upsnet_confusion_accumulate(stream(), ptr(gt_label), ptr(pred_label), int(gt_label.numel()), int(class_num),
                                            int(ignore_label), ptr(confusion)), "confusion_accumulate")
    return confusion


def mask_roi_dedup(a_src, a_cls, a_num, b_src, b_cls, b_boxes, b_num):
    require_cuda(a_src, b_src, b_boxes)
    cap_a, cap_b = a_src.shape[0], b_src.shape[0]
    dev = b_boxes.device
    mp = torch.empty((cap_b,), dtype=torch.int32, device=dev)
    extra = torch.empty((cap_b, 5), dtype=torch.float32, device=dev)
    n_extra = torch.empty((1,), dtype=torch.int32, device=dev)
    check(lib().upsnet_mask_roi_dedup(stream(), ptr(a_src), ptr(a_cls), ptr(a_num), cap_a, ptr(b_src), ptr(b_cls), ptr(f32c(b_boxes)),
                                      ptr(b_num), cap_b, ptr(mp), ptr(extra), ptr(n_extra)), "mask_roi_dedup")
    return mp, extra, n_extra


def pack_winograd_weight(weight, tn32=False):
    require_cuda(weight)
    weight = f32c(weight)
    Cout, Cin, kh, kw = weight.shape
    if (kh, kw) != (3, 3):
        raise RuntimeError("pack_winograd_weight: kernel must be 3x3")
    if tn32:
        ldw = (Cout + 31) // 32 * 32
        wp = torch.empty((16 * Cin, ldw), dtype=torch.float32, device=weight.device)
        check(lib().upsnet_conv_pack_weight_winograd_tn32(stream(), ptr(weight), Cout, Cin, ldw, ptr(wp)), "conv_pack_weight_winograd_tn32")
        return wp, ldw
    ldw = 32 if Cout <= 32 else (Cout + 63) // 64 * 64
    wp = torch.empty((16 * Cin, ldw), dtype=torch.float32, device=weight.device)
    check(lib().upsnet_conv_pack_weight_winograd(stream(), ptr(weight), Cout, Cin, ldw, ptr(wp)), "conv_pack_weight_winograd")
    return wp, ldw


def conv2d_winograd_splitk(x, wpack, ldw, bias, cout, ksplit, relu=False, residual=None):
    require_cuda(x, wpack)
    x = nhwc(x.float())
    N, C, H, W = x.shape
    out = _nhwc_out(N, cout, H, W, x.device)
    res = None
    if residual is not None:
        res = nhwc(residual.float())
        if tuple(res.shape) != tuple(out.shape):
            raise RuntimeError("conv2d_winograd_splitk: residual shape %s != %s" % (tuple(res.shape), tuple(out.shape)))
    ws = _ws(lib().upsnet_conv2d_splitk_workspace_bytes(N, H, W, int(cout), 3, 3, 1, 1, int(ksplit)), x.device)
    ev0 = _prof_begin()
    check(lib().upsnet_conv2d_winograd_nhwc_f32_splitk(stream(), ptr(x), ptr(res), ptr(out), N, H, W, C, ptr(wpack), int(ldw),
                                                       ptr(None if bias is None else f32c(bias)), int(cout), int(bool(relu)), int(ksplit),
                                                       ptr(ws)), "conv2d_winograd_nhwc_f32_splitk")
    if ev0 is not None:
        npix = N * H * W
        _prof_end(ev0, 'conv', 2.0 * cout * C * 9 * npix, 4.0 * (C * npix + cout * npix * (2 if res is not None else 1) + cout * C * 9),
                  "winograd split-K x%d 3x3/1 %d->%d %s" % (ksplit, C, cout, (N, H, W)))
    return out


def conv2d_winograd_tail(x, wpack, ldw, wpack32, ldw32, bias, cout, n_main, relu=False):
    require_cuda(wpack, wpack32, x)
    x = nhwc(x.float())
    N, C, H, W = x.shape
    out = _nhwc_out(N, cout, H, W, x.device)
    ev0 = _prof_begin()
    check(lib().upsnet_conv2d_winograd_nhwc_f32_tail(stream(), ptr(x), ptr(out), int(N), int(n_main), int(H), int(W), int(C), ptr(wpack), int(ldw),
                                                     ptr(wpack32), int(ldw32), ptr(None if bias is None else f32c(bias)), int(cout),
                                                     int(bool(relu))), "conv2d_winograd_nhwc_f32_tail")
    if ev0 is not None:
        npix = N * H * W
        _prof_end(ev0, 'conv', 2.0 * cout * C * 9 * npix, 4.0 * (C * npix + cout * npix + cout * C * 9),
                  "winograd 3x3/1 %d->%d [%s] tail %d" % (C, cout, (N, H, W), N - n_main))
    return out


def conv2d_winograd_multi(xs, wpack, ldw, bias, cout, relu=False, residuals=None, outs=None, tn32=False):
    require_cuda(wpack, *xs)
    assert 1 <= len(xs) <= 5
    xs = [nhwc(x.float()) for x in xs]
    cin = xs[0].shape[1]
    given, outs, ress = outs, [], None
    for i, x in enumerate(xs):
        N, C, H, W = x.shape
        if C != cin:
            raise RuntimeError("conv2d_winograd_multi: channel mismatch")
        if given is not None:
            o = given[i]
            if tuple(o.shape) != (N, cout, H, W) or o.dtype != torch.float32 or not o.permute(0, 2, 3, 1).is_contiguous():
                raise RuntimeError("conv2d_winograd_multi: outs[%d] must be a channels_last fp32 [%d,%d,%d,%d]" % (i, N, cout, H, W))
            outs.append(o)
        else:
            outs.append(_nhwc_out(N, cout, H, W, x.device))
    if residuals is not None:
        ress = [nhwc(r.float()) for r in residuals]
        for r, o in zip(ress, outs):
            if tuple(r.shape) != tuple(o.shape):
                raise RuntimeError("conv2d_winograd: residual shape %s != %s" % (tuple(r.shape), tuple(o.shape)))
    ev0 = _prof_begin()
    fn = lib().upsnet_conv2d_winograd_nhwc_f32_tn32 if tn32 else lib().upsnet_conv2d_winograd_nhwc_f32
    check(fn(stream(), len(xs), ptr_array(xs), ptr_array(ress) if ress is not None else None,
             ptr_array(outs), int_array([x.shape[0] for x in xs]), int_array([x.shape[2] for x in xs]),
             int_array([x.shape[3] for x in xs]), int(cin), ptr(wpack), int(ldw),
             ptr(None if bias is None else f32c(bias)), int(cout), int(bool(relu))),
          "conv2d_winograd_nhwc_f32")
    if ev0 is not None:
        npix = sum(o.shape[0] * o.shape[2] * o.shape[3] for o in outs)
        _prof_end(ev0, 'conv', 2.0 * cout * cin * 9 * npix, 4.0 * (cin * npix + cout * npix * (2 if ress is not None else 1) + cout * cin * 9),
                  "winograd 3x3/1 %d->%d %s%s%s" % (cin, cout, [tuple(x.shape[0:1] + x.shape[2:]) for x in xs],
                                                    " +res" if ress is not None else "", " tn32" if tn32 else ""))
    return outs


def pack_winograd36_weight(weight):
    require_cuda(weight)
    weight = f32c(weight)
    Cout, Cin, kh, kw = weight.shape
    if (kh, kw) != (3, 3) or Cin % 32:
        raise RuntimeError("pack_winograd36_weight: 3x3 kernel and Cin %% 32 == 0")
    ldw = (Cout + 63) // 64 * 64
    wp = torch.empty((36 * Cin, ldw), dtype=torch.float32, device=weight.device)
    check(lib().upsnet_conv_pack_weight_winograd36(stream(), ptr(weight), Cout, Cin, ldw, ptr(wp)), "conv_pack_weight_winograd36")
    return wp, ldw


def conv2d_winograd36_multi(xs, wpack, ldw, bias, cout, relu=False, outs=None):
    require_cuda(wpack, *xs)
    assert 1 <= len(xs) <= 5
    xs = [nhwc(x.float()) for x in xs]
    cin = xs[0].shape[1]
    given, outs = outs, []
    for i, x in enumerate(xs):
        N, C, H, W = x.shape
        if C != cin:
            raise RuntimeError("conv2d_winograd36_multi: channel mismatch")
        if given is not None:
            o = given[i]
            if tuple(o.shape) != (N, cout, H, W) or o.dtype != torch.float32 or not o.permute(0, 2, 3, 1).is_contiguous():
                raise RuntimeError("conv2d_winograd36_multi: outs[%d] must be a channels_last fp32 [%d,%d,%d,%d]" % (i, N, cout, H, W))
            outs.append(o)
        else:
            outs.append(_nhwc_out(N, cout, H, W, x.device))
    ev0 = _prof_begin()
    check(lib().upsnet_conv2d_winograd36_nhwc_f32(stream(), len(xs), ptr_array(xs), ptr_array(outs), int_array([x.shape[0] for x in xs]),
                                                  int_array([x.shape[2] for x in xs]), int_array([x.shape[3] for x in xs]), int(cin), ptr(wpack),
                                                  int(ldw), ptr(None if bias is None else f32c(bias)), int(cout), int(bool(relu))),
          "conv2d_winograd36_nhwc_f32")
    if ev0 is not None:
        npix = sum(o.shape[0] * o.shape[2] * o.shape[3] for o in outs)
        _prof_end(ev0, 'conv', 2.0 * cout * cin * 9 * npix, 4.0 * (cin * npix + cout * npix + cout * cin * 9),
                  "winograd36 3x3/1 %d->%d %s" % (cin, cout, [tuple(x.shape[0:1] + x.shape[2:]) for x in xs]))
    return outs


def conv2d_winograd36_splitk(x, wpack, ldw, bias, cout, ksplit, relu=False):
    require_cuda(wpack, x)
    x = nhwc(x.float())
    N, cin, H, W = x.shape
    out = _nhwc_out(N, cout, H, W, x.device)
    ws = _ws(lib().upsnet_conv2d_winograd36_splitk_workspace_bytes(N, H, W, int(cout), int(ksplit)), x.device)
    ev0 = _prof_begin()
    check(lib().upsnet_conv2d_winograd36_nhwc_f32_splitk(stream(), ptr(x), ptr(out), N, H, W, int(cin), ptr(wpack), int(ldw),
                                                         ptr(None if bias is None else f32c(bias)), int(cout), int(bool(relu)), int(ksplit), ptr(ws)),
          "conv2d_winograd36_nhwc_f32_splitk")
    if ev0 is not None:
        npix = N * H * W
        _prof_end(ev0, 'conv', 2.0 * cout * cin * 9 * npix, 4.0 * (cin * npix + cout * npix + cout * cin * 9),
                  "winograd36 split-K x%d 3x3/1 %d->%d %s" % (ksplit, cin, cout, (N, H, W)))
    return out


def pack_conv_weight_bf16(weight, split=True):
    require_cuda(weight)
    weight = f32c(weight)
    Cout, Cin, kh, kw = weight.shape
    ldw = (Cout + 127) // 128 * 128
    shape = (kh * kw * Cin // 32, ldw, 32)
    hi = torch.empty(shape, dtype=torch.bfloat16, device=weight.device)
    lo = torch.empty(shape, dtype=torch.bfloat16, device=weight.device) if split else None
    check(lib().upsnet_conv_pack_weight_bf16(stream(), ptr(weight), Cout, Cin, kh, kw, ldw, ptr(hi), ptr(lo)), "conv_pack_weight_bf16")
    return hi, lo, ldw


def conv2d_nhwc_bf16_multi(xs, whi, wlo, ldw, bias, cout, ksize, stride, pad, relu=False, residuals=None, residual_up=False,
                           out_dtype=torch.float32):
    require_cuda(whi, *xs)
    assert 1 <= len(xs) <= 5
    in16 = xs[0].dtype == torch.bfloat16
    out16 = out_dtype == torch.bfloat16
    if (in16 or out16) and wlo is not None:
        raise RuntimeError("conv2d_nhwc_bf16_multi: bf16 tensors only in the plain bf16 mode")
    xs = [nhwc(x if (in16 and x.dtype == torch.bfloat16) else x.float()) for x in xs]
    if in16 and any(x.dtype != torch.bfloat16 for x in xs):
        raise RuntimeError("conv2d_nhwc_bf16_multi: mixed input dtypes in one launch")
    cin = xs[0].shape[1]
    outs, ress = [], None
    for x in xs:
        N, C, H, W = x.shape
        if C != cin:
            raise RuntimeError("conv2d_nhwc_bf16_multi: channel mismatch")
        Ho, Wo = (H + 2 * pad - ksize) // stride + 1, (W + 2 * pad - ksize) // stride + 1
        outs.append(torch.empty((N, Ho, Wo, cout), dtype=torch.bfloat16, device=x.device).permute(0, 3, 1, 2) if out16
                    else _nhwc_out(N, cout, Ho, Wo, x.device))
    res16 = False
    if residuals is not None:
        res16 = residuals[0].dtype == torch.bfloat16 and wlo is None
        ress = [nhwc(r if (res16 and r.dtype == torch.bfloat16) else r.float()) for r in residuals]
        if res16 and any(r.dtype != torch.bfloat16 for r in ress):
            raise RuntimeError("conv2d_nhwc_bf16_multi: mixed residual dtypes in one launch")
        for r, o in zip(ress, outs):
            want = (o.shape[0], o.shape[1], o.shape[2] // 2, o.shape[3] // 2) if residual_up else tuple(o.shape)
            if tuple(r.shape) != want:
                raise RuntimeError("conv2d_nhwc_bf16: residual shape %s != %s" % (tuple(r.shape), want))
    ev0 = _prof_begin()
    check(lib().upsnet_conv2d_nhwc_bf16(stream(), len(xs), ptr_array(xs), ptr_array(ress) if ress is not None else None, ptr_array(outs),
                                        int_array([x.shape[0] for x in xs]), int_array([x.shape[2] for x in xs]),
                                        int_array([x.shape[3] for x in xs]), int(cin), ptr(whi), ptr(wlo), int(ldw),
                                        ptr(None if bias is None else f32c(bias)), int(cout), int(ksize), int(ksize), int(stride), int(pad),
                                        int(bool(relu)) | (2 if (residual_up and ress is not None) else 0) | (4 if in16 else 0) |
                                        (8 if out16 else 0) | (16 if res16 else 0)), "conv2d_nhwc_bf16")
    if ev0 is not None:
        npix = sum(o.shape[0] * o.shape[2] * o.shape[3] for o in outs)
        nin = sum(x.shape[0] * x.shape[2] * x.shape[3] for x in xs)
        _prof_end(ev0, 'conv_bf16', 2.0 * cout * cin * ksize * ksize * npix,
                  (2.0 if in16 else 4.0) * cin * nin + (2.0 if out16 else 4.0) * cout * npix +
                  ((2.0 if res16 else 4.0) * cout * npix * (0.25 if residual_up else 1.0) if ress is not None else 0.0) +
                  2.0 * cout * cin * ksize * ksize)
    return outs


def _bf16_fragments(w2d):
    cout, k = w2d.shape
    return w2d.to(torch.bfloat16).view(cout // 32, 32, k // 16, 2, 8).permute(0, 2, 3, 1, 4).contiguous()


def pack_bottleneck_bf16(w1, w2, w3, b1, b2, b3):
    require_cuda(w1, w2, w3)
    cm, c = w1.shape[0], w1.shape[1]
    if not (c == 4 * cm and tuple(w2.shape) == (cm, cm, 3, 3) and tuple(w3.shape) == (c, cm, 1, 1) and cm in (64, 128, 256, 512)):
        raise RuntimeError("pack_bottleneck_bf16: not an identity bottleneck of width 64/128/256/512")
    zeros = lambda n: torch.zeros(n, dtype=torch.float32, device=w1.device)
    return (_bf16_fragments(w1.detach().float().reshape(cm, c)),
            _bf16_fragments(w2.detach().float().permute(0, 2, 3, 1).reshape(cm, 9 * cm)),
            _bf16_fragments(w3.detach().float().reshape(c, cm)),
            zeros(cm) if b1 is None else f32c(b1.detach()), zeros(cm) if b2 is None else f32c(b2.detach()),
            zeros(c) if b3 is None else f32c(b3.detach()), cm)


def pack_bottleneck_proj_bf16(w1, w2, w3, wd, b1, b2, b3, bd):
    require_cuda(w1, w2, w3, wd)
    cm, cin = w1.shape[0], w1.shape[1]
    c = 4 * cm
    if not (tuple(w2.shape) == (cm, cm, 3, 3) and tuple(w3.shape) == (c, cm, 1, 1) and tuple(wd.shape) == (c, cin, 1, 1) and
            (cm, cin) in ((64, 64), (128, 256), (256, 512))):
        raise RuntimeError("pack_bottleneck_proj_bf16: not the first bottleneck of res2 / res3 / res4")
    z = lambda b, n: torch.zeros(n, dtype=torch.float32, device=w1.device) if b is None else f32c(b.detach())
    w3d = torch.cat([w3.detach().float().reshape(c, cm), wd.detach().float().reshape(c, cin)], 1)
    return (_bf16_fragments(w1.detach().float().reshape(cm, cin)),
            _bf16_fragments(w2.detach().float().permute(0, 2, 3, 1).reshape(cm, 9 * cm)),
            _bf16_fragments(w3d), z(b1, cm), z(b2, cm), (z(b3, c) + z(bd, c)).contiguous(), cm, cin)


def bottleneck_proj_bf16(x, pack, stride):
    w1, w2, w3d, b1, b2, b3d, cm, cin = pack
    require_cuda(x, w1)
    if x.dtype != torch.bfloat16 or x.shape[1] != cin:
        raise RuntimeError("bottleneck_proj_bf16: expects a bf16 map of %d channels" % cin)
    x = nhwc(x)
    N, C, H, W = x.shape
    Ho, Wo = (H - 1) // stride + 1, (W - 1) // stride + 1
    out = torch.empty((N, Ho, Wo, 4 * cm), dtype=torch.bfloat16, device=x.device).permute(0, 3, 1, 2)
    ev0 = _prof_begin()
    check(lib().upsnet_bottleneck_proj_bf16(stream(), ptr(x), ptr(out), N, H, W, int(cin), int(cm), int(stride), ptr(w1), ptr(w2), ptr(w3d),
                                            ptr(b1), ptr(b2), ptr(b3d)), "bottleneck_proj_bf16")
    if ev0 is not None:
        k = cm * cin + 9 * cm * cm + 4 * cm * (cm + cin)
        _prof_end(ev0, 'bottleneck_bf16', 2.0 * k * N * Ho * Wo, 2.0 * C * N * Ho * Wo + 2.0 * 4 * cm * N * Ho * Wo + 2.0 * k)
    return out


def bottleneck_bf16(x, pack):
    w1, w2, w3, b1, b2, b3, cm = pack
    require_cuda(x, w1)
    if x.dtype != torch.bfloat16 or x.shape[1] != 4 * cm:
        raise RuntimeError("bottleneck_bf16: expects a bf16 map of %d channels" % (4 * cm))
    x = nhwc(x)
    N, C, H, W = x.shape
    out = torch.empty((N, H, W, C), dtype=torch.bfloat16, device=x.device).permute(0, 3, 1, 2)
    ev0 = _prof_begin()
    check(lib().upsnet_bottleneck_bf16(stream(), ptr(x), ptr(out), N, H, W, cm, ptr(w1), ptr(w2), ptr(w3), ptr(b1), ptr(b2), ptr(b3)),
          "bottleneck_bf16")
    if ev0 is not None:
        _prof_end(ev0, 'bottleneck_bf16', 2.0 * 17 * cm * cm * N * H * W, 2.0 * 2 * C * N * H * W + 2.0 * 17 * cm * cm)
    return out


def conv2d_nhwc_splitk(x, wpack, ldw, bias, cout, ksize, stride, pad, ksplit, relu=False, residual=None):
    require_cuda(x, wpack)
    x = nhwc(x.float())
    N, C, H, W = x.shape
    Ho, Wo = (H + 2 * pad - ksize) // stride + 1, (W + 2 * pad - ksize) // stride + 1
    out = _nhwc_out(N, cout, Ho, Wo, x.device)
    res = None
    if residual is not None:
        res = nhwc(residual.float())
        if tuple(res.shape) != tuple(out.shape):
            raise RuntimeError("conv2d_nhwc_splitk: residual shape %s != %s" % (tuple(res.shape), tuple(out.shape)))
    ws = _ws(lib().upsnet_conv2d_splitk_workspace_bytes(N, H, W, int(cout), int(ksize), int(ksize), int(stride), int(pad), int(ksplit)), x.device)
    ev0 = _prof_begin()
    check(lib().upsnet_conv2d_nhwc_f32_splitk(stream(), ptr(x), ptr(res), ptr(out), N, H, W, C, ptr(wpack), int(ldw),
                                              ptr(None if bias is None else f32c(bias)), int(cout), int(ksize), int(ksize), int(stride),
                                              int(pad), int(bool(relu)), int(ksplit), ptr(ws)), "conv2d_nhwc_f32_splitk")
    if ev0 is not None:
        npix = N * Ho * Wo
        _prof_end(ev0, 'conv', 2.0 * cout * C * ksize * ksize * npix,
                  4.0 * (C * N * H * W + cout * npix * (2 if res is not None else 1) + cout * C * ksize * ksize),
                  "split-K x%d %dx%d/%d %d->%d %s" % (ksplit, ksize, ksize, stride, C, cout, (N, H, W)))
    return out


PROPOSAL_RECALL_MAX_GT = 4096


def proposal_recall_workspace_bytes(num_problems, total_proposals):
    return int(lib().upsnet_proposal_recall_workspace_bytes(int(num_problems), int(total_proposals)))


def proposal_recall(problems, proposals, gt_boxes, max_gt, total_proposals, workspace, out):
    require_cuda(problems, proposals, gt_boxes, workspace, out)
    if problems.dtype != torch.int64 or problems.dim() != 2 or problems.shape[1] != 6 or not problems.is_contiguous():
        raise ValueError("proposal_recall: problems must be a contiguous int64 [n, 6] table, got %s %s" % (problems.dtype, tuple(problems.shape)))
    for name, b in (('proposals', proposals), ('gt_boxes', gt_boxes)):
        if b.dtype != torch.float32 or b.dim() != 2 or b.shape[1] != 4 or not b.is_contiguous():
            raise ValueError("proposal_recall: %s must be contiguous float32 [., 4], got %s %s" % (name, b.dtype, tuple(b.shape)))
    if not 0 <= int(max_gt) <= PROPOSAL_RECALL_MAX_GT:
        raise ValueError("proposal_recall: %d GT boxes in a problem (at most %d)" % (int(max_gt), PROPOSAL_RECALL_MAX_GT))
    n = int(problems.shape[0])
    if workspace.numel() * workspace.element_size() < proposal_recall_workspace_bytes(n, total_proposals):
        raise ValueError("proposal_recall: workspace of %d bytes, %d needed" % (workspace.numel() * workspace.element_size(),
                                                                             proposal_recall_workspace_bytes(n, total_proposals)))
    if out.dtype != torch.float32 or not out.is_contiguous():
        raise ValueError("proposal_recall: out must be contiguous float32")
    check(lib().upsnet_proposal_recall(stream(), n, ptr(problems), ptr(proposals), ptr(gt_boxes), int(max_gt), int(total_proposals),
                                       ptr(workspace), ptr(out)), "proposal_recall")
    return out
```

Baseline: 171.8.

## Let Winograd convs read strided NHWC views and fold histogram zeroing into key kernel

Adds strided-input variants of the Winograd 16 and 36 conv kernels that take per-segment pixel and row pitches. The Python wrappers can then pass non-contiguous channels_last views, such as the stride-2 subsampled P6, without first copying them into a packed NHWC buffer. FPN P6 is now produced as a strided view of P5 (p5[:, :, ::2, ::2]) rather than by calling the fpn_p6 module. The proposal histogram clear is moved into prop_key_kernel, which removes a separate memset launch but relies on every block of that grid running before the histogram is used.

```diff
diff --git a/include/upsnet_hip.h b/include/upsnet_hip.h
--- a/include/upsnet_hip.h
+++ b/include/upsnet_hip.h
@@ -125,6 +125,9 @@
 int upsnet_conv2d_winograd_nhwc_f32(void *stream, int nseg, const float *const x[], const float *const residual[],
                                     float *const out[], const int batch[], const int height[], const int width[], int Cin,
                                     const float *wpack, int ldw, const float *bias, int Cout, int relu);
+int upsnet_conv2d_winograd_nhwc_f32_strided(void *stream, int nseg, const float *const x[], const int xpix[], const int xrow[],
+                                            const float *const residual[], float *const out[], const int batch[], const int height[],
+                                            const int width[], int Cin, const float *wpack, int ldw, const float *bias, int Cout, int relu);
 
 int upsnet_conv2d_winograd_nhwc_f32_splitk(void *stream, const float *x, const float *residual, float *out, int batch, int height,
                                            int width, int Cin, const float *wpack, int ldw, const float *bias, int Cout, int relu,
@@ -184,6 +187,9 @@
 int upsnet_conv2d_winograd36_nhwc_f32(void *stream, int nseg, const float *const x[], float *const out[], const int batch[],
                                       const int height[], const int width[], int Cin, const float *wpack, int ldw, const float *bias,
                                       int Cout, int relu);
+int upsnet_conv2d_winograd36_nhwc_f32_strided(void *stream, int nseg, const float *const x[], const int xpix[], const int xrow[],
+                                              float *const out[], const int batch[], const int height[], const int width[], int Cin,
+                                              const float *wpack, int ldw, const float *bias, int Cout, int relu);
 int upsnet_conv_pack_weight_winograd36(void *stream, const float *weight, int cout, int cin, int ldw, float *wpack);
 size_t upsnet_conv2d_winograd36_splitk_workspace_bytes(int batch, int height, int width, int Cout, int ksplit);
 int upsnet_conv2d_winograd36_nhwc_f32_splitk(void *stream, const float *x, float *out, int batch, int height, int width, int Cin,
diff --git a/upsnet_amd/_lib.py b/upsnet_amd/_lib.py
--- a/upsnet_amd/_lib.py
+++ b/upsnet_amd/_lib.py
@@ -97,12 +97,14 @@
     "upsnet_combined_pan_result": (c_int, [P, c_int, P, c_int, c_int, c_long, P, P, c_int, c_int, c_int, c_double, P]),
     "upsnet_mask_roi_dedup": (c_int, [P, P, P, P, c_int, P, P, P, P, c_int, P, P, P]),
     "upsnet_conv2d_winograd_nhwc_f32": (c_int, [P, c_int, P, P, P, P, P, P, c_int, P, c_int, P, c_int, c_int]),
+    "upsnet_conv2d_winograd_nhwc_f32_strided": (c_int, [P, c_int, P, P, P, P, P, P, P, P, c_int, P, c_int, P, c_int, c_int]),
     "upsnet_conv2d_winograd_nhwc_f32_splitk": (c_int, [P, P, P, P, c_int, c_int, c_int, c_int, P, c_int, P, c_int, c_int, c_int, P]),
     "upsnet_conv_pack_weight_winograd": (c_int, [P, P, c_int, c_int, c_int, P]),
     "upsnet_conv_pack_weight_winograd_tn32": (c_int, [P, P, c_int, c_int, c_int, P]),
     "upsnet_conv2d_winograd_nhwc_f32_tn32": (c_int, [P, c_int, P, P, P, P, P, P, c_int, P, c_int, P, c_int, c_int]),
     "upsnet_conv2d_winograd_nhwc_f32_tail": (c_int, [P, P, P, c_int, c_int, c_int, c_int, c_int, P, c_int, P, c_int, P, c_int, c_int]),
     "upsnet_conv2d_winograd36_nhwc_f32": (c_int, [P, c_int, P, P, P, P, P, c_int, P, c_int, P, c_int, c_int]),
+    "upsnet_conv2d_winograd36_nhwc_f32_strided": (c_int, [P, c_int, P, P, P, P, P, P, P, c_int, P, c_int, P, c_int, c_int]),
     "upsnet_conv_pack_weight_winograd36": (c_int, [P, P, c_int, c_int, c_int, P]),
     "upsnet_conv2d_nhwc_bf16": (c_int, [P, c_int, P, P, P, P, P, P, c_int, P, P, c_int, P, c_int, c_int, c_int, c_int, c_int, c_int]),
     "upsnet_bottleneck_proj_bf16": (c_int, [P, P, P, c_int, c_int, c_int, c_int, c_int, c_int, P, P, P, P, P, P]),
diff --git a/upsnet_amd/csrc/conv_params.h b/upsnet_amd/csrc/conv_params.h
--- a/upsnet_amd/csrc/conv_params.h
+++ b/upsnet_amd/csrc/conv_params.h
@@ -16,6 +16,8 @@
     int OH, OW;
     int tile_start;
     long M;
+    int xpix, xrow;
+    long xext;
 };
 
 struct ConvParams {
@@ -61,18 +63,35 @@
             UPS_REQUIRE(s.Ho > 0 && s.Wo > 0, "%s: empty output for feature map %d", who, i);
             UPS_REQUIRE((long)nb * height[i] * width[i] * Cin < (1L << 30), "%s: feature map %d exceeds 4 GiB (32-bit byte offsets); split the batch", who, i);
             s.M = (long)nb * s.Ho * s.Wo;
+            s.xpix = Cin; s.xrow = width[i] * Cin; s.xext = (long)nb * height[i] * width[i] * Cin;
             UPS_REQUIRE(s.M * Cout < (1L << 29), "%s: output %d exceeds 2 GiB (32-bit byte offsets in the epilogue); split the batch", who, i);
             s.tile_start = tiles;
             tiles += (int)((s.M + 127) / 128);
         } else {
             s.x = s.res = s.off = s.mask = nullptr; s.w = nullptr; s.out = nullptr;
             s.N = s.H = s.W = s.Ho = s.Wo = s.OH = s.OW = 0; s.M = 0; s.tile_start = 0x7fffffff;
+            s.xpix = s.xrow = 0; s.xext = 0;
         }
     }
     p.m_tiles = tiles;
     return 0;
 }
 
+static inline int conv_set_xstride(ConvParams &p, const char *who, const int xpix[], const int xrow[])
+{
+    if (!xpix || !xrow) return 0;
+    for (int i = 0; i < p.nseg; ++i) {
+        ConvSeg &s = p.seg[i];
+        if (xpix[i] == 0 && xrow[i] == 0) continue;
+        UPS_REQUIRE(xpix[i] >= p.Cin && xpix[i] % 4 == 0 && xrow[i] % 4 == 0 && (long)xrow[i] >= (long)(s.W - 1) * xpix[i] + p.Cin,
+                    "%s: feature map %d: pixel pitch >= Cin, row pitch >= one row, both multiples of 4 elements (got %d, %d)", who, i, xpix[i], xrow[i]);
+        s.xpix = xpix[i]; s.xrow = xrow[i];
+        s.xext = ((long)s.N * s.H - 1) * s.xrow + (long)(s.W - 1) * s.xpix + p.Cin;
+        UPS_REQUIRE(s.xext < (1L << 28), "%s: feature map %d spans more than 1 GiB; split the batch", who, i);
+    }
+    return 0;
+}
+
 
 int conv_splitk_reduce(hipStream_t st, const float *partial, int ksplit, long m_total, long M, int Cout, const float *bias, const float *res,
                        int relu, float *out);
diff --git a/upsnet_amd/csrc/conv_wino.hip b/upsnet_amd/csrc/conv_wino.hip
--- a/upsnet_amd/csrc/conv_wino.hip
+++ b/upsnet_amd/csrc/conv_wino.hip
@@ -62,13 +62,13 @@
         const int rem = (int)(ppc - (long)n * HoWo);
         const int ty = rem / sg.Wo, tx = rem - ty * sg.Wo;
         const int h0 = 2 * ty - 1, w0 = 2 * tx - 1;
-        const unsigned cin4 = 4u * (unsigned)p.Cin;
+        const unsigned pix4 = 4u * (unsigned)sg.xpix, row4 = 4u * (unsigned)sg.xrow;
         unsigned ro[4], co[4];
 #pragma unroll
         for (int r = 0; r < 4; ++r) {
             const int h = h0 + r, w = w0 + r;
-            const unsigned rv = (unsigned)((n * sg.H + min(max(h, 0), sg.H - 1)) * sg.W) * cin4;
-            const unsigned cv = (unsigned)min(max(w, 0), sg.W - 1) * cin4 + 8u * (unsigned)lc2;
+            const unsigned rv = (unsigned)(n * sg.H + min(max(h, 0), sg.H - 1)) * row4;
+            const unsigned cv = (unsigned)min(max(w, 0), sg.W - 1) * pix4 + 8u * (unsigned)lc2;
             ro[r] = rv | ((tile_ok && h >= 0 && h < sg.H) ? 0u : 0x80000000u);
             co[r] = cv | ((w >= 0 && w < sg.W) ? 0u : 0x40000000u);
         }
@@ -77,7 +77,7 @@
     }
     const size_t xaddr = reinterpret_cast<size_t>(sg.x);
     const unsigned xlo = __builtin_amdgcn_readfirstlane((unsigned)xaddr), xhi = __builtin_amdgcn_readfirstlane((unsigned)(xaddr >> 32));
-    const unsigned xbytes = __builtin_amdgcn_readfirstlane((unsigned)(sg.N * sg.H * sg.W) * 4u * (unsigned)p.Cin);
+    const unsigned xbytes = __builtin_amdgcn_readfirstlane((unsigned)sg.xext * 4u);
     const char *xbase = reinterpret_cast<const char *>(((size_t)xhi << 32) | xlo);
     const unsigned st_base = (unsigned)((lq * TM + (ltile ^ (2 * lq))) * 16 + (lc2 & 1) * 8);
     const int frow = 32 * wm + l32;
@@ -312,7 +312,7 @@
 {
     UPS_REQUIRE(p.Cin % 16 == 0 && (p.ldw == 32 || p.ldw % 64 == 0 || (tn32 && p.ldw % 32 == 0)), "conv2d_winograd_nhwc_f32: Cin %% 16 must be 0 and ldw 32 or a multiple of 64");
     for (int i = 0; i < p.nseg; ++i) {
-        UPS_REQUIRE((long)p.seg[i].N * p.seg[i].H * p.seg[i].W * p.Cin < (1L << 28), "conv2d_winograd_nhwc_f32: feature map %d exceeds 1 GiB; split the batch", i);
+        UPS_REQUIRE((long)p.seg[i].N * p.seg[i].H * p.seg[i].W * p.Cin < (1L << 28) && p.seg[i].xext < (1L << 28), "conv2d_winograd_nhwc_f32: feature map %d exceeds 1 GiB; split the batch", i);
         UPS_REQUIRE((long)p.seg[i].N * p.seg[i].OH * p.seg[i].OW * p.Cout < (1L << 29), "conv2d_winograd_nhwc_f32: output %d exceeds 2 GiB; split the batch", i);
     }
     if (p.ksplit > 1) {
@@ -412,6 +412,19 @@
 {
     ConvParams p;
     int rc = wino_fill(p, "conv2d_winograd_nhwc_f32", nseg, x, residual, out, batch, height, width, Cin, Cout, wpack, ldw, bias, relu);
+    if (rc) return rc;
+    return conv_wino16_launch((hipStream_t)stream, p);
+}
+
+extern "C" int upsnet_conv2d_winograd_nhwc_f32_strided(void *stream, int nseg, const float *const x[], const int xpix[], const int xrow[],
+                                                       const float *const residual[], float *const out[], const int batch[], const int height[],
+                                                       const int width[], int Cin, const float *wpack, int ldw, const float *bias, int Cout, int relu)
+{
+    ConvParams p;
+    int rc = wino_fill(p, "conv2d_winograd_nhwc_f32_strided", nseg, x, residual, out, batch, height, width, Cin, Cout, wpack, ldw, bias, relu);
+    if (rc) return rc;
+    UPS_REQUIRE(xpix && xrow, "conv2d_winograd_nhwc_f32_strided: null pointer");
+    rc = conv_set_xstride(p, "conv2d_winograd_nhwc_f32_strided", xpix, xrow);
     if (rc) return rc;
     return conv_wino16_launch((hipStream_t)stream, p);
 }
diff --git a/upsnet_amd/csrc/conv_wino36.hip b/upsnet_amd/csrc/conv_wino36.hip
--- a/upsnet_amd/csrc/conv_wino36.hip
+++ b/upsnet_amd/csrc/conv_wino36.hip
@@ -86,7 +86,7 @@
 #pragma unroll
         for (int c = 0; c < 6; ++c) ncmask |= (wcol0 + c >= 0 && wcol0 + c < sg.W) ? 0u : (1u << c);
         lane_fix = tile_ok && (nrmask | ncmask) != 0;
-        tbase = (unsigned)(hrow0 * sg.W + wcol0) * (4u * (unsigned)p.Cin) + 4u * (unsigned)lch;
+        tbase = (unsigned)hrow0 * (4u * (unsigned)sg.xrow) + (unsigned)wcol0 * (4u * (unsigned)sg.xpix) + 4u * (unsigned)lch;
     }
     const bool fix = __builtin_amdgcn_ballot_w64(lane_fix) != 0ull;
     bool risky;
@@ -94,17 +94,17 @@
         const long plast = min(p0 + (long)W36_TM, sg.M) - 1;
         const long nl = plast / HoWo;
         const long tyl = (plast - nl * HoWo) / sg.Wo;
-        risky = (nl * sg.H + 4 * tyl + 4) * (long)sg.W + 4L * sg.Wo >= (long)sg.N * sg.H * sg.W;
-    }
-    const unsigned cin4 = 4u * (unsigned)p.Cin;
-    const unsigned rowpitch = (unsigned)sg.W * cin4;
+        risky = (nl * sg.H + 4 * tyl + 4) * (long)sg.xrow + 4L * sg.Wo * sg.xpix + p.Cin > sg.xext;
+    }
+    const unsigned cin4 = 4u * (unsigned)sg.xpix;
+    const unsigned rowpitch = 4u * (unsigned)sg.xrow;
     const unsigned cin4_s = __builtin_amdgcn_readfirstlane(cin4);
-    const unsigned rowpitch_s = __builtin_amdgcn_readfirstlane((unsigned)sg.W) * cin4_s;
+    const unsigned rowpitch_s = __builtin_amdgcn_readfirstlane(rowpitch);
     const unsigned cbase = (unsigned)wcol0 * cin4 + 4u * (unsigned)lch;
 #define W36_ROWOFF(R) (((unsigned)min(max(hrow0 + (R), hlo), max(hhi - 1, hlo)) * rowpitch) | ((hrow0 + (R) >= hlo && hrow0 + (R) < hhi) ? 0u : 0x80000000u))
     const size_t xaddr = reinterpret_cast<size_t>(sg.x);
     const unsigned xlo = __builtin_amdgcn_readfirstlane((unsigned)xaddr), xhi = __builtin_amdgcn_readfirstlane((unsigned)(xaddr >> 32));
-    const unsigned xbytes = __builtin_amdgcn_readfirstlane((unsigned)(sg.N * sg.H * sg.W) * 4u * (unsigned)p.Cin - (SK ? (unsigned)s_first * 64u : 0u));
+    const unsigned xbytes = __builtin_amdgcn_readfirstlane((unsigned)sg.xext * 4u - (SK ? (unsigned)s_first * 64u : 0u));
     const char *xbase = reinterpret_cast<const char *>(((size_t)xhi << 32) | xlo) + (SK ? (size_t)s_first * 64 : 0);
 #define W36_SWZ(Q) ((((Q) & 1) << 2) | (((Q) >> 1) << 1))
     const unsigned st_base = (unsigned)((((lch >> 2) * W36_TM + (ltile ^ W36_SWZ(lch >> 2))) * 16) + (lch & 3) * 4);
@@ -285,6 +285,8 @@
     return 0;
 }
 
+static int w36_launch(hipStream_t stream, const ConvParams &p);
+
 extern "C" int upsnet_conv2d_winograd36_nhwc_f32(void *stream, int nseg, const float *const x[], float *const out[], const int batch[],
                                                  const int height[], const int width[], int Cin, const float *wpack, int ldw, const float *bias,
                                                  int Cout, int relu)
@@ -292,13 +294,31 @@
     ConvParams p;
     int rc = w36_fill(p, "conv2d_winograd36_nhwc_f32", nseg, x, out, batch, height, width, Cin, Cout, wpack, ldw, bias, relu);
     if (rc) return rc;
+    return w36_launch((hipStream_t)stream, p);
+}
+
+static int w36_launch(hipStream_t stream, const ConvParams &p)
+{
     static std::atomic<unsigned long long> attr_dev{0};
     UPS_ONCE_PER_DEVICE(attr_dev, UPS_CHECK_HIP(hipFuncSetAttribute(reinterpret_cast<const void *>(&conv_wino36_f32_kernel<false>), hipFuncAttributeMaxDynamicSharedMemorySize, W36_XCH)));
     const int grid = 8 * ((p.m_tiles + 7) / 8) * p.n_tiles;
-    hipLaunchKernelGGL(conv_wino36_f32_kernel<false>, dim3(grid), dim3(512), W36_XCH, (hipStream_t)stream, p);
+    hipLaunchKernelGGL(conv_wino36_f32_kernel<false>, dim3(grid), dim3(512), W36_XCH, stream, p);
     UPS_CHECK_LAUNCH("conv_wino36_f32_kernel");
     ups_set_form("wino36<%d,%d>", W36_TM, W36_TN);
     return 0;
+}
+
+extern "C" int upsnet_conv2d_winograd36_nhwc_f32_strided(void *stream, int nseg, const float *const x[], const int xpix[], const int xrow[],
+                                                         float *const out[], const int batch[], const int height[], const int width[], int Cin,
+                                                         const float *wpack, int ldw, const float *bias, int Cout, int relu)
+{
+    ConvParams p;
+    int rc = w36_fill(p, "conv2d_winograd36_nhwc_f32_strided", nseg, x, out, batch, height, width, Cin, Cout, wpack, ldw, bias, relu);
+    if (rc) return rc;
+    UPS_REQUIRE(xpix && xrow, "conv2d_winograd36_nhwc_f32_strided: null pointer");
+    rc = conv_set_xstride(p, "conv2d_winograd36_nhwc_f32_strided", xpix, xrow);
+    if (rc) return rc;
+    return w36_launch((hipStream_t)stream, p);
 }
 
 extern "C" size_t upsnet_conv2d_winograd36_splitk_workspace_bytes(int batch, int height, int width, int Cout, int ksplit)
diff --git a/upsnet_amd/csrc/proposal.hip b/upsnet_amd/csrc/proposal.hip
--- a/upsnet_amd/csrc/proposal.hip
+++ b/upsnet_amd/csrc/proposal.hip
@@ -36,7 +36,7 @@
 #define PROP_BINS 2048
 
 __global__ void __launch_bounds__(256)
-prop_key_kernel(const PropLevels lv, ups_u64 *__restrict__ keys, PropSel *__restrict__ sel, const int k)
+prop_key_kernel(const PropLevels lv, ups_u64 *__restrict__ keys, PropSel *__restrict__ sel, unsigned *__restrict__ hist, const int k)
 {
     const int l = blockIdx.y;
     if (blockIdx.x == 0 && threadIdx.x == 0) {
@@ -44,6 +44,7 @@
         st.prefix = 0; st.need = (unsigned)k; st.done = 0; st.cnt = 0; st.pad = 0;
         sel[l] = st;
     }
+    for (int i = blockIdx.x * blockDim.x + threadIdx.x; i < PROP_BINS; i += blockDim.x * gridDim.x) hist[(long)l * PROP_BINS + i] = 0u;
     const int n = lv.n[l], A = lv.A;
     const long hw = (long)lv.H[l] * lv.W[l];
     const float *__restrict__ s = lv.cls[l];
@@ -582,8 +583,7 @@
     if (gx > 1024) gx = 1024;
     unsigned *hist = (unsigned *)(ws + plan.off_hist);
     PropSel *sel = (PropSel *)(ws + plan.off_sel);
-    if (ups_zero_async(hist, (size_t)nlev * PROP_BINS * 4, st)) return 1;
-    hipLaunchKernelGGL(prop_key_kernel, dim3(gx, nlev), dim3(256), 0, st, lv, kbuf[0], sel, pre_n);
+    hipLaunchKernelGGL(prop_key_kernel, dim3(gx, nlev), dim3(256), 0, st, lv, kbuf[0], sel, hist, pre_n);
     UPS_CHECK_LAUNCH("prop_key_kernel");
 
     if (int rc = prop_select_compact(st, lv, nlev, maxn, pre_n, kbuf[0], kbuf[1], hist, sel)) return rc;
diff --git a/upsnet_amd/models/fpn.py b/upsnet_amd/models/fpn.py
--- a/upsnet_amd/models/fpn.py
+++ b/upsnet_amd/models/fpn.py
@@ -58,5 +58,5 @@
         p3 = hipconv.conv(self.fpn_p3, p3_plus)
         p2 = hipconv.conv(self.fpn_p2, p2_plus)
         if hasattr(self, 'fpn_p6'):
-            return p2, p3, p4, p5, self.fpn_p6(p5)
+            return p2, p3, p4, p5, p5[:, :, ::2, ::2]
         return p2, p3, p4, p5
diff --git a/upsnet_amd/ops.py b/upsnet_amd/ops.py
--- a/upsnet_amd/ops.py
+++ b/upsnet_amd/ops.py
@@ -1309,10 +1309,20 @@
     return out
 
 
+def _nhwc_pitched(x):
+    N, C, H, W = x.shape
+    if x.dtype == torch.float32 and not x.is_contiguous(memory_format=torch.channels_last):
+        sn, sc, sh, sw = x.stride()
+        if (sc == 1 and sw >= C and sw % 4 == 0 and sh % 4 == 0 and sh >= (W - 1) * sw + C and (N == 1 or sn == H * sh)
+                and x.data_ptr() % 16 == 0):
+            return x, sw, sh
+    return nhwc(x.float()), 0, 0
+
+
 def conv2d_winograd_multi(xs, wpack, ldw, bias, cout, relu=False, residuals=None, outs=None, tn32=False):
     require_cuda(wpack, *xs)
     assert 1 <= len(xs) <= 5
-    xs = [nhwc(x.float()) for x in xs]
+    xs, xpix, xrow = zip(*[(nhwc(x.float()), 0, 0) if tn32 else _nhwc_pitched(x) for x in xs])
     cin = xs[0].shape[1]
     given, outs, ress = outs, [], None
     for i, x in enumerate(xs):
@@ -1332,12 +1342,16 @@
             if tuple(r.shape) != tuple(o.shape):
                 raise RuntimeError("conv2d_winograd: residual shape %s != %s" % (tuple(r.shape), tuple(o.shape)))
     ev0 = _prof_begin()
-    fn = lib().upsnet_conv2d_winograd_nhwc_f32_tn32 if tn32 else lib().upsnet_conv2d_winograd_nhwc_f32
-    check(fn(stream(), len(xs), ptr_array(xs), ptr_array(ress) if ress is not None else None,
-             ptr_array(outs), int_array([x.shape[0] for x in xs]), int_array([x.shape[2] for x in xs]),
-             int_array([x.shape[3] for x in xs]), int(cin), ptr(wpack), int(ldw),
-             ptr(None if bias is None else f32c(bias)), int(cout), int(bool(relu))),
-          "conv2d_winograd_nhwc_f32")
+    tail = (ptr_array(outs), int_array([x.shape[0] for x in xs]), int_array([x.shape[2] for x in xs]),
+            int_array([x.shape[3] for x in xs]), int(cin), ptr(wpack), int(ldw),
+            ptr(None if bias is None else f32c(bias)), int(cout), int(bool(relu)))
+    rs = ptr_array(ress) if ress is not None else None
+    if any(xpix):
+        check(lib().upsnet_conv2d_winograd_nhwc_f32_strided(stream(), len(xs), ptr_array(xs), int_array(xpix), int_array(xrow), rs, *tail),
+              "conv2d_winograd_nhwc_f32_strided")
+    else:
+        fn = lib().upsnet_conv2d_winograd_nhwc_f32_tn32 if tn32 else lib().upsnet_conv2d_winograd_nhwc_f32
+        check(fn(stream(), len(xs), ptr_array(xs), rs, *tail), "conv2d_winograd_nhwc_f32")
     if ev0 is not None:
         npix = sum(o.shape[0] * o.shape[2] * o.shape[3] for o in outs)
         _prof_end(ev0, 'conv', 2.0 * cout * cin * 9 * npix, 4.0 * (cin * npix + cout * npix * (2 if ress is not None else 1) + cout * cin * 9),
@@ -1361,7 +1375,7 @@
 def conv2d_winograd36_multi(xs, wpack, ldw, bias, cout, relu=False, outs=None):
     require_cuda(wpack, *xs)
     assert 1 <= len(xs) <= 5
-    xs = [nhwc(x.float()) for x in xs]
+    xs, xpix, xrow = zip(*[_nhwc_pitched(x) for x in xs])
     cin = xs[0].shape[1]
     given, outs = outs, []
     for i, x in enumerate(xs):
@@ -1376,10 +1390,13 @@
         else:
             outs.append(_nhwc_out(N, cout, H, W, x.device))
     ev0 = _prof_begin()
-    check(lib().upsnet_conv2d_winograd36_nhwc_f32(stream(), len(xs), ptr_array(xs), ptr_array(outs), int_array([x.shape[0] for x in xs]),
-                                                  int_array([x.shape[2] for x in xs]), int_array([x.shape[3] for x in xs]), int(cin), ptr(wpack),
-                                                  int(ldw), ptr(None if bias is None else f32c(bias)), int(cout), int(bool(relu))),
-          "conv2d_winograd36_nhwc_f32")
+    tail = (ptr_array(outs), int_array([x.shape[0] for x in xs]), int_array([x.shape[2] for x in xs]), int_array([x.shape[3] for x in xs]),
+            int(cin), ptr(wpack), int(ldw), ptr(None if bias is None else f32c(bias)), int(cout), int(bool(relu)))
+    if any(xpix):
+        check(lib().upsnet_conv2d_winograd36_nhwc_f32_strided(stream(), len(xs), ptr_array(xs), int_array(xpix), int_array(xrow), *tail),
+              "conv2d_winograd36_nhwc_f32_strided")
+    else:
+        check(lib().upsnet_conv2d_winograd36_nhwc_f32(stream(), len(xs), ptr_array(xs), *tail), "conv2d_winograd36_nhwc_f32")
     if ev0 is not None:
         npix = sum(o.shape[0] * o.shape[2] * o.shape[3] for o in outs)
         _prof_end(ev0, 'conv', 2.0 * cout * cin * 9 * npix, 4.0 * (cin * npix + cout * npix + cout * cin * 9),
```

Result: no change. 171.8 (-0.0%).
